# LJacksonPan/RaTrack

Hardware: AMD Instinct MI355X
Metric: radar frame-pairs/sec (backbone forward, eval) at B=64,N=256 per GPU (higher is better)
Workload: dtype f32 (2xfp16 split MFMA: three fp16 products per fp32 product, fp32 accumulate, power-of-two scales per matrix and position); 1 GPU; Track4D.backbone forward, B=64 frame-pairs x N=256 points per GPU, S=512 centroids, eval-mode BN, random-init weights, hipGraph=True, batches in flight=4; global_batch=64, parallelism=replicas x1 (no collective on the forward path)

## Files before the change

include/rtk_fused.h:

```cpp
#ifndef RTK_FUSED_H
#define RTK_FUSED_H

#include "rtk_pointnet2.h"

#ifdef __cplusplus
extern "C" {
#endif

#define RTK_MAX_SRC 4
#define RTK_MAX_LAYERS 4

typedef struct {
    const float *ptr;
    int pitch;
    int channels;
    int per_sample;
} rtk_src_t;

#define RTK_LAYER_SPLIT 0x100
typedef struct {
    const float *w_packed;
    const float *bias;
    int cin16, cout16;
    int act;
    float inv_scale;
} rtk_layer_t;

typedef struct {
    const float *known_feats;
    int pitch, channels, m;
    const int *idx;
    const float *dist2;
    const int *nuniq;
} rtk_interp_t;

RTK_EXPORT int rtk_pointwise_mlp(int rows, int rows_per_sample, const rtk_interp_t *interp, int nsrc,
                                 const rtk_src_t *srcs, const float *sample_bias, int nlayers,
                                 const rtk_layer_t *layers, float *out, int out_pitch, int out_channels,
                                 int out_channel_major, const int *row_nuniq, float *colmax, rtk_stream_t stream);

RTK_EXPORT int rtk_sa_scale(int samples, int n, int npoint, int nsample, const float *xyz,
                            const float *new_xyz, const int *idx, const float *q, int q_pitch, int c1_16,
                            const float *w1xyz_packed, int nlayers, const rtk_layer_t *layers, float *out,
                            int out_pitch, int out_offset, const int *src_nuniq, const int *dst_nuniq,
                            rtk_stream_t stream);

RTK_EXPORT int rtk_cost_volume(int samples, int n1, int n2, const float *xyz1, const float *xyz2,
                               const int64_t *knn_idx, const float *p1, const float *p2,
                               const float *wd_packed, const rtk_layer_t *layers,
                               const rtk_layer_t *wn, float *out, int out_pitch, rtk_stream_t stream);

RTK_EXPORT int rtk_patch_cost(int samples, int n, const float *xyz, const int64_t *knn_idx,
                              const float *feat, int feat_pitch, const rtk_layer_t *wn, float *out,
                              int out_pitch, int out_channel_major, rtk_stream_t stream);

RTK_EXPORT int rtk_pack_split_layer(int cout, int cin, const float *w, int transposed, void *image, float *inv_scale,
                                    rtk_stream_t stream);
RTK_EXPORT int rtk_cost_volume_split(int samples, int n1, int n2, const float *xyz1, const float *xyz2,
                                     const int64_t *knn_idx, const float *p1, const float *p2, const float *wd_packed,
                                     const void *split_images, const float *image_scales, const float *bias2,
                                     const float *bias3, const rtk_layer_t *wn, float *out, int out_pitch, rtk_stream_t stream);
RTK_EXPORT int rtk_cost_volume_split_shared(int samples, int n1, int n2, const float *xyz1, const float *xyz2,
                                            const int64_t *knn_idx, const float *p1, const float *p2, const float *wd_packed,
                                            const void *split_images, const float *image_scales, const float *bias2,
                                            const float *bias3, const rtk_layer_t *wn, float *out, int out_pitch, int workgroups,
                                            rtk_stream_t stream);
RTK_EXPORT int rtk_sa_scale_split(int samples, int n, int npoint, int nsample, const float *xyz, const float *new_xyz,
                                  const int *idx, const float *q, int q_pitch, int c1, const float *w1xyz_packed,
                                  const void *split_image, const float *image_scale, const float *bias2, float *out, int out_pitch,
                                  int out_offset, const int *src_nuniq, const int *dst_nuniq, rtk_stream_t stream);
RTK_EXPORT int rtk_split_mlp2(int positions, const float *x, const void *images, const float *image_scales, const float *bias1,
                              const float *bias2, float *y, rtk_stream_t stream);

RTK_EXPORT int rtk_prepare_inputs(int b, int n, const float *pc1, const float *pc2, const float *feature1,
                                  const float *feature2, float *xyz, float *raw, rtk_stream_t stream);

RTK_EXPORT int rtk_fps_centroids(int b, int n, int npoint, const float *xyz, int *idx, float *new_xyz, int *nuniq,
                                 int *tie, const int *n_valid, float *snap, int *first_tie, rtk_stream_t stream);

RTK_EXPORT int rtk_knn_point_masked(int b, int s, int n, int k, const float *query, const float *points, int64_t *idx,
                                    const int *n_valid, rtk_stream_t stream);

RTK_EXPORT int rtk_fps_relevel(int b, int npoint, int levels, const float *xyz1, const int *nuniq1, const int *tie,
                               int *idx, float *new_xyz, int *nuniq, int *tie_work, const int *idx1, const float *snap1,
                               int snap_pitch, const int *first_tie1, rtk_stream_t stream);

RTK_EXPORT int rtk_gru_step(int b, int layers, int hidden, const float *x, const float *h_in, const float *w_ih,
                            const float *w_hh, const float *b_ih, const float *b_hh, float *h_out, float *y,
                            rtk_stream_t stream);

RTK_EXPORT int rtk_gru_step_head(int b, int layers, int hidden, const float *x, const float *h_in, const float *w_ih,
                                 const float *w_hh, const float *b_ih, const float *b_hh, float *h_out, float *y, const float *head_wt,
                                 const float *head_bias, float *head_out, int head_cout, rtk_stream_t stream);

#define RTK_GT_MAX_JOBS 4
typedef struct {
    const float *wt, *bias;
    float *out;
    int cout, s0, count, out_pitch;
} rtk_gterm_job_t;
RTK_EXPORT int rtk_global_terms(int samples, int cin, const float *g, int njobs, const rtk_gterm_job_t *jobs, float *bcast, int bcast_pitch,
                                int n, rtk_stream_t stream);

#define RTK_COPY_MAX_JOBS 8
typedef struct {
    const void *src;
    void *dst;
    long bytes;
} rtk_copy_job_t;
RTK_EXPORT int rtk_copy_multi(int njobs, const rtk_copy_job_t *jobs, rtk_stream_t stream);

RTK_EXPORT int rtk_to_channel_major(int samples, int n, int channels, const float *src, int src_pitch, int per_sample,
                                    float *dst, int dst_channels, int dst_channel_offset, rtk_stream_t stream);

RTK_EXPORT int rtk_ball_query_pair(int b, int n, int npoint, float radius1, int nsample1, float radius2, int nsample2,
                                   const float *new_xyz, const float *xyz, int *idx1, int *idx2, const int *nuniq,
                                   rtk_stream_t stream);

RTK_EXPORT int rtk_three_nn_masked(int b, int n, int m, const float *unknown, const float *known, float *dist2, int *idx,
                                   const int *unknown_nuniq, const int *known_nuniq, rtk_stream_t stream);

RTK_EXPORT int rtk_geometry_front(int b, int clouds, int n, int npoint, const float *frame1, const float *frame2, int channel_major,
                                  const float *feature1, const float *feature2, float *xyz, float *raw, int *fps_idx, float *new_xyz,
                                  int *nuniq, int *tie, int *first_tie, float *snap, const int *n_valid, int64_t *knn12, int64_t *knn11,
                                  const float *q1_w, float *q1_out, int q1_cout, rtk_stream_t stream);
RTK_EXPORT int rtk_geometry_tables(int samples, int n, int npoint, const float *xyz0, const float *new_xyz, const int *nuniq,
                                   const float *radii, const int *nsamples, int *const *ball, int *const *nn_idx, float *const *nn_dist2,
                                   rtk_stream_t stream);

typedef struct {
    const float *src; float *dst;
    int channels, src_pitch, per_sample, dst_channels, dst_channel_offset;
} rtk_layout_job_t;
RTK_EXPORT int rtk_to_channel_major_multi(int samples, int n, int njobs, const rtk_layout_job_t *jobs, rtk_stream_t stream);

RTK_EXPORT int rtk_log_sinkhorn(int m, int n, const float *scores, float alpha, int iters, float *out, rtk_stream_t stream);

RTK_EXPORT int rtk_dbscan(int n, const float *feat, int pitch, const int *channels, const float *score, float threshold, double eps,
                          int min_samples, int *labels, rtk_stream_t stream);

#define RTK_DESC 141

typedef struct {
    const float *ptr;
    long long sb, sc, sp;
} rtk_bcn_view_t;

typedef struct {
    int B, N;
    rtk_bcn_view_t pc1, flow, feature1, prop, cls;
    const int *n_valid;
    const unsigned char *active;
} rtk_track_frame_t;

#define RTK_DBSCAN_POINT_BYTES 48
RTK_EXPORT int rtk_dbscan_batched(const rtk_track_frame_t *frame, float threshold, double eps, int min_samples, int K, int *labels,
                                  int *obj, int *num_objects, int *flags, void *work, long long work_bytes, rtk_stream_t stream);

RTK_EXPORT int rtk_object_descriptors(const rtk_track_frame_t *frame, int K, const int *obj, const int *num_objects,
                                      const int *prev_count, const float *desc_prev, float *desc, rtk_stream_t stream);

#define RTK_AFFINITY_WEIGHTS (141 * 564 + 564 + 564 * 282 + 282 + 282 * 70 + 70 + 70 * 35 + 35 + 35 + 1)
RTK_EXPORT int rtk_affinity_pairs(int B, int K, const float *weights, const float *desc_prev, const int *prev_count,
                                  const unsigned char *reset, const float *desc, const int *num_objects, float *aff,
                                  rtk_stream_t stream);

RTK_EXPORT int rtk_associate_batched(int B, int N, int K, const unsigned char *active, const unsigned char *reset, const float *aff,
                                     const int *num_objects, const int *obj, const int *prev_ids, const int *prev_count, float alpha,
                                     int iters, int *counter, int *ids, int *count, int *object_ids, float *object_conf, int *indices1,
                                     int *num_prev, int *point_track_id, float *scores, rtk_stream_t stream);

RTK_EXPORT int rtk_track_max_objects(void);

#ifdef __cplusplus
}
#endif
#endif
```

ratrack_amd/csrc/fused_common.h:

```cpp
#pragma once
#include <hip/hip_runtime.h>

#include <utility>

typedef float f4 __attribute__((ext_vector_type(4)));

#define RTK_ACT_NONE 0
#define RTK_ACT_RELU 1
#define RTK_ACT_LEAKY 2
#define RTK_ACT_SIGMOID 3

__device__ __forceinline__ f4 f4_zero() { return (f4){0.f, 0.f, 0.f, 0.f}; }

__device__ __forceinline__ f4 mfma4(float a, float b, f4 c) { return __builtin_amdgcn_mfma_f32_16x16x4f32(a, b, c, 0, 0, 0); }

__device__ __forceinline__ float act1(float x, int act) {
    switch (act) {
        case RTK_ACT_RELU: return fmaxf(x, 0.f);
        case RTK_ACT_LEAKY: return x > 0.f ? x : 0.1f * x;
        case RTK_ACT_SIGMOID: return 1.f / (1.f + __expf(-x));
        default: return x;
    }
}

// ... 111 lines not shown
struct LayerStep {
    static constexpr int G = V >= 4 ? 4 : V;
    static constexpr int GV = (V + G - 1) / G;
    static constexpr int NG = U * GV;
    template <int GJ>
    static __device__ __forceinline__ void load(WS &ws, f4 (&dst)[G]) {
        constexpr int u = GJ / GV, v0 = (GJ % GV) * G;
#pragma unroll
        for (int q = 0; q < G; ++q) {
            if (v0 + q < V) {
                const int fi = FBASE + u * V + v0 + q;
                if (fi % F == 0 && fi != 0) ws.next();
                dst[q] = ws.frag(fi % F);
            }
        }
    }
    static __device__ __forceinline__ void run(WS &ws, const f4 (&h)[U], f4 (&acc)[V], f4 (&a)[2][G]) {
        constexpr int u = GI / GV, v0 = (GI % GV) * G;
        if constexpr (GI + 1 < NG) load<GI + 1>(ws, a[(GI + 1) & 1]);
        f4(&c)[G] = a[GI & 1];
#pragma unroll
        for (int q = 0; q < G; ++q) if (v0 + q < V) acc[v0 + q] = mfma4(c[q].x, h[u].x, acc[v0 + q]);
#pragma unroll
        for (int q = 0; q < G; ++q) if (v0 + q < V) acc[v0 + q] = mfma4(c[q].y, h[u].y, acc[v0 + q]);
#pragma unroll
        for (int q = 0; q < G; ++q) if (v0 + q < V) acc[v0 + q] = mfma4(c[q].z, h[u].z, acc[v0 + q]);
#pragma unroll
        for (int q = 0; q < G; ++q) if (v0 + q < V) acc[v0 + q] = mfma4(c[q].w, h[u].w, acc[v0 + q]);
        __builtin_amdgcn_sched_barrier(0);
    }
};

template <int U, int V, int FBASE, class WS, int F, int... GI>
__device__ __forceinline__ void mlp_layer_ws_impl(WS &ws, const f4 (&h)[U], f4 (&acc)[V], std::integer_sequence<int, GI...>) {
    constexpr int G = V >= 4 ? 4 : V;
    f4 a[2][G];
    LayerStep<U, V, FBASE, 0, WS, F>::template load<0>(ws, a[0]);
    (LayerStep<U, V, FBASE, GI, WS, F>::run(ws, h, acc, a), ...);
}

template <int U, int V, int FBASE, int NW, int F, int NF>
__device__ __forceinline__ void mlp_layer_ws(WStream<NW, F, NF> &ws, const f4 (&h)[U], f4 (&acc)[V]) {
    constexpr int G = V >= 4 ? 4 : V;
    constexpr int NG = U * ((V + G - 1) / G);
    mlp_layer_ws_impl<U, V, FBASE, WStream<NW, F, NF>, F>(ws, h, acc, std::make_integer_sequence<int, NG>{});
}


typedef __bf16 bf8v __attribute__((ext_vector_type(8)));
typedef unsigned u4v __attribute__((ext_vector_type(4)));

__device__ __forceinline__ unsigned pack_hi16(float lo, float hi) {
    return __builtin_amdgcn_perm(__float_as_uint(hi), __float_as_uint(lo), 0x07060302u);
}
__device__ __forceinline__ float trunc_bf16(float x) { return __uint_as_float(__float_as_uint(x) & 0xffff0000u); }

__device__ __forceinline__ void split3(const f4 x0, const f4 x1, u4v (&b)[3]) {
    float x[8] = {x0.x, x0.y, x0.z, x0.w, x1.x, x1.y, x1.z, x1.w}, r1[8], r2[8];
#pragma unroll
    for (int t = 0; t < 8; ++t) {
        r1[t] = __fsub_rn(x[t], trunc_bf16(x[t]));
        r2[t] = __fsub_rn(r1[t], trunc_bf16(r1[t]));
    }
#pragma unroll
    for (int w = 0; w < 4; ++w) {
        b[0][w] = pack_hi16(x[2 * w], x[2 * w + 1]);
        b[1][w] = pack_hi16(r1[2 * w], r1[2 * w + 1]);
        b[2][w] = pack_hi16(r2[2 * w], r2[2 * w + 1]);
    }
}


typedef _Float16 h8v __attribute__((ext_vector_type(8)));
typedef _Float16 h2v __attribute__((ext_vector_type(2)));
typedef float f2v __attribute__((ext_vector_type(2)));

struct LaneScale {
    float s;
    float inv;
    unsigned mb;
};
__device__ __forceinline__ LaneScale lane_scale_of(unsigned mbits) {
    const unsigned e = mbits >> 23;
    unsigned sf = 268u - e;
    sf = sf > 253u ? 253u : sf;
    return LaneScale{__uint_as_float(sf << 23), __uint_as_float((254u - sf) << 23), mbits};
}
__device__ __forceinline__ void tensor_amax_update(float *amax, unsigned mb) {
#pragma unroll
    for (int d = 32; d >= 1; d >>= 1) { const unsigned o = (unsigned)__shfl_xor((int)mb, d, 64); mb = o > mb ? o : mb; }
    if ((threadIdx.x & 63) == 0 && mb > __atomic_load_n(reinterpret_cast<unsigned *>(amax), __ATOMIC_RELAXED))
        atomicMax(reinterpret_cast<unsigned *>(amax), mb);
}

template <int N>
__device__ __forceinline__ float abs_max_f4(const f4 (&h)[N]) {
    float m = 0.f;
#pragma unroll
    for (int e = 0; e < N; ++e) {
        m = __builtin_fmaxf(__builtin_fmaxf(m, __builtin_fabsf(h[e].x)), __builtin_fabsf(h[e].y));
        m = __builtin_fmaxf(__builtin_fmaxf(m, __builtin_fabsf(h[e].z)), __builtin_fabsf(h[e].w));
    }
    return m;
}
struct SplitWord { unsigned h, l; };
__device__ __forceinline__ SplitWord split2_word(float xa, float xb, float s) {
    const f2v xs = (f2v){xa, xb} * s;
    const h2v h = __builtin_convertvector(xs, h2v);
    const _Float16 la = (_Float16)__builtin_fmaf(xa, s, -(float)h[0]);
    const _Float16 lb = (_Float16)__builtin_fmaf(xb, s, -(float)h[1]);
    return SplitWord{__builtin_bit_cast(unsigned, h), __builtin_bit_cast(unsigned, (h2v){la, lb})};
}
__device__ __forceinline__ void split2(const f4 x0, const f4 x1, float s, u4v (&b)[2]) {
    const SplitWord w0 = split2_word(x0.x, x0.y, s), w1 = split2_word(x0.z, x0.w, s), w2 = split2_word(x1.x, x1.y, s), w3 = split2_word(x1.z, x1.w, s);
    b[0] = (u4v){w0.h, w1.h, w2.h, w3.h};
    b[1] = (u4v){w0.l, w1.l, w2.l, w3.l};
}
__device__ __forceinline__ f4 mfma16_h(u4v a, u4v b, f4 c) {
    return __builtin_amdgcn_mfma_f32_16x16x32_f16(__builtin_bit_cast(h8v, a), __builtin_bit_cast(h8v, b), c, 0, 0, 0);
}

__device__ __forceinline__ f4 mfma16_bf(u4v a, u4v b, f4 c) {
    return __builtin_amdgcn_mfma_f32_16x16x32_bf16(__builtin_bit_cast(bf8v, a), __builtin_bit_cast(bf8v, b), c, 0, 0, 0);
}

constexpr int split16_nf(int U, int V) { return ((U + 1) / 2) * V * 2; }

template <int N>
__device__ __forceinline__ LaneScale lane_scale16(const f4 (&h)[N]) {
    unsigned mb = __float_as_uint(abs_max_f4(h));
    auto r = __builtin_amdgcn_permlane16_swap(mb, mb, false, false);
    mb = r[0] > r[1] ? r[0] : r[1];
    r = __builtin_amdgcn_permlane32_swap(mb, mb, false, false);
    return lane_scale_of(r[0] > r[1] ? r[0] : r[1]);
}

template <int U, int V, int FBASE, int GI, class WS, int F>
struct LayerStepS {
    static constexpr int GV = (V + 1) / 2;
    static constexpr int NG = ((U + 1) / 2) * GV;
    template <int GJ>
    static __device__ __forceinline__ void load(WS &ws, f4 (&dst)[4]) {
        constexpr int up = GJ / GV, v0 = (GJ % GV) * 2;
#pragma unroll
        for (int q = 0; q < 4; ++q) {
            if (v0 + q / 2 < V) {
                const int fi = FBASE + (up * V + v0 + q / 2) * 2 + q % 2;
                if (fi % F == 0 && fi != 0) ws.next();
                dst[q] = ws.frag(fi % F);
            }
        }
    }
    static __device__ __forceinline__ void run(WS &ws, const f4 (&h)[U], float scale, f4 (&acc)[V], f4 (&a)[2][4], u4v (&b)[2]) {
        constexpr int up = GI / GV, v0 = (GI % GV) * 2;
        if constexpr (GI + 1 < NG) load<GI + 1>(ws, a[(GI + 1) & 1]);
        if constexpr (GI % GV == 0) split2(h[2 * up], 2 * up + 1 < U ? h[2 * up + 1] : f4_zero(), scale, b);
        const f4(&c)[4] = a[GI & 1];
#define RTK_S16_MM(pa, pb)                                                                            \
        acc[v0] = mfma16_h(__builtin_bit_cast(u4v, c[pa]), b[pb], acc[v0]);                            \
        if constexpr (v0 + 1 < V) acc[v0 + 1] = mfma16_h(__builtin_bit_cast(u4v, c[2 + pa]), b[pb], acc[v0 + 1]);
        RTK_S16_MM(1, 0) RTK_S16_MM(0, 1) RTK_S16_MM(0, 0)
#undef RTK_S16_MM
        __builtin_amdgcn_sched_barrier(0);
    }
};

template <int U, int V, int FBASE, class WS, int F, int... GI>
__device__ __forceinline__ void mlp_layer_split_impl(WS &ws, const f4 (&h)[U], float scale, f4 (&acc)[V], std::integer_sequence<int, GI...>) {
    f4 a[2][4];
    u4v b[2];
    LayerStepS<U, V, FBASE, 0, WS, F>::template load<0>(ws, a[0]);
    (LayerStepS<U, V, FBASE, GI, WS, F>::run(ws, h, scale, acc, a, b), ...);
}

template <int U, int V, int FBASE, int NW, int F, int NF>
__device__ __forceinline__ void mlp_layer_ws_split(WStream<NW, F, NF> &ws, const f4 (&h)[U], float scale, f4 (&acc)[V]) {
    constexpr int NG = ((U + 1) / 2) * ((V + 1) / 2);
    mlp_layer_split_impl<U, V, FBASE, WStream<NW, F, NF>, F>(ws, h, scale, acc, std::make_integer_sequence<int, NG>{});
}

struct WResident {
    const f4 *w;
    int lane;
    __device__ __forceinline__ void next() {}
    __device__ __forceinline__ f4 frag(int f) const { return w[f * 64 + lane]; }
};

template <int U, int V>
__device__ __forceinline__ void mlp_layer_res(const f4 *w, int lane, const f4 (&h)[U], f4 (&acc)[V]) {
    constexpr int G = V >= 4 ? 4 : V;
    constexpr int NG = U * ((V + G - 1) / G);
    WResident wr{w, lane};
    mlp_layer_ws_impl<U, V, 0, WResident, (1 << 30)>(wr, h, acc, std::make_integer_sequence<int, NG>{});
}

__device__ __forceinline__ f4 bias_frag(const float *__restrict__ bias, int v, int g) {
    return *reinterpret_cast<const f4 *>(bias + 16 * v + 4 * g);
}

__device__ __forceinline__ void rtk_dpp_fence(f4 &v) {
    int zero;
    asm volatile("s_mov_b32 %0, 0" : "=s"(zero));
    v.x = __int_as_float(__float_as_int(v.x) | zero);
    v.y = __int_as_float(__float_as_int(v.y) | zero);
    v.z = __int_as_float(__float_as_int(v.z) | zero);
    v.w = __int_as_float(__float_as_int(v.w) | zero);
}
#define RTK_DPP4(op, ctrl)                                                 \
    op " %0, %0, %0 " ctrl " row_mask:0xf bank_mask:0xf\n"                 \
    op " %1, %1, %1 " ctrl " row_mask:0xf bank_mask:0xf\n"                 \
    op " %2, %2, %2 " ctrl " row_mask:0xf bank_mask:0xf\n"                 \
    op " %3, %3, %3 " ctrl " row_mask:0xf bank_mask:0xf\n"

__device__ __forceinline__ void row_max16_f4(f4 &v) {
    rtk_dpp_fence(v);
    asm volatile("s_nop 1\n" RTK_DPP4("v_max_f32_dpp", "row_ror:8") RTK_DPP4("v_max_f32_dpp", "row_ror:4")
                 RTK_DPP4("v_max_f32_dpp", "row_ror:2") RTK_DPP4("v_max_f32_dpp", "row_ror:1")
                 : "+v"(v.x), "+v"(v.y), "+v"(v.z), "+v"(v.w));
}

__device__ __forceinline__ void row_sum16_f4(f4 &v) {
    rtk_dpp_fence(v);
    asm volatile("s_nop 1\n" RTK_DPP4("v_add_f32_dpp", "row_ror:8") RTK_DPP4("v_add_f32_dpp", "row_ror:4")
                 RTK_DPP4("v_add_f32_dpp", "row_ror:2") RTK_DPP4("v_add_f32_dpp", "row_ror:1")
                 : "+v"(v.x), "+v"(v.y), "+v"(v.z), "+v"(v.w));
}

__device__ __forceinline__ void row_sum16_valu_f4(f4 &v) {
    asm volatile("s_nop 1\n" RTK_DPP4("v_add_f32_dpp", "row_ror:8") RTK_DPP4("v_add_f32_dpp", "row_ror:4")
                 RTK_DPP4("v_add_f32_dpp", "row_ror:2") RTK_DPP4("v_add_f32_dpp", "row_ror:1")
                 : "+v"(v.x), "+v"(v.y), "+v"(v.z), "+v"(v.w));
}

#define RTK_DPP16(op, ctrl)                                                                                                          \
    op " %0, %0, %0 " ctrl " row_mask:0xf bank_mask:0xf\n" op " %1, %1, %1 " ctrl " row_mask:0xf bank_mask:0xf\n"                   \
    op " %2, %2, %2 " ctrl " row_mask:0xf bank_mask:0xf\n" op " %3, %3, %3 " ctrl " row_mask:0xf bank_mask:0xf\n"                   \
    op " %4, %4, %4 " ctrl " row_mask:0xf bank_mask:0xf\n" op " %5, %5, %5 " ctrl " row_mask:0xf bank_mask:0xf\n"                   \
    op " %6, %6, %6 " ctrl " row_mask:0xf bank_mask:0xf\n" op " %7, %7, %7 " ctrl " row_mask:0xf bank_mask:0xf\n"                   \
    op " %8, %8, %8 " ctrl " row_mask:0xf bank_mask:0xf\n" op " %9, %9, %9 " ctrl " row_mask:0xf bank_mask:0xf\n"                   \
    op " %10, %10, %10 " ctrl " row_mask:0xf bank_mask:0xf\n" op " %11, %11, %11 " ctrl " row_mask:0xf bank_mask:0xf\n"             \
    op " %12, %12, %12 " ctrl " row_mask:0xf bank_mask:0xf\n" op " %13, %13, %13 " ctrl " row_mask:0xf bank_mask:0xf\n"             \
    op " %14, %14, %14 " ctrl " row_mask:0xf bank_mask:0xf\n" op " %15, %15, %15 " ctrl " row_mask:0xf bank_mask:0xf\n"
__device__ __forceinline__ void row_sum16_valu_f4x4(f4 (&v)[4]) {
    asm volatile("s_nop 1\n" RTK_DPP16("v_add_f32_dpp", "row_ror:8") RTK_DPP16("v_add_f32_dpp", "row_ror:4")
                 RTK_DPP16("v_add_f32_dpp", "row_ror:2") RTK_DPP16("v_add_f32_dpp", "row_ror:1")
                 : "+v"(v[0].x), "+v"(v[0].y), "+v"(v[0].z), "+v"(v[0].w), "+v"(v[1].x), "+v"(v[1].y), "+v"(v[1].z), "+v"(v[1].w),
                   "+v"(v[2].x), "+v"(v[2].y), "+v"(v[2].z), "+v"(v[2].w), "+v"(v[3].x), "+v"(v[3].y), "+v"(v[3].z), "+v"(v[3].w));
}

#define RTK_DPP_PAIR(op, c0, m0, c1, m1)                                                                                     \
    asm volatile("s_nop 1\n"                                                                                                 \
                 op " %0, %0, %0 " c0 " row_mask:0xf bank_mask:" m0 "\n" op " %1, %1, %1 " c0 " row_mask:0xf bank_mask:" m0 "\n"  \
                 op " %2, %2, %2 " c0 " row_mask:0xf bank_mask:" m0 "\n" op " %3, %3, %3 " c0 " row_mask:0xf bank_mask:" m0 "\n"  \
                 op " %0, %4, %4 " c1 " row_mask:0xf bank_mask:" m1 "\n" op " %1, %5, %5 " c1 " row_mask:0xf bank_mask:" m1 "\n"  \
                 op " %2, %6, %6 " c1 " row_mask:0xf bank_mask:" m1 "\n" op " %3, %7, %7 " c1 " row_mask:0xf bank_mask:" m1 "\n"  \
                 : "+v"(a.x), "+v"(a.y), "+v"(a.z), "+v"(a.w) : "v"(b.x), "v"(b.y), "v"(b.z), "v"(b.w))
__device__ __forceinline__ void row_max_pair8(f4 &a, const f4 b) { RTK_DPP_PAIR("v_max_f32_dpp", "row_ror:8", "0x3", "row_ror:8", "0xc"); }
__device__ __forceinline__ void row_max_pair4(f4 &a, const f4 b) { RTK_DPP_PAIR("v_max_f32_dpp", "row_shl:4", "0x5", "row_shr:4", "0xa"); }
__device__ __forceinline__ void row_sum_pair8(f4 &a, const f4 b) { RTK_DPP_PAIR("v_add_f32_dpp", "row_ror:8", "0x3", "row_ror:8", "0xc"); }
__device__ __forceinline__ void row_sum_pair4(f4 &a, const f4 b) { RTK_DPP_PAIR("v_add_f32_dpp", "row_shl:4", "0x5", "row_shr:4", "0xa"); }
#undef RTK_DPP_PAIR
__device__ __forceinline__ void quad_max_valu_f4(f4 &v) {
    asm volatile("s_nop 1\n" RTK_DPP4("v_max_f32_dpp", "quad_perm:[1,0,3,2]") RTK_DPP4("v_max_f32_dpp", "quad_perm:[2,3,0,1]")
                 : "+v"(v.x), "+v"(v.y), "+v"(v.z), "+v"(v.w));
}
__device__ __forceinline__ void quad_sum_valu_f4(f4 &v) {
    asm volatile("s_nop 1\n" RTK_DPP4("v_add_f32_dpp", "quad_perm:[1,0,3,2]") RTK_DPP4("v_add_f32_dpp", "quad_perm:[2,3,0,1]")
                 : "+v"(v.x), "+v"(v.y), "+v"(v.z), "+v"(v.w));
}
__device__ __forceinline__ f4 wave_max_pair16(const f4 a, const f4 b, float inf) {
    f4 o;
#pragma unroll
    for (int r = 0; r < 4; ++r) {
        const auto t = __builtin_amdgcn_permlane16_swap(__float_as_uint(a[r]), __float_as_uint(b[r]), false, false);
        o[r] = __builtin_amdgcn_fmed3f(__uint_as_float(t[0]), __uint_as_float(t[1]), inf);
    }
    return o;
}
__device__ __forceinline__ f4 row_max16_transpose4(f4 q0, f4 q1, const f4 q2, const f4 q3) {
    row_max_pair8(q0, q2);
    row_max_pair8(q1, q3);
    row_max_pair4(q0, q1);
    quad_max_valu_f4(q0);
    return q0;
}
__device__ __forceinline__ f4 row_sum16_transpose4(f4 q0, f4 q1, const f4 q2, const f4 q3) {
    row_sum_pair8(q0, q2);
    row_sum_pair8(q1, q3);
    row_sum_pair4(q0, q1);
    quad_sum_valu_f4(q0);
    return q0;
}

template <int GROUP>
__device__ __forceinline__ void row_max_group_f4(f4 &v) {
    if constexpr (GROUP >= 16) {
        row_max16_f4(v);
    } else if constexpr (GROUP == 8) {
        rtk_dpp_fence(v);
        asm volatile("s_nop 1\n" RTK_DPP4("v_max_f32_dpp", "quad_perm:[1,0,3,2]") RTK_DPP4("v_max_f32_dpp", "quad_perm:[2,3,0,1]")
                     RTK_DPP4("v_max_f32_dpp", "row_half_mirror")
                     : "+v"(v.x), "+v"(v.y), "+v"(v.z), "+v"(v.w));
    } else {
        rtk_dpp_fence(v);
        asm volatile("s_nop 1\n" RTK_DPP4("v_max_f32_dpp", "quad_perm:[1,0,3,2]") RTK_DPP4("v_max_f32_dpp", "quad_perm:[2,3,0,1]")
                     : "+v"(v.x), "+v"(v.y), "+v"(v.z), "+v"(v.w));
    }
}
```

ratrack_amd/csrc/fused_misc.hip:

```cpp
#include <math.h>

#include "assoc_common.h"
#include "rtk_common.h"
#include "rtk_fused.h"
#include "rtk_train.h"

__global__ void prepare_inputs_kernel(int b, int n, const float *__restrict__ pc1, const float *__restrict__ pc2,
                                      const float *__restrict__ f1, const float *__restrict__ f2, float *__restrict__ xyz,
                                      float *__restrict__ raw) {
    const long t = (long)blockIdx.x * blockDim.x + threadIdx.x;
    if (t >= 2L * b * n) return;
    const int s = (int)(t / n), p = (int)(t % n);
    const bool second = s >= b;
    const int sb = second ? s - b : s;
    const float *pc = second ? pc2 : pc1;
    const float *f = second ? f2 : f1;
    xyz[t * 3 + 0] = pc[((long)sb * 3 + 0) * n + p];
    xyz[t * 3 + 1] = pc[((long)sb * 3 + 1) * n + p];
    xyz[t * 3 + 2] = pc[((long)sb * 3 + 2) * n + p];
    *reinterpret_cast<float4 *>(raw + t * 4) = make_float4(f[((long)sb * 2 + 0) * n + p], f[((long)sb * 2 + 1) * n + p], 0.f, 0.f);
}

extern "C" int rtk_prepare_inputs(int b, int n, const float *pc1, const float *pc2, const float *feature1,
                                  const float *feature2, float *xyz, float *raw, rtk_stream_t stream) {
    RTK_REQUIRE(b > 0 && n > 0 && pc1 && pc2 && feature1 && feature2 && xyz && raw, "prepare_inputs: bad arguments");
    const long total = 2L * b * n;
    prepare_inputs_kernel<<<rtk_divup(total, 256), 256, 0, (hipStream_t)stream>>>(b, n, pc1, pc2, feature1, feature2, xyz, raw);
    RTK_CHECK_LAUNCH("prepare_inputs");
    return RTK_OK;
}

#define GRU_MAXL 8
constexpr int GRU_INFLIGHT = 32;
__global__ __launch_bounds__(384) void gru_step_kernel(int b, int layers, int hidden, const float *__restrict__ x,
                                                       const float *__restrict__ h_in, const float *__restrict__ w_ih,
                                                       const float *__restrict__ w_hh, const float *__restrict__ b_ih,
                                                       const float *__restrict__ b_hh, float *__restrict__ h_out,
                                                       float *__restrict__ y, const float *__restrict__ head_wt,
                                                       const float *__restrict__ head_bias, float *__restrict__ head_out, int head_cout) {
    __shared__ float s_x[128], s_h[128], s_gi[384], s_gh[384];
    const int s = blockIdx.x, t = threadIdx.x, H = hidden;
    if (t < H) s_x[t] = x[(long)s * H + t];
    for (int l = 0; l < layers; ++l) {
        if (t < H) s_h[t] = h_in[((long)l * b + s) * H + t];
        __syncthreads();
        if (t < 3 * H) {
            const float *wi = w_ih + (long)l * H * 3 * H + t;
            const float *wh = w_hh + (long)l * H * 3 * H + t;
            float ai = b_ih[l * 3 * H + t], ah = b_hh[l * 3 * H + t];
            for (int k0 = 0; k0 < H; k0 += GRU_INFLIGHT) {
                float wv[GRU_INFLIGHT], uv[GRU_INFLIGHT];
#pragma unroll
                for (int q = 0; q < GRU_INFLIGHT; ++q) {
                    wv[q] = wi[(long)(k0 + q) * 3 * H];
                    uv[q] = wh[(long)(k0 + q) * 3 * H];
                }
#pragma unroll
                for (int q = 0; q < GRU_INFLIGHT; ++q) {
                    ai = fmaf(wv[q], s_x[k0 + q], ai);
                    ah = fmaf(uv[q], s_h[k0 + q], ah);
                }
            }
            s_gi[t] = ai;
            s_gh[t] = ah;
        }
        __syncthreads();
        if (t < H) {
            const float r = 1.f / (1.f + expf(-(s_gi[t] + s_gh[t])));
            const float z = 1.f / (1.f + expf(-(s_gi[H + t] + s_gh[H + t])));
            const float nn = tanhf(s_gi[2 * H + t] + r * s_gh[2 * H + t]);
            const float hn = (1.f - z) * nn + z * s_h[t];
            h_out[((long)l * b + s) * H + t] = hn;
            s_x[t] = hn;
            if (l == layers - 1) y[(long)s * H + t] = hn;
        }
        __syncthreads();
    }
    if (head_wt) {
        for (int c = t; c < head_cout; c += blockDim.x) {
            float acc = head_bias ? head_bias[c] : 0.f;
            for (int k0 = 0; k0 < H; k0 += 16) {
                float wv[16];
#pragma unroll
                for (int q = 0; q < 16; ++q) wv[q] = head_wt[(long)(k0 + q) * head_cout + c];
#pragma unroll
                for (int q = 0; q < 16; ++q) acc = fmaf(wv[q], s_x[k0 + q], acc);
            }
            head_out[(long)s * head_cout + c] = acc;
        }
    }
}

extern "C" int rtk_gru_step(int b, int layers, int hidden, const float *x, const float *h_in, const float *w_ih,
                            const float *w_hh, const float *b_ih, const float *b_hh, float *h_out, float *y,
                            rtk_stream_t stream) {
    RTK_REQUIRE(b > 0 && layers > 0 && layers <= GRU_MAXL && hidden > 0 && hidden <= 128 && hidden % GRU_INFLIGHT == 0 && x && h_in && w_ih &&
                w_hh && b_ih && b_hh && h_out && y, "gru_step: bad arguments (hidden=%d, layers=%d)", hidden, layers);
    gru_step_kernel<<<b, 384, 0, (hipStream_t)stream>>>(b, layers, hidden, x, h_in, w_ih, w_hh, b_ih, b_hh, h_out, y, nullptr, nullptr, nullptr, 0);
    RTK_CHECK_LAUNCH("gru_step");
    return RTK_OK;
}

extern "C" int rtk_gru_step_head(int b, int layers, int hidden, const float *x, const float *h_in, const float *w_ih,
                                 const float *w_hh, const float *b_ih, const float *b_hh, float *h_out, float *y, const float *head_wt,
                                 const float *head_bias, float *head_out, int head_cout, rtk_stream_t stream) {
    RTK_REQUIRE(b > 0 && layers > 0 && layers <= GRU_MAXL && hidden > 0 && hidden <= 128 && hidden % GRU_INFLIGHT == 0 && x && h_in && w_ih &&
                w_hh && b_ih && b_hh && h_out && y && head_wt && head_out && head_cout > 0,
                "gru_step_head: bad arguments (hidden=%d, layers=%d, head_cout=%d)", hidden, layers, head_cout);
    gru_step_kernel<<<b, 384, 0, (hipStream_t)stream>>>(b, layers, hidden, x, h_in, w_ih, w_hh, b_ih, b_hh, h_out, y, head_wt, head_bias,
                                                        head_out, head_cout);
    RTK_CHECK_LAUNCH("gru_step_head");
    return RTK_OK;
}

struct GtParams {
    int samples, cin, njobs, n, bcast_pitch;
    const float *g;
    float *bcast;
    rtk_gterm_job_t job[RTK_GT_MAX_JOBS];
};

__global__ __launch_bounds__(256) void global_terms_kernel(const GtParams P) {
    __shared__ __attribute__((aligned(16))) float s_g[512];
    const int s = blockIdx.x, t = threadIdx.x;
    for (int k = t; k < P.cin; k += 256) s_g[k] = P.g[(long)s * P.cin + k];
    __syncthreads();
    int total = 0;
    for (int j = 0; j < P.njobs; ++j)
        if (s >= P.job[j].s0 && s < P.job[j].s0 + P.job[j].count) total += P.job[j].cout;
    for (int o = blockIdx.y * 256 + t; o < total; o += 256 * gridDim.y) {
        int c = o, j = 0;
        for (; j < P.njobs; ++j) {
            if (s < P.job[j].s0 || s >= P.job[j].s0 + P.job[j].count) continue;
            if (c < P.job[j].cout) break;
            c -= P.job[j].cout;
        }
        const rtk_gterm_job_t &J = P.job[j];
        float acc = J.bias ? J.bias[c] : 0.f;
        for (int k0 = 0; k0 < P.cin; k0 += 64) {
            float wv[64];
#pragma unroll
            for (int q = 0; q < 64; ++q) wv[q] = J.wt[(long)min(k0 + q, P.cin - 1) * J.cout + c];
#pragma unroll
            for (int q = 0; q < 64; ++q)
                if (k0 + q < P.cin) acc = fmaf(wv[q], s_g[k0 + q], acc);
        }
        J.out[(long)(s - J.s0) * J.out_pitch + c] = acc;
    }
    if (P.bcast) {
        const int per_row = P.cin >> 2, rows_per_iter = 256 / per_row, q = t % per_row;
        if (t < rows_per_iter * per_row) {
            const float4 v = *reinterpret_cast<const float4 *>(s_g + 4 * q);
            for (int r = blockIdx.y * rows_per_iter + t / per_row; r < P.n; r += rows_per_iter * gridDim.y)
                *reinterpret_cast<float4 *>(P.bcast + ((long)s * P.n + r) * P.bcast_pitch + 4 * q) = v;
        }
    }
}

extern "C" int rtk_global_terms(int samples, int cin, const float *g, int njobs, const rtk_gterm_job_t *jobs, float *bcast, int bcast_pitch,
                                int n, rtk_stream_t stream) {
    RTK_REQUIRE(samples > 0 && cin > 0 && cin <= 512 && cin % 32 == 0 && g && njobs >= 0 && njobs <= RTK_GT_MAX_JOBS && (njobs == 0 || jobs),
                "global_terms: bad arguments (samples=%d cin=%d njobs=%d)", samples, cin, njobs);
    RTK_REQUIRE(!bcast || (n > 0 && bcast_pitch >= cin && bcast_pitch % 4 == 0 && cin <= 1024), "global_terms: bad broadcast target");
    GtParams P;
    P.samples = samples; P.cin = cin; P.njobs = njobs; P.n = n; P.bcast_pitch = bcast_pitch; P.g = g; P.bcast = bcast;
    for (int j = 0; j < njobs; ++j) {
        RTK_REQUIRE(jobs[j].wt && jobs[j].out && jobs[j].cout > 0 && jobs[j].s0 >= 0 && jobs[j].count >= 0 && jobs[j].s0 + jobs[j].count <= samples &&
                    jobs[j].out_pitch >= jobs[j].cout, "global_terms: bad job %d", j);
        P.job[j] = jobs[j];
    }
    global_terms_kernel<<<dim3(samples, bcast ? 8 : 2), 256, 0, (hipStream_t)stream>>>(P);
    RTK_CHECK_LAUNCH("global_terms");
    return RTK_OK;
}

struct CopyParams {
    int njobs;
    rtk_copy_job_t job[RTK_COPY_MAX_JOBS];
    long first_block[RTK_COPY_MAX_JOBS + 1];
};
constexpr int COPY_BLOCK_BYTES = 256 * 16 * 4;

__global__ __launch_bounds__(256) void copy_multi_kernel(const CopyParams P) {
    const long blk = blockIdx.x;
    int j = 0;
#pragma unroll
    for (int q = 1; q < RTK_COPY_MAX_JOBS; ++q) j += (q < P.njobs && blk >= P.first_block[q]) ? 1 : 0;
    const rtk_copy_job_t &J = P.job[j];
    const long off = (blk - P.first_block[j]) * COPY_BLOCK_BYTES;
    const char *src = reinterpret_cast<const char *>(J.src) + off;
    char *dst = reinterpret_cast<char *>(J.dst) + off;
    const long left = J.bytes - off;
    if ((((uintptr_t)src | (uintptr_t)dst) & 15) == 0) {
#pragma unroll
        for (int u = 0; u < 4; ++u) {
            const long o = ((long)u * 256 + threadIdx.x) * 16;
            if (o + 16 <= left) *reinterpret_cast<float4 *>(dst + o) = *reinterpret_cast<const float4 *>(src + o);
            else for (long b = o; b < left && b < o + 16; b += 4) *reinterpret_cast<float *>(dst + b) = *reinterpret_cast<const float *>(src + b);
        }
    } else {
        for (long o = (long)threadIdx.x * 4; o < left && o < COPY_BLOCK_BYTES; o += 256 * 4)
            *reinterpret_cast<float *>(dst + o) = *reinterpret_cast<const float *>(src + o);
    }
}

extern "C" int rtk_copy_multi(int njobs, const rtk_copy_job_t *jobs, rtk_stream_t stream) {
    RTK_REQUIRE(njobs > 0 && njobs <= RTK_COPY_MAX_JOBS && jobs, "copy_multi: %d jobs (1..%d)", njobs, RTK_COPY_MAX_JOBS);
    CopyParams P;
    P.njobs = njobs;
    long blocks = 0;
    for (int j = 0; j < njobs; ++j) {
        RTK_REQUIRE(jobs[j].src && jobs[j].dst && jobs[j].bytes > 0 && jobs[j].bytes % 4 == 0 &&
                    (((uintptr_t)jobs[j].src | (uintptr_t)jobs[j].dst) & 3) == 0, "copy_multi: bad job %d", j);
        P.job[j] = jobs[j];
        P.first_block[j] = blocks;
        blocks += (jobs[j].bytes + COPY_BLOCK_BYTES - 1) / COPY_BLOCK_BYTES;
    }
    P.first_block[njobs] = blocks;
    RTK_REQUIRE(blocks < 0x7fffffffL, "copy_multi: too large");
    copy_multi_kernel<<<(unsigned)blocks, 256, 0, (hipStream_t)stream>>>(P);
    RTK_CHECK_LAUNCH("copy_multi");
    return RTK_OK;
}

__global__ __launch_bounds__(384) void gru_step_bwd_kernel(int b, int layers, int hidden, const float *__restrict__ x,
                                                           const float *__restrict__ h_in, const float *__restrict__ h_out,
                                                           const float *__restrict__ w_ih_t, const float *__restrict__ w_hh_t,
                                                           const float *__restrict__ w_ih, const float *__restrict__ w_hh,
                                                           const float *__restrict__ b_ih, const float *__restrict__ b_hh,
                                                           const float *__restrict__ dy, const float *__restrict__ dh_out,
                                                           float *__restrict__ dx, float *__restrict__ dh_in, float *__restrict__ dgi,
                                                           float *__restrict__ dgh) {
    __shared__ float s_x[128], s_h[128], s_gi[384], s_gh[384], s_dx[3][128], s_dh[3][128], s_carry[128], s_direct[128];
    const int s = blockIdx.x, t = threadIdx.x, H = hidden;
    if (t < H) s_carry[t] = dy[(long)s * H + t];
    for (int l = layers - 1; l >= 0; --l) {
        if (t < H) {
            s_x[t] = l == 0 ? x[(long)s * H + t] : h_out[((long)(l - 1) * b + s) * H + t];
            s_h[t] = h_in[((long)l * b + s) * H + t];
        }
        __syncthreads();
        if (t < 3 * H) {
            const float *wi = w_ih_t + (long)l * H * 3 * H + t;
            const float *wh = w_hh_t + (long)l * H * 3 * H + t;
            float ai = b_ih[l * 3 * H + t], ah = b_hh[l * 3 * H + t];
            for (int k0 = 0; k0 < H; k0 += GRU_INFLIGHT) {
                float wv[GRU_INFLIGHT], uv[GRU_INFLIGHT];
#pragma unroll
                for (int q = 0; q < GRU_INFLIGHT; ++q) {
                    wv[q] = wi[(long)(k0 + q) * 3 * H];
                    uv[q] = wh[(long)(k0 + q) * 3 * H];
                }
#pragma unroll
                for (int q = 0; q < GRU_INFLIGHT; ++q) {
                    ai = fmaf(wv[q], s_x[k0 + q], ai);
                    ah = fmaf(uv[q], s_h[k0 + q], ah);
                }
            }
            s_gi[t] = ai;
            s_gh[t] = ah;
        }
        __syncthreads();
        float g_r = 0.f, g_z = 0.f, g_n = 0.f, g_nr = 0.f;
        if (t < H) {
            const float r = 1.f / (1.f + expf(-(s_gi[t] + s_gh[t])));
            const float z = 1.f / (1.f + expf(-(s_gi[H + t] + s_gh[H + t])));
            const float hn = s_gh[2 * H + t];
            const float nn = tanhf(s_gi[2 * H + t] + r * hn);
            const float dhp = s_carry[t] + (dh_out ? dh_out[((long)l * b + s) * H + t] : 0.f);
            const float dn = dhp * (1.f - z) * (1.f - nn * nn);
            g_n = dn;
            g_nr = dn * r;
            g_r = dn * hn * r * (1.f - r);
            g_z = dhp * (s_h[t] - nn) * z * (1.f - z);
            s_direct[t] = dhp * z;
        }
        __syncthreads();
        if (t < H) {
            s_gi[t] = g_r; s_gi[H + t] = g_z; s_gi[2 * H + t] = g_n;
            s_gh[t] = g_r; s_gh[H + t] = g_z; s_gh[2 * H + t] = g_nr;
        }
        __syncthreads();
        if (t < 3 * H) {
            dgi[((long)l * b + s) * 3 * H + t] = s_gi[t];
            dgh[((long)l * b + s) * 3 * H + t] = s_gh[t];
        }
        {
            const int part = t / H, j = t % H;
            if (part < 3) {
                const float *wi = w_ih + ((long)l * 3 * H + (long)part * H) * H + j;
                const float *wh = w_hh + ((long)l * 3 * H + (long)part * H) * H + j;
                float ax = 0.f, ah = 0.f;
                for (int i0 = 0; i0 < H; i0 += 16) {
                    float wv[16], uv[16];
#pragma unroll
                    for (int q = 0; q < 16; ++q) {
                        wv[q] = wi[(long)(i0 + q) * H];
                        uv[q] = wh[(long)(i0 + q) * H];
                    }
#pragma unroll
                    for (int q = 0; q < 16; ++q) {
                        ax = fmaf(wv[q], s_gi[part * H + i0 + q], ax);
                        ah = fmaf(uv[q], s_gh[part * H + i0 + q], ah);
                    }
                }
                s_dx[part][j] = ax;
                s_dh[part][j] = ah;
            }
        }
        __syncthreads();
        if (t < H) {
            const float gx = s_dx[0][t] + s_dx[1][t] + s_dx[2][t];
            dh_in[((long)l * b + s) * H + t] = s_direct[t] + (s_dh[0][t] + s_dh[1][t] + s_dh[2][t]);
            s_carry[t] = gx;
            if (l == 0) dx[(long)s * H + t] = gx;
        }
        __syncthreads();
    }
}

extern "C" int rtk_gru_step_bwd(int b, int layers, int hidden, const float *x, const float *h_in, const float *h_out,
// ... 143 lines not shown
```

ratrack_amd/csrc/fused_pointwise.hip:

```cpp
#include <string.h>

#include "rtk_common.h"
#include "fused_common.h"
#include "rtk_fused.h"

struct PwParams {
    int rows, rows_per_sample;
    rtk_interp_t interp;
    int nsrc;
    rtk_src_t src[RTK_MAX_SRC];
    const float *sample_bias;
    rtk_layer_t layer[RTK_MAX_LAYERS];
    float *out;
    int out_pitch, out_channels, out_cm;
    const int *row_nuniq;
    float *colmax;
    int gx;
};

template <int V>
__device__ __forceinline__ void init_bias(f4 (&acc)[V], const float *__restrict__ bias, int g) {
#pragma unroll
    for (int v = 0; v < V; ++v) acc[v] = bias_frag(bias, v, g);
}
template <int V>
__device__ __forceinline__ void init_zero(f4 (&acc)[V]) {
#pragma unroll
    for (int v = 0; v < V; ++v) acc[v] = f4_zero();
}
template <int V>
__device__ __forceinline__ void scale_bias(f4 (&acc)[V], float c, const float *__restrict__ bias, int g) {
#pragma unroll
    for (int v = 0; v < V; ++v) acc[v] = __builtin_elementwise_fma(acc[v], (f4){c, c, c, c}, bias_frag(bias, v, g));
}

template <bool SPLIT, int U, int V, int FBASE, class WS>
__device__ __forceinline__ void pw_layer(WS &ws, const f4 (&h)[U], f4 (&acc)[V], const rtk_layer_t &L, int g, const float *sample_bias, bool first) {
    if constexpr (SPLIT) {
        const LaneScale sc = lane_scale16(h);
        init_zero<V>(acc);
        if (first) ws.next_if_deferred();
        mlp_layer_ws_split<U, V, FBASE>(ws, h, sc.s, acc);
        scale_bias<V>(acc, sc.inv * L.inv_scale, L.bias, g);
    } else {
        init_bias<V>(acc, L.bias, g);
        if (first) ws.next_if_deferred();
        mlp_layer_ws<U, V, FBASE>(ws, h, acc);
    }
    if (sample_bias) {
#pragma unroll
        for (int v = 0; v < V; ++v) acc[v] += bias_frag(sample_bias, v, g);
    }
    apply_act<V>(acc, L.act);
}

template <int V>
__device__ __forceinline__ void store_tile(const PwParams &P, const f4 (&acc)[V], int p, int b, int g, bool valid) {
    if (P.colmax) {
        unsigned *cm = reinterpret_cast<unsigned *>(P.colmax) + (size_t)b * 16 * V + 4 * g;
        const bool lead = (threadIdx.x & 15) == 0;
#pragma unroll
        for (int v = 0; v < V; ++v) {
            f4 m = valid ? acc[v] : f4_zero();
            row_max16_f4(m);
            if (lead) {
                atomicMax(cm + 16 * v + 0, __float_as_uint(m.x));
                atomicMax(cm + 16 * v + 1, __float_as_uint(m.y));
                atomicMax(cm + 16 * v + 2, __float_as_uint(m.z));
                atomicMax(cm + 16 * v + 3, __float_as_uint(m.w));
            }
        }
    }
    if (!valid) return;
    if (!P.out_cm) {
        float *o = P.out + (size_t)p * P.out_pitch;
#pragma unroll
        for (int v = 0; v < V; ++v) {
            const int c = 16 * v + 4 * g;
            if (c + 3 < P.out_channels) {
                *reinterpret_cast<f4 *>(o + c) = acc[v];
            } else {
                if (c + 0 < P.out_channels) o[c + 0] = acc[v].x;
                if (c + 1 < P.out_channels) o[c + 1] = acc[v].y;
                if (c + 2 < P.out_channels) o[c + 2] = acc[v].z;
            }
        }
    } else {
        const int n = P.rows_per_sample;
        float *o = P.out + (size_t)b * P.out_channels * n + (p - b * n);
#pragma unroll
        for (int v = 0; v < V; ++v) {
            const int c = 16 * v + 4 * g;
            if (c + 0 < P.out_channels) o[(size_t)(c + 0) * n] = acc[v].x;
            if (c + 1 < P.out_channels) o[(size_t)(c + 1) * n] = acc[v].y;
            if (c + 2 < P.out_channels) o[(size_t)(c + 2) * n] = acc[v].z;
            if (c + 3 < P.out_channels) o[(size_t)(c + 3) * n] = acc[v].w;
        }
    }
}

#define PW_NW 4
#ifndef PW_WGS_TARGET
#define PW_WGS_TARGET 256
#endif
#ifndef PW_F
#define PW_F 16
#endif

template <int U, int V1, int V2, int V3, int V4, bool INTERP, bool SPLIT>
__global__ __launch_bounds__(64 * PW_NW, 2) void pointwise_mlp_kernel(const PwParams P) {
    __shared__ __attribute__((aligned(16))) f4 s_w[2 * PW_F * 64];
    const int lane = threadIdx.x & 63, g = lane >> 4, j = lane & 15;
    const int wave_in_wg = threadIdx.x >> 6;
    int b, bx, nbx;
    rtk_decode_block(P.gx, b, bx, nbx);
    const int rps = P.rows_per_sample;
    const int live_rows = P.row_nuniq ? min(rps, __builtin_amdgcn_readfirstlane(P.row_nuniq[b])) : rps;
    const int live_groups = (live_rows + PW_NW * 16 - 1) / (PW_NW * 16);
    if (bx >= live_groups) return;
    constexpr int F1 = SPLIT ? split16_nf(U, V1) : U * V1, F2 = SPLIT ? split16_nf(V1, V2) : V1 * V2,
                  F3 = SPLIT ? split16_nf(V2, V3) : V2 * V3, F4 = SPLIT ? split16_nf(V3, V4) : V3 * V4;
    constexpr int NF = F1 + F2 + F3 + F4;
    WStream<PW_NW, PW_F, NF> ws;
    if constexpr (NF > PW_F) ws.start_deferred(reinterpret_cast<const f4 *>(P.layer[0].w_packed), s_w, wave_in_wg, lane);
    else ws.start(reinterpret_cast<const f4 *>(P.layer[0].w_packed), s_w, wave_in_wg, lane);

    int ustart[RTK_MAX_SRC + 1];
    ustart[0] = INTERP ? (P.interp.channels + 15) >> 4 : 0;
#pragma unroll
    for (int s = 0; s < RTK_MAX_SRC; ++s) ustart[s + 1] = ustart[s] + (s < P.nsrc ? (P.src[s].channels + 15) >> 4 : 0);
    const int uend = ustart[RTK_MAX_SRC];

    for (int G = bx; G < live_groups; G += nbx) {
        asm volatile("" ::: "memory");
        const int r = G * (PW_NW * 16) + wave_in_wg * 16 + j;
        const bool valid = r < live_rows;
        const int p = b * rps + (r < rps ? r : rps - 1);

        f4 h[U];
        if (INTERP) {
            const int *idp = P.interp.idx + (size_t)p * 3;
            int id[3] = {idp[0], idp[1], idp[2]};
            if (P.interp.nuniq) {
                const int e = P.interp.nuniq[b];
                id[0] = id[0] < e ? id[0] : 0; id[1] = id[1] < e ? id[1] : 0; id[2] = id[2] < e ? id[2] : 0;
            }
            const float *d2 = P.interp.dist2 + (size_t)p * 3;
            const float r0 = __fdiv_rn(1.0f, __fadd_rn(__fsqrt_rn(d2[0]), 1e-8f));
            const float r1 = __fdiv_rn(1.0f, __fadd_rn(__fsqrt_rn(d2[1]), 1e-8f));
            const float r2 = __fdiv_rn(1.0f, __fadd_rn(__fsqrt_rn(d2[2]), 1e-8f));
            const float norm = __fadd_rn(__fadd_rn(r0, r1), r2);
            const float w0 = __fdiv_rn(r0, norm), w1 = __fdiv_rn(r1, norm), w2 = __fdiv_rn(r2, norm);
            const float *k0 = P.interp.known_feats + ((size_t)b * P.interp.m + id[0]) * P.interp.pitch;
            const float *k1 = P.interp.known_feats + ((size_t)b * P.interp.m + id[1]) * P.interp.pitch;
            const float *k2 = P.interp.known_feats + ((size_t)b * P.interp.m + id[2]) * P.interp.pitch;
#pragma unroll
            for (int u = 0; u < U; ++u) {
                if (u < ustart[0]) {
                    const int c = 16 * u + 4 * g;
                    const bool ok = c < P.interp.channels;
                    const int cc = ok ? c : 0;
                    const f4 a0 = *reinterpret_cast<const f4 *>(k0 + cc);
                    const f4 a1 = *reinterpret_cast<const f4 *>(k1 + cc);
                    const f4 a2 = *reinterpret_cast<const f4 *>(k2 + cc);
                    f4 v;
                    v.x = __fmaf_rn(w2, a2.x, __fmaf_rn(w1, a1.x, __fmul_rn(w0, a0.x)));
                    v.y = __fmaf_rn(w2, a2.y, __fmaf_rn(w1, a1.y, __fmul_rn(w0, a0.y)));
                    v.z = __fmaf_rn(w2, a2.z, __fmaf_rn(w1, a1.z, __fmul_rn(w0, a0.z)));
                    v.w = __fmaf_rn(w2, a2.w, __fmaf_rn(w1, a1.w, __fmul_rn(w0, a0.w)));
                    h[u] = ok ? v : f4_zero();
                }
            }
        }
        const float *rowp[RTK_MAX_SRC];
        const float *dummy = reinterpret_cast<const float *>(P.layer[0].w_packed);
#pragma unroll
        for (int q = 0; q < RTK_MAX_SRC; ++q)
            rowp[q] = q < P.nsrc ? P.src[q].ptr + (P.src[q].per_sample ? (size_t)b : (size_t)p) * P.src[q].pitch + 4 * g : nullptr;
#pragma unroll
        for (int u = 0; u < U; ++u) {
            if (!INTERP || u >= ustart[0]) {
                const float *rp = rowp[0];
                int us = ustart[0], ch = P.src[0].channels;
#pragma unroll
                for (int q = 1; q < RTK_MAX_SRC; ++q)
                    if (q < P.nsrc && u >= ustart[q]) { rp = rowp[q]; us = ustart[q]; ch = P.src[q].channels; }
                const int c = 16 * (u - us);
                const bool ok = u < uend && c + 4 * g < ch;
                const f4 v = *reinterpret_cast<const f4 *>(ok ? rp + c : dummy);
                h[u] = ok ? v : f4_zero();
            }
        }

        f4 a1[V1];
        pw_layer<SPLIT, U, V1, 0>(ws, h, a1, P.layer[0], g, P.sample_bias ? P.sample_bias + (size_t)b * 16 * V1 : nullptr, true);
        if constexpr (V2 == 0) {
            store_tile<V1>(P, a1, p, b, g, valid);
        } else {
            f4 a2[V2];
            pw_layer<SPLIT, V1, V2, F1>(ws, a1, a2, P.layer[1], g, nullptr, false);
            if constexpr (V3 == 0) {
                store_tile<V2>(P, a2, p, b, g, valid);
            } else {
                f4 a3[V3];
                pw_layer<SPLIT, V2, V3, F1 + F2>(ws, a2, a3, P.layer[2], g, nullptr, false);
                if constexpr (V4 == 0) {
                    store_tile<V3>(P, a3, p, b, g, valid);
                } else {
                    f4 a4[V4];
                    pw_layer<SPLIT, V3, V4, F1 + F2 + F3>(ws, a3, a4, P.layer[3], g, nullptr, false);
                    store_tile<V4>(P, a4, p, b, g, valid);
                }
            }
        }
    }
    ws.finish();
}

template <int U, int V1, int V2, int V3, int V4>
static int launch_pw(const PwParams &P0, bool interp, bool split, hipStream_t s) {
    PwParams P = P0;
    const int samples = P.rows / P.rows_per_sample;
    const int groups = (P.rows_per_sample + PW_NW * 16 - 1) / (PW_NW * 16);
    int gx = PW_WGS_TARGET / samples;
    if (gx < 1) gx = 1;
    if (gx > groups) gx = groups;
    P.gx = samples % 8 == 0 ? gx : 0;
    const dim3 blocks = P.gx ? dim3(gx * samples) : dim3(gx, samples);
    if (interp && split) pointwise_mlp_kernel<U, V1, V2, V3, V4, true, true><<<blocks, 256, 0, s>>>(P);
    else if (interp) pointwise_mlp_kernel<U, V1, V2, V3, V4, true, false><<<blocks, 256, 0, s>>>(P);
    else if (split) pointwise_mlp_kernel<U, V1, V2, V3, V4, false, true><<<blocks, 256, 0, s>>>(P);
    else pointwise_mlp_kernel<U, V1, V2, V3, V4, false, false><<<blocks, 256, 0, s>>>(P);
    return 0;
}

extern "C" int rtk_pointwise_mlp(int rows, int rows_per_sample, const rtk_interp_t *interp, int nsrc,
                                 const rtk_src_t *srcs, const float *sample_bias, int nlayers,
                                 const rtk_layer_t *layers, float *out, int out_pitch, int out_channels,
                                 int out_channel_major, const int *row_nuniq, float *colmax, rtk_stream_t stream) {
    RTK_REQUIRE(rows > 0 && rows_per_sample > 0 && rows % rows_per_sample == 0 && rows / rows_per_sample <= 65535,
                "pointwise_mlp: bad row counts (%d, %d)", rows, rows_per_sample);
    RTK_REQUIRE(nsrc >= 0 && nsrc <= RTK_MAX_SRC && (nsrc == 0 || srcs), "pointwise_mlp: nsrc=%d", nsrc);
    RTK_REQUIRE(nlayers >= 1 && nlayers <= RTK_MAX_LAYERS && layers && out, "pointwise_mlp: nlayers=%d", nlayers);
    PwParams P;
    memset(&P, 0, sizeof(P));
    P.rows = rows;
    P.rows_per_sample = rows_per_sample;
    int U = 0;
    if (interp) {
        RTK_REQUIRE(interp->known_feats && interp->idx && interp->dist2 && interp->pitch % 4 == 0 && interp->channels % 4 == 0,
                    "pointwise_mlp: bad interp segment");
        P.interp = *interp;
        U += (interp->channels + 15) / 16;
    }
    P.nsrc = nsrc;
    for (int s = 0; s < nsrc; ++s) {
        RTK_REQUIRE(srcs[s].ptr && srcs[s].pitch % 4 == 0 && srcs[s].channels > 0 && srcs[s].pitch >= ((srcs[s].channels + 3) / 4) * 4,
                    "pointwise_mlp: bad source %d (pitch %d, channels %d)", s, srcs[s].pitch, srcs[s].channels);
        P.src[s] = srcs[s];
        U += (srcs[s].channels + 15) / 16;
    }
    P.sample_bias = sample_bias;
    int V[RTK_MAX_LAYERS] = {0, 0, 0, 0};
    int cin = U;
    const bool split = (layers[0].act & RTK_LAYER_SPLIT) != 0;
    for (int l = 0; l < nlayers; ++l) {
        RTK_REQUIRE(layers[l].w_packed && layers[l].bias && layers[l].cin16 == cin && layers[l].cout16 > 0,
                    "pointwise_mlp: layer %d expects cin16=%d, got %d (cout16=%d)", l, cin, layers[l].cin16, layers[l].cout16);
        RTK_REQUIRE(((layers[l].act & RTK_LAYER_SPLIT) != 0) == split, "pointwise_mlp: split and fp32 images in one chain (layer %d)", l);
        const size_t prev_floats = l == 0 ? 0 : (split ? (size_t)split16_nf(layers[l - 1].cin16, layers[l - 1].cout16) * 256
                                                        : (size_t)layers[l - 1].cin16 * layers[l - 1].cout16 * 256);
        RTK_REQUIRE(l == 0 || layers[l].w_packed == layers[l - 1].w_packed + prev_floats,
                    "pointwise_mlp: the packed weights of a chain must be contiguous (layer %d)", l);
        P.layer[l] = layers[l];
        P.layer[l].act = layers[l].act & 0xff;
        V[l] = layers[l].cout16;
        cin = V[l];
    }
    P.out = out;
    P.out_pitch = out_pitch;
    P.out_channels = out_channels;
    P.out_cm = out_channel_major;
    P.row_nuniq = row_nuniq;
    P.colmax = colmax;
    RTK_REQUIRE(out_channels > 0 && out_channels <= 16 * cin, "pointwise_mlp: out_channels=%d", out_channels);
    RTK_REQUIRE(out_channel_major || (out_pitch % 4 == 0 && out_pitch >= out_channels), "pointwise_mlp: bad out_pitch %d", out_pitch);
    hipStream_t s = (hipStream_t)stream;
    const bool it = interp != nullptr;
    const long key = ((((long)U * 32 + V[0]) * 32 + V[1]) * 32 + V[2]) * 32 + V[3];
#define PW_CASE(u, v1, v2, v3, v4)                                               \
    case ((((long)(u) * 32 + (v1)) * 32 + (v2)) * 32 + (v3)) * 32 + (v4):        \
        launch_pw<u, v1, v2, v3, v4>(P, it, split, s);                           \
        break;
    switch (key) {
        PW_CASE(1, 2, 0, 0, 0)
        PW_CASE(4, 6, 0, 0, 0)
        PW_CASE(6, 12, 0, 0, 0)
        PW_CASE(8, 4, 0, 0, 0)
        PW_CASE(8, 8, 0, 0, 0)
        PW_CASE(10, 8, 0, 0, 0)
        PW_CASE(8, 16, 0, 0, 0)
        PW_CASE(16, 8, 4, 2, 1)
        PW_CASE(8, 8, 4, 2, 1)
        PW_CASE(25, 2, 0, 0, 0)
        PW_CASE(8, 2, 0, 0, 0)
        default:
            rtk_set_error("pointwise_mlp: no kernel instance for shape U=%d V=(%d,%d,%d,%d)", U, V[0], V[1], V[2], V[3]);
            return RTK_ERR_UNSUPPORTED;
    }
#undef PW_CASE
    RTK_CHECK_LAUNCH("pointwise_mlp");
    return RTK_OK;
}
```

ratrack_amd/csrc/fused_split.hip:

```cpp
#include "rtk_common.h"
#include "rtk_fused.h"
#include "split_mfma.h"

namespace {

#ifndef SP_NW
#define SP_NW 4
#endif
#ifndef SP_F
#define SP_F 32
#endif
constexpr int CV_F = 32;

__global__ __launch_bounds__(256) void pack_split_kernel(int cout, int cin, const float *__restrict__ w, int transposed, u4v *__restrict__ out,
                                                         float *__restrict__ inv_scale) {
    __shared__ unsigned s_m[4];
    float m = 0.f;
    const f4 *w4 = reinterpret_cast<const f4 *>(w);
    for (int i = threadIdx.x; i < cout * cin / 4; i += 256) {
        const f4 t = w4[i];
        m = __builtin_fmaxf(__builtin_fmaxf(m, __builtin_fabsf(t.x)), __builtin_fabsf(t.y));
        m = __builtin_fmaxf(__builtin_fmaxf(m, __builtin_fabsf(t.z)), __builtin_fabsf(t.w));
    }
    unsigned mb = __float_as_uint(m);
#pragma unroll
    for (int d = 32; d >= 1; d >>= 1) { const unsigned o = __shfl_xor(mb, d, 64); mb = o > mb ? o : mb; }
    if ((threadIdx.x & 63) == 0) s_m[threadIdx.x >> 6] = mb;
    __syncthreads();
    mb = max(max(s_m[0], s_m[1]), max(s_m[2], s_m[3]));
    const LaneScale sc = lane_scale_of(mb);
    if (blockIdx.x == 0 && threadIdx.x == 0) *inv_scale = sc.inv;
    const int VB = cout / 32, slot = blockIdx.x * 256 + threadIdx.x;
    if (slot >= (cin / 16) * VB * 64) return;
    const int lane = slot & 63, v = (slot >> 6) % VB, s = (slot >> 6) / VB, hh = lane >> 5, i = lane & 31;
    const int o = 32 * v + i, c0 = 32 * (s >> 1) + 16 * (s & 1) + 4 * hh;
    f4 x0, x1;
    if (transposed) {
#pragma unroll
        for (int r = 0; r < 4; ++r) { x0[r] = w[(size_t)(c0 + r) * cout + o]; x1[r] = w[(size_t)(c0 + 8 + r) * cout + o]; }
    } else {
        const float *row = w + (size_t)o * cin + c0;
        x0 = *reinterpret_cast<const f4 *>(row); x1 = *reinterpret_cast<const f4 *>(row + 8);
    }
    u4v b[2];
    split2(x0, x1, sc.s, b);
#pragma unroll
    for (int p = 0; p < 2; ++p) out[((size_t)(s * VB + v) * 2 + p) * 64 + lane] = b[p];
}

__device__ __forceinline__ f4 leaky_med4(f4 t, float inf) {
    const f4 u = t * 0.1f;
    return (f4){__builtin_amdgcn_fmed3f(t.x, u.x, inf), __builtin_amdgcn_fmed3f(t.y, u.y, inf), __builtin_amdgcn_fmed3f(t.z, u.z, inf),
                __builtin_amdgcn_fmed3f(t.w, u.w, inf)};
}
__device__ __forceinline__ f4 scale_bias4(f4 a, float c, f4 b) { return __builtin_elementwise_fma(a, (f4){c, c, c, c}, b); }
__device__ __forceinline__ float rtk_hidden_inf();

__global__ __launch_bounds__(64 * SP_NW) __attribute__((amdgpu_waves_per_eu(1, 1)))
void split_mlp2_kernel(int positions, const float *__restrict__ x, const f4 *__restrict__ blob, const float *__restrict__ wsc,
                       const float *__restrict__ bias1, const float *__restrict__ bias2, float *__restrict__ y) {
    const float kinf = rtk_hidden_inf();
    __shared__ __attribute__((aligned(16))) f4 s_w[2 * SP_F * 64];
    const int lane = threadIdx.x & 63, wave = __builtin_amdgcn_readfirstlane(threadIdx.x >> 6), hh = lane >> 5, col = lane & 31;
    constexpr int NF = 2 * SPLIT_NF;
    WStreamA<SP_NW, SP_F, NF> ws;
    ws.start_parts(blob, s_w, wave, lane);
    const float wi1 = ldc(wsc), wi2 = ldc(wsc + 1);
    const int tiles = (positions + 32 * SP_NW - 1) / (32 * SP_NW);
    for (int T = blockIdx.x; T < tiles; T += gridDim.x) {
        asm volatile("" ::: "memory");
        const long pos = (long)T * 32 * SP_NW + 32 * wave + col;
        const bool valid = pos < positions;
        const float *xr = x + (valid ? pos : (long)positions - 1) * 256 + 4 * hh;
        f4 h[32], bq[2][8];
#pragma unroll
        for (int i = 0; i < 32; ++i) h[i] = *reinterpret_cast<const f4 *>(xr + 8 * i);
        f16v acc[SPLIT_VB];
        LaneScale sc = lane_scale32(h);
        split_layer<0>(ws, h, sc.s, acc, BiasSide{bias1 + 4 * hh, bq});
        float c = sc.inv * wi1;
        split_epilogue(acc, bias1 + 4 * hh, bq, [&](int e, f4 a, f4 b) { h[e] = leaky_med4(scale_bias4(a, c, b), kinf); });
        sc = lane_scale32(h);
        split_layer<SPLIT_NF>(ws, h, sc.s, acc, BiasSide{bias2 + 4 * hh, bq});
        ws.sync();
        c = sc.inv * wi2;
        float *yr = y + pos * 256 + 4 * hh;
        split_epilogue(acc, bias2 + 4 * hh, bq, [&](int e, f4 a, f4 b) {
            if (valid) *reinterpret_cast<f4 *>(yr + 8 * e) = leaky_med4(scale_bias4(a, c, b), kinf);
        });
    }
    ws.finish();
}

__device__ __forceinline__ f16v mfma_f32x2(float a, float b, f16v c) { return __builtin_amdgcn_mfma_f32_32x32x2f32(a, b, c, 0, 0, 0); }

struct WnSplit {
    const float *wa;
    const float *wb, *wc;
    const float *bb, *bc;
};

struct CvSplitParams {
    int samples, n1, n2, gx;
    const float *xyz1, *xyz2;
    const int64_t *knn;
    const float *p1, *p2;
    const float *wd;
    const f4 *blob;
    const float *wsc;
    const float *bias2, *bias3;
    WnSplit wn;
    float *out;
    int out_pitch;
    float *amax;
    float *sv1, *sv2, *sv3;
    uint2 *mk1, *mk2;
};

__device__ __forceinline__ void split_sign_masks(const f4 (&a)[32], uint2 (&m)[2]) {
    m[0] = m[1] = make_uint2(0u, 0u);
#pragma unroll
    for (int v = 0; v < SPLIT_VB; ++v)
#pragma unroll
        for (int q = 0; q < 4; ++q)
#pragma unroll
            for (int r = 0; r < 4; ++r) {
                const unsigned bit = (a[4 * v + q][r] > 0.f ? 1u : 0u) << (4 * ((2 * v + (q >> 1)) & 7) + r);
                if (v < 4) m[q & 1].x |= bit; else m[q & 1].y |= bit;
            }
}
__device__ __forceinline__ unsigned split_mask_bits(const uint2 (&m)[2], int v, int q) {
    return ((v < 4 ? m[q & 1].x : m[q & 1].y) >> (4 * ((2 * v + (q >> 1)) & 7))) & 15u;
}

__device__ __forceinline__ f4 *cv_at(float *base, unsigned byte_off) { return reinterpret_cast<f4 *>(reinterpret_cast<char *>(base) + byte_off); }
__device__ __forceinline__ const f4 *cv_at(const float *base, unsigned byte_off) {
    return reinterpret_cast<const f4 *>(reinterpret_cast<const char *>(base) + byte_off);
}

__device__ __forceinline__ void wn_hidden(const WnSplit &W, float dx, float dy, float dz, float (&t2)[8]) {
    float t1[8];
#pragma unroll
    for (int o = 0; o < 8; ++o) {
        float a = __fmaf_rn(ldc(W.wa + o), dx, 0.f);
        a = __fmaf_rn(ldc(W.wa + 16 + o), dy, a);
        a = __fmaf_rn(ldc(W.wa + 32 + o), dz, a);
        t1[o] = fmaxf(__fadd_rn(a, ldc(W.wa + 48 + o)), 0.f);
    }
#pragma unroll
    for (int o = 0; o < 8; ++o) {
        float a = ldc(W.bb + o);
#pragma unroll
        for (int c = 0; c < 8; ++c) a = __fmaf_rn(ldc(W.wb + (16 * (c >> 2) + o) * 4 + (c & 3)), t1[c], a);
        t2[o] = fmaxf(a, 0.f);
    }
}
struct WnBlock {
    f16v bias;
    float w[4];
};
__device__ __forceinline__ WnBlock wn_block(const WnSplit &W, int v, int hh, int col) {
    WnBlock k;
    k.bias = split_bias(W.bc, v, hh);
    const int ch = 32 * v + col;
    const float *wr = W.wc + ((ch >> 4) * 64 + (ch & 15)) * 4;
#pragma unroll
    for (int st = 0; st < 4; ++st) {
        const int kk = 2 * st + hh;
        k.w[st] = ldc(wr + 64 * (kk >> 2) + (kk & 3));
    }
    return k;
}
__device__ __forceinline__ f16v wn_pre(const WnBlock &k, int hh, const float (&t2)[8]) {
    f16v w = k.bias;
#pragma unroll
    for (int st = 0; st < 4; ++st) w = mfma_f32x2(k.w[st], hh ? t2[2 * st + 1] : t2[2 * st], w);
    return w;
}
__device__ __forceinline__ float rtk_hidden_inf() {
    float v;
    asm volatile("s_mov_b32 %0, 0x7f800000" : "=s"(v));
    return v;
}
__device__ __forceinline__ float relu1(float x, float inf) { return __builtin_amdgcn_fmed3f(x, 0.f, inf); }
__device__ __forceinline__ f4 relu_med4(f4 t, float inf) { return (f4){relu1(t.x, inf), relu1(t.y, inf), relu1(t.z, inf), relu1(t.w, inf)}; }

constexpr int CV_ROWS_F4 = 32 * 32;
struct CvRowsRequest {
    const char *p2;
    f4 *rows;
    int nbrow;
    unsigned lanepart;
    int sub;
    __device__ __forceinline__ CvRowsRequest(const float *p2_, f4 *rows_, int nbrow_, int half, int lane)
        : p2(reinterpret_cast<const char *>(p2_)), rows(rows_), nbrow(nbrow_), lanepart(512u * half + (unsigned)(((lane & 31) ^ (lane >> 5)) << 4)), sub(lane >> 5) {}
    template <int T>
    __device__ __forceinline__ void one() const {
        const int r0 = __builtin_amdgcn_readlane(nbrow, 2 * T), r1 = __builtin_amdgcn_readlane(nbrow, 2 * T + 1);
        const unsigned off = ((unsigned)(sub ? r1 : r0) << 10) + (lanepart ^ (unsigned)(((2 * T) & 15) << 4));
        __builtin_amdgcn_global_load_lds((const __attribute__((address_space(1))) void *)(p2 + off),
                                         (__attribute__((address_space(3))) void *)(rows + T * 64), 16, 0, 0);
    }
    template <int... T>
    __device__ __forceinline__ void all(std::integer_sequence<int, T...>) const { (one<T>(), ...); }
};
template <int HALF>
__device__ __forceinline__ void cv_rows_request(const float *p2, int nbrow, f4 *rows, int lane) {
    asm volatile("s_waitcnt lgkmcnt(0)" ::: "memory");
    CvRowsRequest(p2, rows, nbrow, HALF, lane).all(std::make_integer_sequence<int, 16>{});
}
template <bool SAVE>
struct CvLayer2Side {
    StoreRowsSide st;
    CvRowsRequest rq;
    template <int GI>
    __device__ __forceinline__ void at(const f4 (&h)[32]) const {
        if constexpr (SAVE) st.template at<GI>(h);
        constexpr int per_chunk = CV_F / SPLIT_GF, ig = split_issue_groups(CV_F), g = GI % per_chunk, n = (GI / per_chunk) * ig + g;
        if constexpr (g < ig && 3 * n < 16) {
            rq.template one<3 * n>();
            if constexpr (3 * n + 1 < 16) rq.template one<3 * n + 1>();
            if constexpr (3 * n + 2 < 16) rq.template one<3 * n + 2>();
        }
    }
};
template <int HALF>
__device__ __forceinline__ void cv_rows_read(const f4 *rows, int col, int hh, f4 (&h)[32]) {
#pragma unroll
    for (int e = 0; e < 16; ++e) h[16 * HALF + e] = rows[col * 32 + ((2 * e + hh) ^ (col & 15))];
}
template <int K>
__device__ __forceinline__ f4 add_row_bcast(const f4 q, const f4 r) {
    f4 o;
    asm("s_nop 1\n"
        "v_add_f32_dpp %0, %4, %8 row_newbcast:%12 row_mask:0xf bank_mask:0xf\n"
        "v_add_f32_dpp %1, %5, %9 row_newbcast:%12 row_mask:0xf bank_mask:0xf\n"
        "v_add_f32_dpp %2, %6, %10 row_newbcast:%12 row_mask:0xf bank_mask:0xf\n"
        "v_add_f32_dpp %3, %7, %11 row_newbcast:%12 row_mask:0xf bank_mask:0xf"
        : "=&v"(o.x), "=&v"(o.y), "=&v"(o.z), "=&v"(o.w)
        : "v"(q.x), "v"(q.y), "v"(q.z), "v"(q.w), "v"(r.x), "v"(r.y), "v"(r.z), "v"(r.w), "n"(K));
    return o;
}
template <int K>
__device__ __forceinline__ f4 mul_row_bcast(const f4 q, const f4 r) {
    f4 o;
    asm("s_nop 1\n"
        "v_mul_f32_dpp %0, %4, %8 row_newbcast:%12 row_mask:0xf bank_mask:0xf\n"
        "v_mul_f32_dpp %1, %5, %9 row_newbcast:%12 row_mask:0xf bank_mask:0xf\n"
        "v_mul_f32_dpp %2, %6, %10 row_newbcast:%12 row_mask:0xf bank_mask:0xf\n"
        "v_mul_f32_dpp %3, %7, %11 row_newbcast:%12 row_mask:0xf bank_mask:0xf"
        : "=&v"(o.x), "=&v"(o.y), "=&v"(o.z), "=&v"(o.w)
        : "v"(q.x), "v"(q.y), "v"(q.z), "v"(q.w), "v"(r.x), "v"(r.y), "v"(r.z), "v"(r.w), "n"(K));
    return o;
}
template <int V0, int V1>
__device__ __forceinline__ void cv_layer1_blocks(const CvSplitParams &P, const f4 q0, const f4 q1, float b0, float b1, int hh, int col, float kinf, f4 (&h)[32]) {
    static_assert(V1 <= 8, "eight 32-channel blocks");
    auto block = [&](auto vc) {
        constexpr int v = decltype(vc)::value;
        f16v c;
        auto slot = [&](auto qc) {
            constexpr int q = decltype(qc)::value, e = 4 * v + q;
            const f4 t = add_row_bcast<e & 15>(e < 16 ? q0 : q1, h[e]);
            c[4 * q] = t.x; c[4 * q + 1] = t.y; c[4 * q + 2] = t.z; c[4 * q + 3] = t.w;
        };
        slot(std::integral_constant<int, 0>{}); slot(std::integral_constant<int, 1>{});
        slot(std::integral_constant<int, 2>{}); slot(std::integral_constant<int, 3>{});
        const int ch = 32 * v + col;
        const float *wr = P.wd + (ch >> 4) * 64 + (ch & 15);
        c = mfma_f32x2(ldc(wr + 16 * hh), b0, c);
        c = mfma_f32x2(ldc(wr + 16 * (2 + hh)), b1, c);
#pragma unroll
        for (int q = 0; q < 4; ++q) h[4 * v + q] = leaky_med4((f4){c[4 * q], c[4 * q + 1], c[4 * q + 2], c[4 * q + 3]}, kinf);
    };
    block(std::integral_constant<int, V0>{}); block(std::integral_constant<int, V0 + 1>{});
    block(std::integral_constant<int, V0 + 2>{}); block(std::integral_constant<int, V0 + 3>{});
}

#ifndef CV_FWD_VGPRS
#define CV_FWD_VGPRS 448
#endif
template <bool SAVE>
__global__ __launch_bounds__(64 * SP_NW) __attribute__((amdgpu_waves_per_eu(1, 1), amdgpu_num_vgpr(CV_FWD_VGPRS)))
void cost_volume_split_kernel(const CvSplitParams P) {
    const float kinf = rtk_hidden_inf();
    __shared__ __attribute__((aligned(16))) f4 s_w[2 * CV_F * 64];
    __shared__ __attribute__((aligned(16))) f4 s_rows[SP_NW * CV_ROWS_F4];
    const int lane = threadIdx.x & 63, wave = __builtin_amdgcn_readfirstlane(threadIdx.x >> 6), hh = lane >> 5, col = lane & 31, pp = col >> 4,
              j = col & 15;
    f4 *rows = s_rows + wave * CV_ROWS_F4;
    constexpr int PPW = 2 * SP_NW;
    const int groups = (P.n1 + PPW - 1) / PPW;
    const bool flat = P.gx > 0;
    const int xcd = blockIdx.x & 7, t0 = flat ? (int)(blockIdx.x >> 3) : (int)blockIdx.x, tstep = flat ? P.gx >> 3 : (int)gridDim.x;
    const int ntiles = flat ? (P.samples >> 3) * groups : groups;
    auto locate = [&](int t, int &b_, int &G_) {
        if (flat) { const int sk = t / groups; b_ = sk * 8 + xcd; G_ = t - sk * groups; }
        else { b_ = blockIdx.y; G_ = t; }
    };
    int b, bx;
    locate(t0 < ntiles ? t0 : 0, b, bx);
    WStreamA<SP_NW, CV_F, 2 * SPLIT_NF> ws;
    ws.start_parts(P.blob, s_w, wave, lane);
    const float wi2 = ldc(P.wsc), wi3 = ldc(P.wsc + 1);
    int pt = bx * PPW + 2 * wave + pp;
    bool valid = pt < P.n1;
    long i = (long)b * P.n1 + (valid ? pt : P.n1 - 1);
    long nb = 0;
    float dx = 0.f, dy = 0.f, dz = 0.f;
    f4 q0 = {0.f, 0.f, 0.f, 0.f}, q1 = q0;
    if (t0 < ntiles) {
        nb = (long)b * P.n2 + (long)P.knn[i * 16 + j];
        cv_rows_request<0>(P.p2, (int)nb, rows, lane);
        q0 = ldc4(P.p1 + i * 256 + 4 * hh + 8 * j); q1 = ldc4(P.p1 + i * 256 + 4 * hh + 8 * (16 + j));
        dx = __fsub_rn(P.xyz2[nb * 3], P.xyz1[i * 3]); dy = __fsub_rn(P.xyz2[nb * 3 + 1], P.xyz1[i * 3 + 1]);
        dz = __fsub_rn(P.xyz2[nb * 3 + 2], P.xyz1[i * 3 + 2]);
    }
    for (int t = t0; t < ntiles; t += tstep) {
        asm volatile("" ::: "memory");
        const bool more = t + tstep < ntiles;
        int bn, Gn;
        locate(more ? t + tstep : t, bn, Gn);
        const int ptn = Gn * PPW + 2 * wave + pp;
        const bool validn = ptn < P.n1;
        const long in_ = (long)bn * P.n1 + (validn ? ptn : P.n1 - 1);
        long knn_next = 0;
        if (more) knn_next = (long)P.knn[in_ * 16 + j];
        f4 h[32];
        float t2[8];
        {
            const float b0 = hh ? dy : dx, b1 = hh ? 0.f : dz;
            cv_rows_read<0>(rows, col, hh, h);
            cv_rows_request<1>(P.p2, (int)nb, rows, lane);
            cv_layer1_blocks<0, 4>(P, q0, q1, b0, b1, hh, col, kinf, h);
            wn_hidden(P.wn, dx, dy, dz, t2);
            __builtin_amdgcn_sched_barrier(0);
            cv_rows_read<1>(rows, col, hh, h);
            cv_layer1_blocks<4, 8>(P, q0, q1, b0, b1, hh, col, kinf, h);
        }
        const long nbn = (long)bn * P.n2 + knn_next;
        const long pos = i * 16 + j;
        const unsigned ro = (unsigned)pos * 1024u + 16u * hh;
        if (SAVE && valid) {
            uint2 m[2];
            split_sign_masks(h, m);
            P.mk1[pos * 4 + hh] = m[0];
            P.mk1[pos * 4 + 2 + hh] = m[1];
        }
        f16v acc[SPLIT_VB];
        f4 bq[2][8];
        LaneScale sc = lane_scale32(h);
        if (SAVE && P.amax) tensor_amax_update(P.amax, sc.mb);
        split_layer<0>(ws, h, sc.s, acc, SidePair<CvLayer2Side<SAVE>, BiasSide>{{StoreRowsSide{P.sv1, ro, valid}, CvRowsRequest(P.p2, rows, (int)nbn, 0, lane)},
                                                                              BiasSide{P.bias2 + 4 * hh, bq}});
        float c = sc.inv * wi2;
        split_epilogue(acc, P.bias2 + 4 * hh, bq, [&](int e, f4 a, f4 b) { h[e] = leaky_med4(scale_bias4(a, c, b), kinf); });
        if (SAVE && valid) {
            uint2 m[2];
            split_sign_masks(h, m);
            P.mk2[pos * 4 + hh] = m[0];
            P.mk2[pos * 4 + 2 + hh] = m[1];
        }
        sc = lane_scale32(h);
        if (SAVE && P.amax) tensor_amax_update(P.amax + 1, sc.mb);
        if (SAVE) split_layer<SPLIT_NF>(ws, h, sc.s, acc, SidePair<StoreRowsSide, BiasSide>{StoreRowsSide{P.sv2, ro, valid}, BiasSide{P.bias3 + 4 * hh, bq}});
        else split_layer<SPLIT_NF>(ws, h, sc.s, acc, BiasSide{P.bias3 + 4 * hh, bq});
        ws.sync();
        c = sc.inv * wi3;
        split_epilogue(acc, P.bias3 + 4 * hh, bq, [&](int e, f4 a, f4 b) { h[e] = leaky_med4(scale_bias4(a, c, b), kinf); });
        if (SAVE && valid) {
#pragma unroll
            for (int e = 0; e < 32; ++e) *cv_at(P.sv3, ro + 32u * e) = h[e];
        }
        WnBlock wk = wn_block(P.wn, 0, hh, col);
        float *o = P.out + i * P.out_pitch + 4 * hh;
        f16v wpre = wn_pre(wk, hh, t2);
        wk = wn_block(P.wn, 1, hh, col);
        auto out_block = [&](int v) {
            const f16v w = wpre;
            if (v + 1 < SPLIT_VB) wpre = wn_pre(wk, hh, t2);
            if (v + 2 < SPLIT_VB) wk = wn_block(P.wn, v + 2, hh, col);
            f4 r[4];
#pragma unroll
            for (int q = 0; q < 4; ++q)
#pragma unroll
                for (int e = 0; e < 4; ++e) r[q][e] = relu1(w[4 * q + e], kinf) * h[4 * v + q][e];
            const f4 t = row_sum16_transpose4(r[0], r[1], r[2], r[3]);
            if (valid && (j & 3) == 0) *reinterpret_cast<f4 *>(o + 32 * v + 8 * (2 * ((j >> 3) & 1) + ((j >> 2) & 1))) = t;
        };
        out_block(0);
        out_block(1);
        float cn[6] = {0.f, 0.f, 0.f, 0.f, 0.f, 0.f};
        f4 q0n = q0, q1n = q1;
        if (more) {
#pragma unroll
            for (int c = 0; c < 3; ++c) { cn[c] = ldc(P.xyz2 + nbn * 3 + c); cn[3 + c] = ldc(P.xyz1 + in_ * 3 + c); }
            q0n = ldc4(P.p1 + in_ * 256 + 4 * hh + 8 * j); q1n = ldc4(P.p1 + in_ * 256 + 4 * hh + 8 * (16 + j));
        }
#pragma unroll
        for (int v = 2; v < SPLIT_VB; ++v) out_block(v);
        pt = ptn; valid = validn; i = in_; nb = nbn; q0 = q0n; q1 = q1n;
        dx = __fsub_rn(cn[0], cn[3]); dy = __fsub_rn(cn[1], cn[4]); dz = __fsub_rn(cn[2], cn[5]);
    }
    ws.finish();
}

struct CvSplitBwdParams {
    CvSplitParams f;
    const float *dout;
    int dout_pitch;
    const float *a3;
    const uint2 *mk1, *mk2;
    float *dz1, *dz2, *dz3, *dq3, *d4, *dp1, *dpd, *dt2, *dbrows;
};

__device__ __forceinline__ f4 leaky_grad_bits4(f4 d, unsigned bits) {
    return (f4){(bits & 1u) ? d.x : 0.1f * d.x, (bits & 2u) ? d.y : 0.1f * d.y, (bits & 4u) ? d.z : 0.1f * d.z, (bits & 8u) ? d.w : 0.1f * d.w};
}

__global__ __launch_bounds__(64 * SP_NW) __attribute__((amdgpu_waves_per_eu(1, 1))) void cost_volume_bwd_split_kernel(const CvSplitBwdParams Q) {
    const float kinf = rtk_hidden_inf();
    __shared__ __attribute__((aligned(16))) f4 s_w[2 * SP_F * 64];
    __shared__ float s_wct[128 * 64];
    const CvSplitParams &P = Q.f;
    const int lane = threadIdx.x & 63, wave = __builtin_amdgcn_readfirstlane(threadIdx.x >> 6), hh = lane >> 5, col = lane & 31, pp = col >> 4,
              j = col & 15;
    const int jq = 2 * ((j >> 3) & 1) + ((j >> 2) & 1);
    for (int e = threadIdx.x; e < 128 * 64; e += 64 * SP_NW) {
        const int l = e & 63, st = e >> 6, o = l & 31, ch = 32 * (st >> 4) + 8 * ((st >> 2) & 3) + 4 * (l >> 5) + (st & 3);
        s_wct[e] = o < 8 ? P.wn.wc[((ch >> 4) * 64 + (o >> 2) * 16 + (ch & 15)) * 4 + (o & 3)] : 0.f;
    }
    int b, bx, nbx;
    rtk_decode_block(P.gx, b, bx, nbx);
    constexpr int PPW = 2 * SP_NW;
    const int groups = (P.n1 + PPW - 1) / PPW;
    WStreamA<SP_NW, SP_F, 2 * SPLIT_NF> ws;
    ws.start_parts(P.blob, s_w, wave, lane);
    const float wi3 = ldc(P.wsc), wi2 = ldc(P.wsc + 1);
    int pt = bx * PPW + 2 * wave + pp;
    bool valid = pt < P.n1;
    long i = (long)b * P.n1 + (valid ? pt : P.n1 - 1);
    float dx = 0.f, dy = 0.f, dz = 0.f;
    if (bx < groups) {
        const long nb = (long)b * P.n2 + (long)P.knn[i * 16 + j];
        dx = __fsub_rn(P.xyz2[nb * 3], P.xyz1[i * 3]); dy = __fsub_rn(P.xyz2[nb * 3 + 1], P.xyz1[i * 3 + 1]);
        dz = __fsub_rn(P.xyz2[nb * 3 + 2], P.xyz1[i * 3 + 2]);
    }
    for (int G = bx; G < groups; G += nbx) {
        asm volatile("" ::: "memory");
        const long pos = i * 16 + j;
        const unsigned ro = (unsigned)pos * 1024u + 16u * hh;
        if (valid && hh == 0) *reinterpret_cast<f4 *>(Q.d4 + pos * 4) = (f4){dx, dy, dz, 1.0f};
        uint2 m2[2] = {Q.mk2[pos * 4 + hh], Q.mk2[pos * 4 + 2 + hh]}, m1[2] = {Q.mk1[pos * 4 + hh], Q.mk1[pos * 4 + 2 + hh]};
        f4 h[32];
#pragma unroll
        for (int e = 0; e < 32; ++e) h[e] = *cv_at(Q.a3, ro + 32u * e);
        float t2[8];
        WnBlock wk = wn_block(P.wn, 0, hh, col);
        const float *dor = Q.dout + i * Q.dout_pitch + 4 * hh;
        const f4 dq0 = ldc4(dor + 8 * j), dq1 = ldc4(dor + 8 * (16 + j));
        wn_hidden(P.wn, dx, dy, dz, t2);
        f16v dt2;
#pragma unroll
        for (int e = 0; e < 16; ++e) dt2[e] = 0.f;
        f16v wpre = wn_pre(wk, hh, t2);
        wk = wn_block(P.wn, 1, hh, col);
        auto block_a = [&](auto vc) {
            constexpr int v = decltype(vc)::value;
            const f16v w = wpre;
            if constexpr (v + 1 < SPLIT_VB) wpre = wn_pre(wk, hh, t2);
            if constexpr (v + 2 < SPLIT_VB) wk = wn_block(P.wn, v + 2, hh, col);
            f4 zs[4];
            auto slot = [&](auto qc) {
                constexpr int q = decltype(qc)::value, e = 4 * v + q;
                const f4 a = h[e];
                f4 wv;
#pragma unroll
                for (int r = 0; r < 4; ++r) wv[r] = relu1(w[4 * q + r], kinf);
                const f4 da = mul_row_bcast<e & 15>(e < 16 ? dq0 : dq1, a);
                const f4 t = mul_row_bcast<e & 15>(e < 16 ? dq0 : dq1, wv);
                f4 qq, z;
#pragma unroll
                for (int r = 0; r < 4; ++r) {
                    qq[r] = wv[r] > 0.f ? da[r] : 0.f;
                    z[r] = a[r] > 0.f ? t[r] : 0.1f * t[r];
                    dt2 = mfma_f32x2(s_wct[(16 * v + 4 * q + r) * 64 + lane], qq[r], dt2);
                }
                h[e] = z;
                zs[q] = z;
                if (valid) *cv_at(Q.dq3, ro + 32u * e) = qq;
            };
            slot(std::integral_constant<int, 0>{}); slot(std::integral_constant<int, 1>{});
            slot(std::integral_constant<int, 2>{}); slot(std::integral_constant<int, 3>{});
            if (Q.dbrows) {
                const f4 r = row_sum16_transpose4(zs[0], zs[1], zs[2], zs[3]);
                if (valid && (j & 3) == 0) *reinterpret_cast<f4 *>(Q.dbrows + i * 512 + 32 * v + 8 * jq + 4 * hh) = r;
            }
        };
        block_a(std::integral_constant<int, 0>{}); block_a(std::integral_constant<int, 1>{}); block_a(std::integral_constant<int, 2>{});
        block_a(std::integral_constant<int, 3>{}); block_a(std::integral_constant<int, 4>{}); block_a(std::integral_constant<int, 5>{});
        block_a(std::integral_constant<int, 6>{}); block_a(std::integral_constant<int, 7>{});
        if (valid) *reinterpret_cast<f4 *>(Q.dt2 + pos * 8 + 4 * hh) = (f4){dt2[0], dt2[1], dt2[2], dt2[3]};
        f16v acc[SPLIT_VB];
        LaneScale sc = lane_scale32(h);
        if (P.amax) tensor_amax_update(P.amax, sc.mb);
        split_layer<0>(ws, h, sc.s, acc, StoreRowsSide{Q.dz3, ro, valid});
        float c = sc.inv * wi3;
#pragma unroll
        for (int v = 0; v < SPLIT_VB; ++v) {
#pragma unroll
            for (int q = 0; q < 4; ++q) h[4 * v + q] = leaky_grad_bits4(acc_slot(acc, 4 * v + q) * c, split_mask_bits(m2, v, q));
            if (Q.dbrows) {
                const f4 r = row_sum16_transpose4(h[4 * v], h[4 * v + 1], h[4 * v + 2], h[4 * v + 3]);
                if (valid && (j & 3) == 0) *reinterpret_cast<f4 *>(Q.dbrows + i * 512 + 256 + 32 * v + 8 * jq + 4 * hh) = r;
            }
        }
        sc = lane_scale32(h);
        if (P.amax) tensor_amax_update(P.amax + 1, sc.mb);
        split_layer<SPLIT_NF>(ws, h, sc.s, acc, StoreRowsSide{Q.dz2, ro, valid});
        ws.sync();
        c = sc.inv * wi2;
        const int Gn = G + nbx;
        const bool more = Gn < groups;
        const int ptn = Gn * PPW + 2 * wave + pp;
        const bool validn = ptn < P.n1;
        const long in_ = (long)b * P.n1 + (validn ? ptn : P.n1 - 1);
        long knn_next = 0;
        if (more) knn_next = (long)P.knn[in_ * 16 + j];
        float dxn = 0.f, dyn = 0.f, dzn = 0.f;
        float *dpr = Q.dp1 + i * 256 + 4 * hh;
        float *dpd = Q.dpd + i * 768 + 4 * hh;
#pragma unroll
        for (int v = 0; v < SPLIT_VB; ++v) {
            if (v == 2 && more) {
                const long nbn = (long)b * P.n2 + knn_next;
                dxn = __fsub_rn(P.xyz2[nbn * 3], P.xyz1[in_ * 3]); dyn = __fsub_rn(P.xyz2[nbn * 3 + 1], P.xyz1[in_ * 3 + 1]);
                dzn = __fsub_rn(P.xyz2[nbn * 3 + 2], P.xyz1[in_ * 3 + 2]);
            }
            f4 r[4];
#pragma unroll
            for (int q = 0; q < 4; ++q) {
                r[q] = leaky_grad_bits4(acc_slot(acc, 4 * v + q) * c, split_mask_bits(m1, v, q));
                if (valid) *cv_at(Q.dz1, ro + 32u * (4 * v + q)) = r[q];
            }
            const f4 s0 = row_sum16_transpose4(r[0], r[1], r[2], r[3]);
            const f4 sx = row_sum16_transpose4(r[0] * dx, r[1] * dx, r[2] * dx, r[3] * dx);
            const f4 sy = row_sum16_transpose4(r[0] * dy, r[1] * dy, r[2] * dy, r[3] * dy);
            const f4 sz = row_sum16_transpose4(r[0] * dz, r[1] * dz, r[2] * dz, r[3] * dz);
            if (valid && (j & 3) == 0) {
                *reinterpret_cast<f4 *>(dpr + 32 * v + 8 * jq) = s0;
                *reinterpret_cast<f4 *>(dpd + 32 * v + 8 * jq) = sx;
                *reinterpret_cast<f4 *>(dpd + 256 + 32 * v + 8 * jq) = sy;
                *reinterpret_cast<f4 *>(dpd + 512 + 32 * v + 8 * jq) = sz;
            }
        }
        pt = ptn; valid = validn; i = in_; dx = dxn; dy = dyn; dz = dzn;
    }
    ws.finish();
}

struct SaSplitParams {
    int samples, n, npoint, gx;
    const float *xyz, *new_xyz;
    const int *idx;
    const float *q;
    int q_pitch;
    const float *w1;
    const f4 *image;
    const float *wsc;
    const float *bias2;
    float *out;
    int out_pitch, out_offset;
    const int *src_nuniq, *dst_nuniq;
};

#ifndef SA_SPLIT_WAVES
#define SA_SPLIT_WAVES 5
#endif
#ifndef SA_WGS_TARGET
#define SA_WGS_TARGET 1024
#endif
template <int NS, int C1>
__global__ __launch_bounds__(256, SA_SPLIT_WAVES) void sa_scale_split_kernel(const SaSplitParams P) {
    constexpr int KS = C1 / 16, VB1 = C1 / 32, NFR = KS * 2 * 2, CPT = 32 / NS;
    const float kinf = rtk_hidden_inf();
    __shared__ __attribute__((aligned(16))) f4 s_img[NFR * 64];
    const int lane = threadIdx.x & 63, hh = lane >> 5, col = lane & 31, pp = col / NS, slot = col % NS;
    int b, bx, nbx;
    rtk_decode_block(P.gx, b, bx, nbx);
    const int dst_e = P.dst_nuniq ? __builtin_amdgcn_readfirstlane(P.dst_nuniq[b]) : P.npoint;
    const int live_c = min(dst_e, P.npoint);
    const int live_units = (live_c + CPT - 1) / CPT;
    if (bx * 4 >= live_units) return;
    for (int i = threadIdx.x; i < NFR * 64; i += blockDim.x) s_img[i] = P.image[i];
    __syncthreads();
    const int src_e = P.src_nuniq ? P.src_nuniq[b] : 0x7fffffff;
    const float winv = ldc(P.wsc);
    for (int unit = bx * 4 + (threadIdx.x >> 6); unit < live_units; unit += nbx * 4) {
        int cl = unit * CPT + pp;
        const bool valid = cl < live_c;
        if (!valid) cl = live_c - 1;
        const int c = b * P.npoint + cl;
        const int id = P.idx[(long)c * NS + slot];
        const long src = (long)b * P.n + id;
        const float dx = __fsub_rn(P.xyz[src * 3], P.new_xyz[(long)c * 3]), dy = __fsub_rn(P.xyz[src * 3 + 1], P.new_xyz[(long)c * 3 + 1]),
                    dz = __fsub_rn(P.xyz[src * 3 + 2], P.new_xyz[(long)c * 3 + 2]);
        const float *qrow = P.q + ((long)b * P.n + (id < src_e ? id : 0)) * P.q_pitch + 4 * hh;
        const float b0 = hh ? dy : dx, b1 = hh ? 1.0f : dz;
        f4 h[4 * VB1];
#pragma unroll
        for (int v = 0; v < VB1; ++v) {
            f16v a;
#pragma unroll
            for (int q = 0; q < 4; ++q) {
                const f4 t = *reinterpret_cast<const f4 *>(qrow + 32 * v + 8 * q);
                a[4 * q] = t.x; a[4 * q + 1] = t.y; a[4 * q + 2] = t.z; a[4 * q + 3] = t.w;
            }
            const int ch = 32 * v + col;
            const float *wr = P.w1 + (ch >> 4) * 64 + (ch & 15);
            a = mfma_f32x2(wr[16 * hh], b0, a);
            a = mfma_f32x2(wr[16 * (2 + hh)], b1, a);
#pragma unroll
            for (int q = 0; q < 4; ++q) h[4 * v + q] = relu_med4((f4){a[4 * q], a[4 * q + 1], a[4 * q + 2], a[4 * q + 3]}, kinf);
        }
        const LaneScale sc = lane_scale32(h);
        const float cs = sc.inv * winv;
        f16v acc[2];
#pragma unroll
        for (int v = 0; v < 2; ++v)
#pragma unroll
            for (int e = 0; e < 16; ++e) acc[v][e] = 0.f;
#pragma unroll
        for (int s = 0; s < KS; ++s) {
            u4v bp[2];
            split2(h[2 * s], h[2 * s + 1], sc.s, bp);
            u4v fr[2][2];
#pragma unroll
            for (int v = 0; v < 2; ++v)
#pragma unroll
                for (int p = 0; p < 2; ++p) fr[v][p] = __builtin_bit_cast(u4v, s_img[((s * 2 + v) * 2 + p) * 64 + lane]);
#define RTK_SA_MM(pa, pb) acc[0] = mfma_h(fr[0][pa], bp[pb], acc[0]); acc[1] = mfma_h(fr[1][pa], bp[pb], acc[1]);
            RTK_SA_MM(1, 0) RTK_SA_MM(0, 1) RTK_SA_MM(0, 0)
#undef RTK_SA_MM
        }
        f4 m[2][4];
#pragma unroll
        for (int v = 0; v < 2; ++v)
#pragma unroll
            for (int q = 0; q < 4; ++q)
                m[v][q] = scale_bias4((f4){acc[v][4 * q], acc[v][4 * q + 1], acc[v][4 * q + 2], acc[v][4 * q + 3]}, cs,
                                      *reinterpret_cast<const f4 *>(P.bias2 + 32 * v + 8 * q + 4 * hh));
        const int qo = 2 * ((col >> 3) & 1) + ((col >> 2) & 1);
        float *o = P.out + (long)c * P.out_pitch + P.out_offset + 4 * hh + 8 * qo;
        if constexpr (NS == 32) {
            f4 t[4];
#pragma unroll
            for (int q = 0; q < 4; ++q) t[q] = wave_max_pair16(m[0][q], m[1][q], kinf);
            const f4 r = relu_med4(row_max16_transpose4(t[0], t[1], t[2], t[3]), kinf);
            if (valid && (col & 3) == 0) *reinterpret_cast<f4 *>(o + 32 * ((col >> 4) & 1)) = r;
        } else {
#pragma unroll
            for (int v = 0; v < 2; ++v) {
                const f4 r = relu_med4(row_max16_transpose4(m[v][0], m[v][1], m[v][2], m[v][3]), kinf);
                if (valid && (col & 3) == 0) *reinterpret_cast<f4 *>(o + 32 * v) = r;
            }
        }
    }
}

}

extern "C" int rtk_pack_split_layer(int cout, int cin, const float *w, int transposed, void *image, float *inv_scale, rtk_stream_t stream) {
    RTK_REQUIRE(cout > 0 && cin > 0 && cout % 32 == 0 && cin % 32 == 0 && w && image && inv_scale, "pack_split_layer: bad arguments");
    RTK_REQUIRE((long)cout * cin <= (1L << 22), "pack_split_layer: more than 2^22 weights (every workgroup scans the matrix for its scale)");
    const int slots = (cin / 16) * (cout / 32) * 64;
    pack_split_kernel<<<(slots + 255) / 256, 256, 0, (hipStream_t)stream>>>(cout, cin, w, transposed, (u4v *)image, inv_scale);
    RTK_CHECK_LAUNCH("pack_split_layer");
    return RTK_OK;
}

extern "C" int rtk_split_mlp2(int positions, const float *x, const void *images, const float *image_scales, const float *bias1,
                              const float *bias2, float *y, rtk_stream_t stream) {
    RTK_REQUIRE(positions > 0 && x && images && image_scales && bias1 && bias2 && y, "split_mlp2: bad arguments");
    const int tiles = (positions + 32 * SP_NW - 1) / (32 * SP_NW);
    split_mlp2_kernel<<<tiles < 256 ? tiles : 256, 64 * SP_NW, 0, (hipStream_t)stream>>>(positions, x, (const f4 *)images, image_scales, bias1, bias2, y);
    RTK_CHECK_LAUNCH("split_mlp2");
    return RTK_OK;
}

static int cv_split_fill(const char *who, CvSplitParams &P, int samples, int n1, int n2, const float *xyz1, const float *xyz2,
                         const int64_t *knn_idx, const void *split_images, const float *image_scales, const rtk_layer_t *wn, dim3 &grid) {
    RTK_REQUIRE(samples > 0 && samples <= 65535 && n1 > 0 && n2 >= 16 && xyz1 && xyz2 && knn_idx && split_images && image_scales,
                "%s: bad arguments", who);
    RTK_REQUIRE(wn && wn[0].w_packed && wn[1].w_packed && wn[2].w_packed && wn[1].bias && wn[2].bias && wn[1].cin16 == 1 &&
                wn[1].cout16 == 1 && wn[2].cin16 == 1 && wn[2].cout16 == 16, "%s: bad WeightNet layers", who);
    P.samples = samples; P.n1 = n1; P.n2 = n2;
    P.xyz1 = xyz1; P.xyz2 = xyz2; P.knn = knn_idx;
    P.blob = reinterpret_cast<const f4 *>(split_images);
    P.wsc = image_scales;
    P.wn.wa = wn[0].w_packed; P.wn.wb = wn[1].w_packed; P.wn.wc = wn[2].w_packed; P.wn.bb = wn[1].bias; P.wn.bc = wn[2].bias;
    P.p1 = P.p2 = P.wd = P.bias2 = P.bias3 = nullptr;
    P.out = nullptr; P.out_pitch = 0; P.sv1 = P.sv2 = P.sv3 = nullptr; P.mk1 = P.mk2 = nullptr; P.amax = nullptr;
    const int groups = (n1 + 2 * SP_NW - 1) / (2 * SP_NW);
    int gx = 256 / samples;
    if (gx < 1) gx = 1;
    if (gx > groups) gx = groups;
    P.gx = samples % 8 == 0 ? gx : 0;
    grid = P.gx ? dim3(gx * samples) : dim3(gx, samples);
    return RTK_OK;
}

static int cu_count() {
    int dev = 0, n = 0;
    if (hipGetDevice(&dev) != hipSuccess || hipDeviceGetAttribute(&n, hipDeviceAttributeMultiprocessorCount, dev) != hipSuccess || n < 8) return 256;
    return n;
}

static int cv_split_forward(const char *who, int samples, int n1, int n2, const float *xyz1, const float *xyz2, const int64_t *knn_idx,
                            const float *p1, const float *p2, const float *wd_packed, const void *split_images, const float *image_scales,
                            const float *bias2, const float *bias3, const rtk_layer_t *wn, float *out, int out_pitch, float *a1, float *a2,
                            float *a3, void *mask1, void *mask2, float *amax, int workgroups, rtk_stream_t stream) {
    CvSplitParams P;
    dim3 grid;
    if (cv_split_fill(who, P, samples, n1, n2, xyz1, xyz2, knn_idx, split_images, image_scales, wn, grid) != RTK_OK) return RTK_ERR_INVALID;
    RTK_REQUIRE(p1 && p2 && wd_packed && bias2 && bias3 && out, "%s: bad arguments", who);
    RTK_REQUIRE((double)samples * n2 <= 4194304.0, "%s: more than 2^22 rows in p2 (32-bit byte offsets of the row requests): split the batch", who);
    RTK_REQUIRE(out_pitch % 4 == 0 && out_pitch >= 256, "%s: bad out_pitch", who);
    const bool save = a1 != nullptr;
    RTK_REQUIRE(!save || ((double)samples * n1 * 16.0 * 1024.0 < 4294967296.0), "%s: more than 4 GiB per saved activation (32-bit row "
                "offsets): split the batch", who);
    P.p1 = p1; P.p2 = p2; P.wd = wd_packed; P.bias2 = bias2; P.bias3 = bias3; P.out = out; P.out_pitch = out_pitch;
    P.sv1 = a1; P.sv2 = a2; P.sv3 = a3; P.mk1 = (uint2 *)mask1; P.mk2 = (uint2 *)mask2; P.amax = amax;
    if (samples % 8 == 0) {
        const int tiles_x = (samples / 8) * ((n1 + 2 * SP_NW - 1) / (2 * SP_NW));
        int per_xcd = (workgroups > 0 ? workgroups : cu_count()) / 8;
        if (per_xcd < 1) per_xcd = 1;
        if (per_xcd > tiles_x) per_xcd = tiles_x;
        P.gx = 8 * per_xcd;
        grid = dim3(P.gx);
    }
    if (save) cost_volume_split_kernel<true><<<grid, 64 * SP_NW, 0, (hipStream_t)stream>>>(P);
    else cost_volume_split_kernel<false><<<grid, 64 * SP_NW, 0, (hipStream_t)stream>>>(P);
    RTK_CHECK_LAUNCH(who);
    return RTK_OK;
}

extern "C" int rtk_cost_volume_split(int samples, int n1, int n2, const float *xyz1, const float *xyz2, const int64_t *knn_idx,
                                     const float *p1, const float *p2, const float *wd_packed, const void *split_images,
                                     const float *image_scales, const float *bias2, const float *bias3, const rtk_layer_t *wn, float *out,
                                     int out_pitch, rtk_stream_t stream) {
    return cv_split_forward("cost_volume_split", samples, n1, n2, xyz1, xyz2, knn_idx, p1, p2, wd_packed, split_images, image_scales, bias2, bias3,
                            wn, out, out_pitch, nullptr, nullptr, nullptr, nullptr, nullptr, nullptr, 0, stream);
}

extern "C" int rtk_cost_volume_split_shared(int samples, int n1, int n2, const float *xyz1, const float *xyz2, const int64_t *knn_idx,
                                            const float *p1, const float *p2, const float *wd_packed, const void *split_images,
                                            const float *image_scales, const float *bias2, const float *bias3, const rtk_layer_t *wn,
                                            float *out, int out_pitch, int workgroups, rtk_stream_t stream) {
    RTK_REQUIRE(workgroups >= 0, "cost_volume_split_shared: workgroups = %d", workgroups);
    return cv_split_forward("cost_volume_split_shared", samples, n1, n2, xyz1, xyz2, knn_idx, p1, p2, wd_packed, split_images, image_scales,
                            bias2, bias3, wn, out, out_pitch, nullptr, nullptr, nullptr, nullptr, nullptr, nullptr, workgroups, stream);
}

extern "C" int rtk_cost_volume_split_train(int samples, int n1, int n2, const float *xyz1, const float *xyz2, const int64_t *knn_idx,
                                           const float *p1, const float *p2, const float *wd_packed, const void *split_images,
                                           const float *image_scales, const float *bias2, const float *bias3, const rtk_layer_t *wn,
                                           float *out, int out_pitch, float *a1, float *a2, float *a3, void *mask1, void *mask2,
                                           float *act_amax, rtk_stream_t stream) {
    RTK_REQUIRE(a1 && a2 && a3 && mask1 && mask2, "cost_volume_split_train: null activation buffer");
    return cv_split_forward("cost_volume_split_train", samples, n1, n2, xyz1, xyz2, knn_idx, p1, p2, wd_packed, split_images, image_scales,
                            bias2, bias3, wn, out, out_pitch, a1, a2, a3, mask1, mask2, act_amax, 0, stream);
}

extern "C" int rtk_cost_volume_bwd_split(int samples, int n1, int n2, const float *xyz1, const float *xyz2, const int64_t *knn_idx,
                                         const void *split_images_t, const float *image_scales_t, const rtk_layer_t *wn, const float *dout,
                                         int dout_pitch,
                                         const float *a3, const void *mask1, const void *mask2, float *dz1, float *dz2, float *dz3,
                                         float *dq3, float *d4, float *dp1, float *dpd, float *dt2, float *dbias_rows,
                                         float *dz_amax, rtk_stream_t stream) {
    CvSplitBwdParams Q;
    dim3 grid;
    if (cv_split_fill("cost_volume_bwd_split", Q.f, samples, n1, n2, xyz1, xyz2, knn_idx, split_images_t, image_scales_t, wn, grid) != RTK_OK)
        return RTK_ERR_INVALID;
    RTK_REQUIRE(dout && mask1 && mask2 && a3 && dz1 && dz2 && dz3 && dq3 && d4 && dp1 && dpd && dt2, "cost_volume_bwd_split: bad arguments");
    RTK_REQUIRE((double)samples * n1 * 16.0 * 1024.0 < 4294967296.0, "cost_volume_bwd_split: more than 4 GiB per (position, 256) tensor "
                "(32-bit row offsets): split the batch");
    RTK_REQUIRE(dout_pitch % 4 == 0 && dout_pitch >= 256, "cost_volume_bwd_split: bad dout_pitch");
    Q.dout = dout; Q.dout_pitch = dout_pitch; Q.a3 = a3; Q.mk1 = (const uint2 *)mask1; Q.mk2 = (const uint2 *)mask2;
    Q.dz1 = dz1; Q.dz2 = dz2; Q.dz3 = dz3; Q.dq3 = dq3; Q.d4 = d4; Q.dp1 = dp1; Q.dpd = dpd; Q.dt2 = dt2; Q.dbrows = dbias_rows;
    Q.f.amax = dz_amax;
    cost_volume_bwd_split_kernel<<<grid, 64 * SP_NW, 0, (hipStream_t)stream>>>(Q);
    RTK_CHECK_LAUNCH("cost_volume_bwd_split");
    return RTK_OK;
}

extern "C" int rtk_sa_scale_split(int samples, int n, int npoint, int nsample, const float *xyz, const float *new_xyz, const int *idx,
                                  const float *q, int q_pitch, int c1, const float *w1xyz_packed, const void *split_image,
                                  const float *image_scale, const float *bias2, float *out, int out_pitch, int out_offset,
                                  const int *src_nuniq, const int *dst_nuniq, rtk_stream_t stream) {
    RTK_REQUIRE(samples > 0 && n > 0 && npoint > 0 && xyz && new_xyz && idx && q && w1xyz_packed && split_image && image_scale && bias2 && out,
                "sa_scale_split: bad arguments");
    RTK_REQUIRE(q_pitch % 4 == 0 && out_pitch % 4 == 0 && out_offset % 4 == 0, "sa_scale_split: pitches/offset must be multiples of 4");
    RTK_REQUIRE((long)samples * npoint * nsample < 0x7fffffffL && (long)samples * n < 0x7fffffffL && samples <= 65535,
                "sa_scale_split: problem too large for 32-bit indexing");
    SaSplitParams P;
    P.samples = samples; P.n = n; P.npoint = npoint;
    P.xyz = xyz; P.new_xyz = new_xyz; P.idx = idx; P.q = q; P.q_pitch = q_pitch; P.w1 = w1xyz_packed;
    P.image = reinterpret_cast<const f4 *>(split_image); P.wsc = image_scale; P.bias2 = bias2;
    P.out = out; P.out_pitch = out_pitch; P.out_offset = out_offset; P.src_nuniq = src_nuniq; P.dst_nuniq = dst_nuniq;
    const int units = (npoint + 32 / nsample - 1) / (32 / nsample);
    int bx = (units + 3) / 4;
    while ((long)bx * samples > SA_WGS_TARGET && bx > 1) bx = (bx + 1) / 2;
    P.gx = samples % 8 == 0 ? bx : 0;
    const dim3 blocks = P.gx ? dim3(bx * samples) : dim3(bx, samples);
    hipStream_t s = (hipStream_t)stream;
    if (nsample == 32 && c1 == 64) sa_scale_split_kernel<32, 64><<<blocks, 256, 0, s>>>(P);
    else if (nsample == 16 && c1 == 64) sa_scale_split_kernel<16, 64><<<blocks, 256, 0, s>>>(P);
    else if (nsample == 16 && c1 == 32) sa_scale_split_kernel<16, 32><<<blocks, 256, 0, s>>>(P);
    else {
        rtk_set_error("sa_scale_split: no kernel instance for nsample=%d, %d -> 64 channels", nsample, c1);
        return RTK_ERR_UNSUPPORTED;
    }
    RTK_CHECK_LAUNCH("sa_scale_split");
    return RTK_OK;
}
```

ratrack_amd/fused.py:

```python
import ctypes
import os

import torch

from . import _lib
from . import pointnet2_hip as _native

ACT_NONE, ACT_RELU, ACT_LEAKY, ACT_SIGMOID = 0, 1, 2, 3


class _Src(ctypes.Structure):
    _fields_ = [("ptr", ctypes.c_void_p), ("pitch", ctypes.c_int), ("channels", ctypes.c_int), ("per_sample", ctypes.c_int)]


class _Layer(ctypes.Structure):
    _fields_ = [("w_packed", ctypes.c_void_p), ("bias", ctypes.c_void_p), ("cin16", ctypes.c_int), ("cout16", ctypes.c_int),
                ("act", ctypes.c_int), ("inv_scale", ctypes.c_float)]


class _Interp(ctypes.Structure):
    _fields_ = [("known_feats", ctypes.c_void_p), ("pitch", ctypes.c_int), ("channels", ctypes.c_int), ("m", ctypes.c_int),
                ("idx", ctypes.c_void_p), ("dist2", ctypes.c_void_p), ("nuniq", ctypes.c_void_p)]


_vp, _ci = ctypes.c_void_p, ctypes.c_int
_lib.SIGNATURES.update({
    "rtk_pointwise_mlp": [_ci, _ci, ctypes.POINTER(_Interp), _ci, ctypes.POINTER(_Src), _vp, _ci, ctypes.POINTER(_Layer), _vp,
                          _ci, _ci, _ci, _vp, _vp, _vp],
    "rtk_sa_scale": [_ci] * 4 + [_vp] * 4 + [_ci, _ci, _vp, _ci, ctypes.POINTER(_Layer), _vp, _ci, _ci, _vp, _vp, _vp],
    "rtk_cost_volume": [_ci] * 3 + [_vp] * 6 + [ctypes.POINTER(_Layer), ctypes.POINTER(_Layer), _vp, _ci, _vp],
    "rtk_patch_cost": [_ci] * 2 + [_vp] * 3 + [_ci, ctypes.POINTER(_Layer), _vp, _ci, _ci, _vp],
    "rtk_pack_split_layer": [_ci, _ci, _vp, _ci, _vp, _vp, _vp],
    "rtk_cost_volume_split": [_ci] * 3 + [_vp] * 10 + [ctypes.POINTER(_Layer), _vp, _ci, _vp],
    "rtk_cost_volume_split_shared": [_ci] * 3 + [_vp] * 10 + [ctypes.POINTER(_Layer), _vp, _ci, _ci, _vp],
    "rtk_split_mlp2": [_ci, _vp, _vp, _vp, _vp, _vp, _vp, _vp],
    "rtk_sa_scale_split": [_ci] * 4 + [_vp] * 4 + [_ci, _ci, _vp, _vp, _vp, _vp, _vp, _ci, _ci, _vp, _vp, _vp],
    "rtk_prepare_inputs": [_ci] * 2 + [_vp] * 6 + [_vp],
    "rtk_fps_centroids": [_ci] * 3 + [_vp] * 8 + [_vp],
    "rtk_knn_point_masked": [_ci] * 4 + [_vp] * 4 + [_vp],
    "rtk_fps_relevel": [_ci] * 3 + [_vp] * 9 + [_ci, _vp, _vp],
    "rtk_gru_step": [_ci] * 3 + [_vp] * 8 + [_vp],
    "rtk_to_channel_major": [_ci] * 3 + [_vp, _ci, _ci, _vp, _ci, _ci, _vp],
    "rtk_ball_query_pair": [_ci] * 3 + [ctypes.c_float, _ci, ctypes.c_float, _ci] + [_vp] * 5 + [_vp],
    "rtk_geometry_front": [_ci] * 4 + [_vp, _vp, _ci] + [_vp] * 13 + [_vp, _vp, _ci, _vp],
    "rtk_geometry_tables": [_ci] * 3 + [_vp] * 3 + [ctypes.POINTER(ctypes.c_float), ctypes.POINTER(_ci), ctypes.POINTER(_vp), ctypes.POINTER(_vp),
                            ctypes.POINTER(_vp), _vp],
    "rtk_three_nn_masked": [_ci] * 3 + [_vp] * 6 + [_vp],
    "rtk_to_channel_major_multi": [_ci] * 3 + [_vp, _vp],
    "rtk_log_sinkhorn": [_ci, _ci, _vp, ctypes.c_float, _ci, _vp, _vp],
    "rtk_dbscan": [_ci, _vp, _ci, _vp, _vp, ctypes.c_float, ctypes.c_double, _ci, _vp, _vp],
    "rtk_dbscan_batched": [_vp, ctypes.c_float, ctypes.c_double, _ci, _ci, _vp, _vp, _vp, _vp, _vp, ctypes.c_longlong, _vp],
    "rtk_object_descriptors": [_vp, _ci, _vp, _vp, _vp, _vp, _vp, _vp],
    "rtk_affinity_pairs": [_ci, _ci] + [_vp] * 7 + [_vp],
    "rtk_associate_batched": [_ci] * 3 + [_vp] * 7 + [ctypes.c_float, _ci] + [_vp] * 9 + [_vp],
    "rtk_track_max_objects": [],
})


class _GtJob(ctypes.Structure):
    _fields_ = [("wt", ctypes.c_void_p), ("bias", ctypes.c_void_p), ("out", ctypes.c_void_p), ("cout", ctypes.c_int), ("s0", ctypes.c_int),
                ("count", ctypes.c_int), ("out_pitch", ctypes.c_int)]


class _CopyJob(ctypes.Structure):
    _fields_ = [("src", ctypes.c_void_p), ("dst", ctypes.c_void_p), ("bytes", ctypes.c_long)]


_lib.SIGNATURES.update({
    "rtk_gru_step_head": [_ci] * 3 + [_vp] * 11 + [_ci, _vp],
    "rtk_global_terms": [_ci, _ci, _vp, _ci, ctypes.POINTER(_GtJob), _vp, _ci, _ci, _vp],
    "rtk_copy_multi": [_ci, ctypes.POINTER(_CopyJob), _vp],
})


def copy_multi(pairs):
    for i in range(0, len(pairs), 8):
        part = pairs[i:i + 8]
        jobs = (_CopyJob * len(part))()
        for j, (d, s_) in enumerate(part):
            assert d.is_contiguous() and s_.is_contiguous() and d.shape == s_.shape and d.dtype == s_.dtype and d.device == s_.device
            jobs[j].src, jobs[j].dst, jobs[j].bytes = s_.data_ptr(), d.data_ptr(), d.numel() * d.element_size()
        _lib.call("rtk_copy_multi", len(part), jobs, _stream())


class _LayoutJob(ctypes.Structure):
    _fields_ = [("src", ctypes.c_void_p), ("dst", ctypes.c_void_p), ("channels", ctypes.c_int), ("src_pitch", ctypes.c_int),
                ("per_sample", ctypes.c_int), ("dst_channels", ctypes.c_int), ("dst_channel_offset", ctypes.c_int)]


def _stream():
    return torch.cuda.current_stream().cuda_stream


def ceil16(c):
    return (c + 15) // 16 * 16


_TRACE = None


class trace_work:
    def __enter__(self):
        global _TRACE
        _TRACE = self.records = []
        return self

    def __exit__(self, *a):
        global _TRACE
        _TRACE = None
        return False

    def executed_macs(self):
        per = {}
        for kind, rows, macs_per_row in self.records:
            r = float(rows.sum().item()) if torch.is_tensor(rows) else float(rows)
            per[kind] = per.get(kind, 0.0) + r * macs_per_row
        return sum(per.values()), per


def _live_rows(nuniq, rows_per_sample, samples):
    if nuniq is None:
        return samples * rows_per_sample
    return torch.clamp(nuniq[:samples].to(torch.int64), max=rows_per_sample)



def fold_bn(w, bn_prefix, sd, eps=1e-5):
    g, b = sd[bn_prefix + ".weight"].double(), sd[bn_prefix + ".bias"].double()
    m, v = sd[bn_prefix + ".running_mean"].double(), sd[bn_prefix + ".running_var"].double()
    s = g / torch.sqrt(v + eps)
    w = w.double().reshape(w.shape[0], -1)
    return (w * s[:, None]), (b - s * m)


def pack_layer(w):
    cout, cin = w.shape
    V, U = ceil16(cout) // 16, ceil16(cin) // 16
    if cout % 16 == 0 and cin % 16 == 0:
        wp = w.float()
    else:
        wp = torch.zeros(V * 16, U * 16, dtype=torch.float32, device=w.device)
        wp[:cout, :cin] = w.float()
    return wp.reshape(V, 16, U, 4, 4).permute(2, 0, 3, 1, 4).contiguous().reshape(-1)


SPLIT_IMAGE_256 = 2 * 256 * 256


def split3_bf16(w):
    x = w.float().contiguous()
    out = []
    for _ in range(3):
        top = (x.view(torch.int32) & -65536)
        out.append((top >> 16).to(torch.int16))
        x = x - top.view(torch.float32)
    return torch.stack(out)


def pow2_scale(amax):
    e = (torch.as_tensor(amax, dtype=torch.float32).reshape(1).view(torch.int32).item() >> 23) & 0xff
    sf = min(268 - e, 253)
    return 2.0 ** (sf - 127), 2.0 ** (127 - sf)


def split2_f16(w, scale):
    x = w.float().contiguous() * scale
    h = x.half()
    l = (x - h.float()).half()
    return torch.stack([h.view(torch.int16), l.view(torch.int16)])


def pack_layer_split(w):
    cout, cin = w.shape
    assert cout % 32 == 0 and cin % 32 == 0
    scale, inv = pow2_scale(w.float().abs().max())
    p = split2_f16(w, scale)
    p = p.reshape(2, cout // 32, 32, cin // 32, 2, 2, 2, 4)
    return p.permute(3, 4, 1, 0, 6, 2, 5, 7).contiguous().reshape(-1), inv


def pack_split_device(w, transposed=False):
    cout, cin = (w.shape[1], w.shape[0]) if transposed else w.shape
    image = torch.empty(2 * cout * cin, dtype=torch.int16, device=w.device)
    inv = torch.empty(1, dtype=torch.float32, device=w.device)
    _lib.call("rtk_pack_split_layer", cout, cin, w.data_ptr(), 1 if transposed else 0, image.data_ptr(), inv.data_ptr(), _stream())
    return image, inv


def pack_layer_split16(w):
    cout, cin = w.shape
    V, U2 = ceil16(cout) // 16, (ceil16(cin) // 16 + 1) // 2
    wp = torch.zeros(V * 16, U2 * 32, dtype=torch.float32, device=w.device)
    wp[:cout, :cin] = w.float()
    scale, inv = pow2_scale(wp.abs().max())
    p = split2_f16(wp, scale).reshape(2, V, 16, U2, 2, 4, 4)
    return p.permute(3, 1, 0, 5, 2, 4, 6).contiguous().reshape(-1), inv


PW_SPLIT = True
LAYER_SPLIT = 0x100


def pad_bias(b, cout):
    out = torch.zeros(ceil16(cout), dtype=torch.float32, device=b.device)
    out[:b.numel()] = b.float()
    return out


class Chain:

    def split_arr(self):
        if self._split is None:
            packed = [pack_layer_split16(w.to(self._device)) for w, _ in self._layers]
            blob = torch.cat([im for im, _ in packed]).contiguous()
            arr = (_Layer * len(self._layers))()
            off = boff = 0
            for i, (w, act) in enumerate(self._layers):
                cout, cin = w.shape
                u, v = ceil16(cin) // 16, ceil16(cout) // 16
                arr[i].w_packed = blob.data_ptr() + 2 * off
                arr[i].bias = self.bias.data_ptr() + 4 * boff
                arr[i].cin16, arr[i].cout16, arr[i].act, arr[i].inv_scale = u, v, act | LAYER_SPLIT, packed[i][1]
                off += ((u + 1) // 2) * v * 2 * 512
                boff += v * 16
            self._split = (arr, blob)
        return self._split[0]

    def __init__(self, layers, device):
        packs, biases, meta = [], [], []
        self.dims = [tuple(w.shape) for w, _, _ in layers]
        for w, b, act in layers:
            cout, cin = w.shape
            packs.append(pack_layer(w.to(device)))
            biases.append(pad_bias(b.to(device), cout))
            meta.append((ceil16(cin) // 16, ceil16(cout) // 16, act))
        self.blob = torch.cat(packs).contiguous()
        self.bias = torch.cat(biases).contiguous()
        self._layers, self._device, self._split = [(w, act) for w, _, act in layers], device, None
        arr = (_Layer * len(layers))()
        woff = boff = 0
        for i, (u, v, act) in enumerate(meta):
            arr[i].w_packed = self.blob.data_ptr() + 4 * woff
            arr[i].bias = self.bias.data_ptr() + 4 * boff
            arr[i].cin16, arr[i].cout16, arr[i].act = u, v, act
            woff += u * v * 256
            boff += v * 16
        self.arr = arr
        self.n = len(layers)
        self.cout = layers[-1][0].shape[0]
        self.cout16 = meta[-1][1]


def _colptr(t, col=0):
    assert t.dim() == 2 and t.stride(1) == 1 and t.dtype == torch.float32
    return t.data_ptr() + 4 * col, t.stride(0)


def pointwise(rows, rows_per_sample, srcs, chain, out, out_channels=None, sample_bias=None, interp=None, channel_major=False,
              row_nuniq=None, colmax=None):
    arr = (_Src * max(len(srcs), 1))()
    for i, (t, ch, per) in enumerate(srcs):
        ptr, pitch = _colptr(t)
        arr[i].ptr, arr[i].pitch, arr[i].channels, arr[i].per_sample = ptr, pitch, ch, int(per)
    ip = None
    if interp is not None:
        kf, ch, m, idx, d2 = interp[:5]
        nu = interp[5] if len(interp) > 5 else None
        ptr, pitch = _colptr(kf)
        ip = ctypes.pointer(_Interp(ptr, pitch, ch, m, idx.data_ptr(), d2.data_ptr(), nu.data_ptr() if nu is not None else None))
    oc = out_channels if out_channels is not None else chain.cout
    if _TRACE is not None:
        macs = sum(co * ci for co, ci in chain.dims) + (3 * interp[1] if interp is not None else 0)
        _TRACE.append(("pointwise", _live_rows(row_nuniq, rows_per_sample, rows // rows_per_sample), macs))
    if channel_major:
        optr, opitch = out.data_ptr(), 0
    else:
        optr, opitch = _colptr(out)
    _lib.call("rtk_pointwise_mlp", rows, rows_per_sample, ip, len(srcs), arr,
              sample_bias.data_ptr() if sample_bias is not None else None, chain.n, chain.split_arr() if PW_SPLIT else chain.arr, optr, opitch, oc,
              int(channel_major), row_nuniq.data_ptr() if row_nuniq is not None else None,
              colmax.data_ptr() if colmax is not None else None, _stream())
    return out


pointwise_mlp = pointwise


def offset_image(w4, device):
    cout = w4.shape[0]
    V = ceil16(cout) // 16
    wp = torch.zeros(V * 16, 4, dtype=torch.float32, device=device)
    wp[:cout] = w4.float().to(device)
    return wp.reshape(V, 16, 4).permute(0, 2, 1).contiguous().reshape(-1)


class _WeightNet:

    def __init__(self, sd, prefix, device):
        g = lambda k: sd[prefix + k].double()
        wa, ba = g(".mlp_convs.0.weight").reshape(8, 3), g(".mlp_convs.0.bias")
        wb, bb = g(".mlp_convs.1.weight").reshape(8, 8), g(".mlp_convs.1.bias")
        wc, bc = g(".mlp_convs.2.weight").reshape(-1, 8), g(".mlp_convs.2.bias")
        self.wa = offset_image(torch.cat([wa, ba[:, None]], 1), device)
        self.wb, self.bb = pack_layer(wb.to(device)), pad_bias(bb.to(device), 8)
        self.wc, self.bc = pack_layer(wc.to(device)), pad_bias(bc.to(device), wc.shape[0])
        arr = (_Layer * 3)()
        arr[0].w_packed, arr[0].cin16, arr[0].cout16 = self.wa.data_ptr(), 1, 1
        arr[1].w_packed, arr[1].bias, arr[1].cin16, arr[1].cout16 = self.wb.data_ptr(), self.bb.data_ptr(), 1, 1
        arr[2].w_packed, arr[2].bias, arr[2].cin16, arr[2].cout16 = self.wc.data_ptr(), self.bc.data_ptr(), 1, ceil16(wc.shape[0]) // 16
        self.arr = arr


SA_SPLIT = True


class _SAScale:

    def __init__(self, sd, prefix, nsample, radius, device):
        self.nsample, self.radius = nsample, float(radius)
        ws = []
        i = 0
        while (prefix + ".layer%d.conv.weight" % i) in sd:
            ws.append(fold_bn(sd[prefix + ".layer%d.conv.weight" % i], prefix + ".layer%d.bn.bn" % i, sd))
            i += 1
        w1, b1 = ws[0]
        self.c1 = w1.shape[0]
        self.wf = w1[:, 3:]
        self.w1img = offset_image(torch.cat([w1[:, :3], b1[:, None]], 1), device)
        self.chain = Chain([(w, b, ACT_RELU) for w, b in ws[1:]], device)
        self.cout = ws[-1][0].shape[0]
        self.split_image = None
        if SA_SPLIT and len(ws) == 2 and self.cout == 64 and self.c1 in (32, 64) and nsample in (16, 32) and torch.device(device).type == "cuda":
            w2 = ws[1][0].float().to(device).contiguous()
            self.split_bias = ws[1][1].float().to(device).contiguous()
            self.split_image, self.split_scale = pack_split_device(w2)
            torch.cuda.current_stream().synchronize()


class _PNHeadWeights:

    RADII = [[2, 4], [4, 8], [8, 16]]
    NSAMPLES = [[4, 8], [8, 16], [16, 32]]

    def __init__(self, sd, prefix, device):
        d = lambda k: sd[prefix + k].double()
        self.scales = [[_SAScale(sd, "%ssa%d.mlps.%d" % (prefix, l + 1, s), self.NSAMPLES[l][s], self.RADII[l][s], device)
                        for s in range(2)] for l in range(3)]
        self.wq1 = torch.cat([self.scales[0][0].wf, self.scales[0][1].wf], 0)
        self.trans = []
        for l in (1, 2):
            wl, bl = d("linear%d.weight" % l), d("linear%d.bias" % l)
            rows, bias = [wl], [bl]
            for s in range(2):
                wf = self.scales[l][s].wf
                rows.append(wf @ wl)
                bias.append(wf @ bl)
            self.trans.append(Chain([(torch.cat(rows, 0), torch.cat(bias, 0), ACT_NONE)], device))
        self.lin3 = Chain([(d("linear3.weight"), d("linear3.bias"), ACT_NONE)], device)
        self.fp = {}
        for name in ("fp3", "fp2", "fp1"):
            w, b = fold_bn(sd[prefix + name + ".mlp.layer0.conv.weight"], prefix + name + ".mlp.layer0.bn.bn", sd)
            self.fp[name] = Chain([(w, b, ACT_RELU)], device)


FUSED_GEOMETRY = True
GEOMETRY_POISON = None
CHECK_FPS_RELEVEL = False


def check_fps_relevel(xyz1, idx, new_xyz, nuniq):
    S_, npoint, _ = xyz1.shape
    src = xyz1
    for l in range(idx.shape[0]):
        i = torch.empty(S_, npoint, dtype=torch.int32, device=src.device)
        out = torch.empty(S_, npoint, 3, dtype=torch.float32, device=src.device)
        cnt = torch.empty(S_, dtype=torch.int32, device=src.device)
        _lib.call("rtk_fps_centroids", S_, npoint, npoint, src.data_ptr(), i.data_ptr(), out.data_ptr(), cnt.data_ptr(), None, None, None, None,
                  _stream())
        assert torch.equal(i, idx[l].view(S_, npoint)), "fps_relevel: level %d indices differ from the full selection" % (l + 2)
        assert torch.equal(out, new_xyz[l].view(S_, npoint, 3)), "fps_relevel: level %d centroids differ" % (l + 2)
        assert torch.equal(cnt, nuniq[l].view(-1)), "fps_relevel: level %d exhausted-cloud counters differ" % (l + 2)
        src = out


class _NullCtx:
    def __enter__(self):
        return self

    def __exit__(self, *a):
        return False


class Geometry:

    def __init__(self, xyz, npoint, side=None, knn_frames=0, finite=False, n_valid=None, level_hook=None, tail_hook=None, zeros=None,
                 prepare=None, q1=None):
        zeros_given = zeros
        zeros = zeros or (lambda n_, dtype, device: torch.zeros(n_, dtype=dtype, device=device))
        S_, n, _ = xyz.shape
        if n_valid is not None:
            assert n_valid.shape == (S_,) and n_valid.dtype == torch.int32 and n_valid.is_contiguous() and n <= 2048
        nv = n_valid.data_ptr() if n_valid is not None else None
        dev = xyz.device
        self.n, self.samples, self.npoint = n, S_, npoint
        self.xyz = [xyz]
        self.nuniq = []
        self.events = {}
        ns_all = [ns for row in _PNHeadWeights.NSAMPLES for ns in row]
        nn_rows = [npoint, npoint, n]
        sizes = [S_ * npoint] * 3 + [S_] * 7 + [S_ * npoint * ns for ns in ns_all] + [S_ * r * 3 for r in nn_rows]
        fused_geo = (FUSED_GEOMETRY and n <= 2048 and npoint <= 512 and max(n, npoint) * 12 <= 64 * 1024 and
                     (not knn_frames or (n >= 16 and S_ == 2 * knn_frames)) and (prepare is None or S_ % 2 == 0))
        if fused_geo and zeros_given is None and not finite:
            ws = torch.empty(sum(sizes), dtype=torch.int32, device=dev)
            if GEOMETRY_POISON is not None:
                ws.fill_(GEOMETRY_POISON)
        else:
            ws = zeros(sum(sizes), torch.int32, dev)
        parts = list(torch.split(ws, sizes))
        fps_idx, cnt, tie, tie23, first_tie, ball, nn_idx = parts[0:3], parts[3:6], parts[6], parts[7:9], parts[9], parts[10:16], parts[16:19]
        snap = torch.empty(S_ * n, dtype=torch.float32, device=dev) if n <= 2048 else None
        self.fps_idx = [t.view(S_, npoint) for t in fps_idx]
        self.tie = tie
        xyz_all = torch.empty(3, S_, npoint, 3, dtype=torch.float32, device=dev)
        new_xyz = [xyz_all[l] for l in range(3)]
        d2_all = zeros(sum(nn_rows) * S_ * 3, torch.float32, dev) if finite else torch.empty(sum(nn_rows) * S_ * 3, dtype=torch.float32, device=dev)
        d2_parts = torch.split(d2_all, [S_ * r * 3 for r in nn_rows])
        B = knn_frames
        self.knn = [torch.empty(B, n, 16, dtype=torch.int64, device=dev) for _ in range(2)] if B else None
        big = n > 2048
        temp = torch.full((S_, n), 1e10, dtype=torch.float32, device=dev) if big else None
        self._scratch = (snap, temp, n_valid, xyz)

        self.fused_geometry = fused_geo
        self.q1_done = False
        q1w = q1 is not None and prepare is not None
        if prepare is not None and not fused_geo:
            pc1, pc2, f1, f2, raw = prepare
# ... 20 lines not shown
                _lib.call("rtk_geometry_front", b1, S_, n, npoint, *fr, fps_idx[0].data_ptr(), xyz_all.data_ptr(), cnt[0].data_ptr(),
                          tie.data_ptr(), first_tie.data_ptr(), snap.data_ptr(), nv, self.knn[0].data_ptr() if B else None,
                          self.knn[1].data_ptr() if B else None, q1[0].data_ptr() if q1w else None, q1[1].data_ptr() if q1w else None,
                          q1[1].shape[1] if q1w else 0, _stream())
                self.q1_done = q1w
                self._record("front", side)
                if CHECK_FPS_RELEVEL and not torch.cuda.is_current_stream_capturing():
                    check_fps_relevel(new_xyz[0], torch.stack(self.fps_idx[1:]), xyz_all[1:], torch.stack(list(cnt[1:3])))
                radii = (ctypes.c_float * 6)(*[float(r) for row in _PNHeadWeights.RADII for r in row])
                nsam = (_ci * 6)(*ns_all)
                balls = (_vp * 6)(*[t.data_ptr() for t in ball])
                self.nn = {}
                for i, (name, (u, k)) in enumerate({"fp3": (2, 3), "fp2": (1, 2), "fp1": (0, 1)}.items()):
                    self.nn[name] = (d2_parts[i].view(S_, nn_rows[i], 3), nn_idx[i].view(S_, nn_rows[i], 3), self.xyz[k].shape[1])
                nni = (_vp * 3)(*[self.nn[k][1].data_ptr() for k in ("fp3", "fp2", "fp1")])
                nnd = (_vp * 3)(*[self.nn[k][0].data_ptr() for k in ("fp3", "fp2", "fp1")])
                _lib.call("rtk_geometry_tables", S_, n, npoint, xyz.data_ptr(), xyz_all.data_ptr(), cnt[0].data_ptr(), radii, nsam, balls, nni, nnd,
                          _stream())
                for lvl in range(3):
                    if level_hook is not None:
                        level_hook(self, lvl)
                    self._record(lvl, side)
                self._record("nn", side)
                if B:
                    self.events["knn"] = self.events.get("front")
                if tail_hook is not None:
                    tail_hook(self)
            return
        with ctx:
            if not big:
                _lib.call("rtk_fps_centroids", S_, n, npoint, xyz.data_ptr(), fps_idx[0].data_ptr(), new_xyz[0].data_ptr(),
                          cnt[0].data_ptr(), tie.data_ptr(), nv, snap.data_ptr(), first_tie.data_ptr(), _stream())
            else:
                _native.furthest_point_sampling_wrapper(S_, n, npoint, xyz, temp, self.fps_idx[0])
                new_xyz[0].copy_(torch.gather(xyz, 1, self.fps_idx[0].long().unsqueeze(-1).expand(-1, -1, 3)))
                cnt[0].fill_(npoint)
                tie.fill_(npoint)

            def relevel():
                resume = (fps_idx[0].data_ptr(), snap.data_ptr(), n, first_tie.data_ptr()) if not big else (None, None, 0, None)
                _lib.call("rtk_fps_relevel", S_, npoint, 2, new_xyz[0].data_ptr(), cnt[0].data_ptr(), tie.data_ptr(),
                          fps_idx[1].data_ptr(), new_xyz[1].data_ptr(), cnt[1].data_ptr(), tie23[0].data_ptr(), *resume, _stream())
                if CHECK_FPS_RELEVEL and not torch.cuda.is_current_stream_capturing():
                    check_fps_relevel(new_xyz[0], torch.stack(self.fps_idx[1:]), xyz_all[1:], torch.stack(list(cnt[1:3])))
            for lvl in range(3):
                self.xyz.append(new_xyz[lvl])
                self.nuniq.append(cnt[lvl])
            self.ball = []
            for lvl in range(3):
                row = []
                for s in range(2):
                    ns, r = _PNHeadWeights.NSAMPLES[lvl][s], _PNHeadWeights.RADII[lvl][s]
                    bidx = ball[lvl * 2 + s].view(S_, npoint, ns)
                    row.append(bidx)
                self.ball.append(row)
            for lvl in range(3):
                (r1, r2), (n1, n2) = _PNHeadWeights.RADII[lvl], _PNHeadWeights.NSAMPLES[lvl]
                nsrc = self.xyz[lvl].shape[1]
                if nsrc * 12 <= 64 * 1024:
                    _lib.call("rtk_ball_query_pair", S_, nsrc, npoint, float(r1), n1, float(r2), n2, self.xyz[lvl + 1].data_ptr(),
                              self.xyz[lvl].data_ptr(), self.ball[lvl][0].data_ptr(), self.ball[lvl][1].data_ptr(),
                              self.nuniq[lvl].data_ptr(), _stream())
                else:
                    for s in range(2):
                        _native.ball_query_wrapper(S_, nsrc, npoint, float(_PNHeadWeights.RADII[lvl][s]), _PNHeadWeights.NSAMPLES[lvl][s],
                                                   self.xyz[lvl + 1], self.xyz[lvl], self.ball[lvl][s])
                if level_hook is not None:
                    level_hook(self, lvl)
                self._record(lvl, side)
                if lvl == 0:
                    relevel()
            self.nn = {}
            for i, (name, (u, k)) in enumerate({"fp3": (2, 3), "fp2": (1, 2), "fp1": (0, 1)}.items()):
                nu, m = self.xyz[u].shape[1], self.xyz[k].shape[1]
                d2 = d2_parts[i].view(S_, nu, 3)
                idx = nn_idx[i].view(S_, nu, 3)
                mask = self.nuniq[u - 1].data_ptr() if u > 0 else None
                _lib.call("rtk_three_nn_masked", S_, nu, m, self.xyz[u].data_ptr(), self.xyz[k].data_ptr(), d2.data_ptr(), idx.data_ptr(),
                          mask, self.nuniq[k - 1].data_ptr(), _stream())
                self.nn[name] = (d2, idx, m)
            self._record("nn", side)
            if B:
                x1, x2 = xyz[:B], xyz[B:]
                if n_valid is None:
                    _native.knn_point_wrapper(B, n, n, 16, x1, x2, self.knn[0])
                    _native.knn_point_wrapper(B, n, n, 16, x1, x1, self.knn[1])
                else:
                    _lib.call("rtk_knn_point_masked", B, n, n, 16, x1.data_ptr(), x2.data_ptr(), self.knn[0].data_ptr(),
                              n_valid[B:].data_ptr(), _stream())
                    _lib.call("rtk_knn_point_masked", B, n, n, 16, x1.data_ptr(), x1.data_ptr(), self.knn[1].data_ptr(),
                              n_valid[:B].data_ptr(), _stream())
                self._record("knn", side)
            if tail_hook is not None:
                tail_hook(self)

    def _record(self, key, side):
        if side is not None:
            ev = torch.cuda.Event()
            ev.record(side)
            self.events[key] = ev

    def wait(self, key):
        ev = self.events.get(key)
        if ev is not None:
            torch.cuda.current_stream().wait_event(ev)

    def head(self, count):
        g = object.__new__(Geometry)
        g.n, g.samples, g.npoint = self.n, count, self.npoint
        g.xyz = [x[:count] for x in self.xyz]
        g.ball = [[b[:count] for b in row] for row in self.ball]
        g.nuniq = [c[:count] for c in self.nuniq]
        g.fps_idx, g.tie = [i[:count] for i in self.fps_idx], self.tie[:count]
        g.events, g.knn = self.events, self.knn
        g.nn = {k: (d2[:count], idx[:count], m) for k, (d2, idx, m) in self.nn.items()}
        return g


CV_SPLIT_MAX_ROWS = 1 << 22


def cv_shared_workgroups(samples, n1, dev):
    cus = torch.cuda.get_device_properties(dev).multi_processor_count
    if samples % 8 or cus % 8:
        return 0
    tiles = (samples // 8) * ((n1 + 7) // 8)
    lo, hi = max(1, cus // 16), max(1, cus // 8 * 3 // 4)
    balance = lambda w: tiles / (w * -(-tiles // w))
    ok = [w for w in range(hi, lo - 1, -1) if balance(w) >= 0.95]
    w = ok[0] if ok else max(range(lo, hi + 1), key=balance)
    return 8 * min(w, tiles)


def sa_scale(geo, W, lvl, s, q, qcol, out, out_offset):
    sc = W.scales[lvl][s]
    qptr, qpitch = _colptr(q, qcol)
    optr, opitch = _colptr(out)
    src, dst = geo.xyz[lvl], geo.xyz[lvl + 1]
    src_nu = geo.nuniq[lvl - 1].data_ptr() if lvl > 0 else None
    if _TRACE is not None:
        macs = sc.nsample * (4 * sc.c1 + sum(co * ci for co, ci in sc.chain.dims))
        _TRACE.append(("sa_scale", _live_rows(geo.nuniq[lvl], geo.npoint, geo.samples), macs))
    if sc.split_image is not None:
        _lib.call("rtk_sa_scale_split", geo.samples, src.shape[1], geo.npoint, sc.nsample, src.data_ptr(), dst.data_ptr(),
                  geo.ball[lvl][s].data_ptr(), qptr, qpitch, sc.c1, sc.w1img.data_ptr(), sc.split_image.data_ptr(), sc.split_scale.data_ptr(),
                  sc.split_bias.data_ptr(),
                  optr, opitch, out_offset, src_nu, geo.nuniq[lvl].data_ptr(), _stream())
        return
    _lib.call("rtk_sa_scale", geo.samples, src.shape[1], geo.npoint, sc.nsample, src.data_ptr(), dst.data_ptr(),
              geo.ball[lvl][s].data_ptr(), qptr, qpitch, ceil16(sc.c1) // 16, sc.w1img.data_ptr(),
              sc.chain.n, sc.chain.arr, optr, opitch, out_offset, src_nu, geo.nuniq[lvl].data_ptr(), _stream())


def run_pnhead(W, geo, q1, out=None, gmax=None):
    S_, n, S = geo.samples, geo.n, geo.npoint
    dev = q1.device
    new = lambda rows, c: torch.empty(rows, c, dtype=torch.float32, device=dev)
    nu = geo.nuniq
    sa1 = new(S_ * S, 64)
    geo.wait(0)
    sa_scale(geo, W, 0, 0, q1, 0, sa1, 0)
    sa_scale(geo, W, 0, 1, q1, 16, sa1, 32)
    t1 = pointwise(S_ * S, S, [(sa1, 64, False)], W.trans[0], new(S_ * S, 96), row_nuniq=nu[0])
    sa2 = new(S_ * S, 96)
    geo.wait(1)
    sa_scale(geo, W, 1, 0, t1, 32, sa2, 0)
    sa_scale(geo, W, 1, 1, t1, 64, sa2, 32)
    t2 = pointwise(S_ * S, S, [(sa2, 96, False)], W.trans[1], new(S_ * S, 192), row_nuniq=nu[1])
    sa3 = new(S_ * S, 128)
    geo.wait(2)
    sa_scale(geo, W, 2, 0, t2, 64, sa3, 0)
    sa_scale(geo, W, 2, 1, t2, 128, sa3, 64)
    l3 = pointwise(S_ * S, S, [(sa3, 128, False)], W.lin3, new(S_ * S, 64), row_nuniq=nu[2])
    geo.wait("nn")
    d2, idx, m = geo.nn["fp3"]
    f3 = pointwise(S_ * S, S, [(t2[:, 0:64], 64, False)], W.fp["fp3"], new(S_ * S, 128), row_nuniq=nu[1],
                   interp=(l3, 64, m, idx.reshape(-1, 3), d2.reshape(-1, 3), nu[2]))
    d2, idx, m = geo.nn["fp2"]
    f2 = pointwise(S_ * S, S, [(t1[:, 0:32], 32, False)], W.fp["fp2"], new(S_ * S, 128), row_nuniq=nu[0],
                   interp=(f3, 128, m, idx.reshape(-1, 3), d2.reshape(-1, 3), nu[1]))
    d2, idx, m = geo.nn["fp1"]
    if gmax is None:
        gmax = torch.zeros(S_, 128, dtype=torch.float32, device=dev)
    out = pointwise(S_ * n, n, [], W.fp["fp1"], out if out is not None else new(S_ * n, 128),
                    interp=(f2, 128, m, idx.reshape(-1, 3), d2.reshape(-1, 3), nu[0]), colmax=gmax)
    return out, gmax


class FusedBackbone:

    def __init__(self, model, split=True):
        sd = {k: v.detach() for k, v in model.state_dict().items()}
        dev = next(model.parameters()).device
        self.dev = dev
        self.npoint = model.pn_head.sa1.npoint
        g = lambda k: torch.stack([sd["fd_layer.torchGRU.%s_l%d" % (k, l)].float() for l in range(5)])
        self.gru_wih = g("weight_ih").transpose(1, 2).contiguous()
        self.gru_whh = g("weight_hh").transpose(1, 2).contiguous()
        self.gru_bih, self.gru_bhh = g("bias_ih").contiguous(), g("bias_hh").contiguous()
        self.kernel_events = None
        self.kernel_token = None
        self._split_hook = None
        self.side, self.use_side_stream = None, True
        self.cv_shared = False
        self._last_cv = None
        self.enc = _PNHeadWeights(sd, "pn_head.", dev)
        self.dec = _PNHeadWeights(sd, "fd_layer.mse.", dev)
        z = lambda n: torch.zeros(n, dtype=torch.float64, device=sd["bin_score"].device)
        self.enc_q1 = Chain([(self.enc.wq1, z(32), ACT_NONE)], dev)
        self.enc_q1_w = self.enc.wq1.float().to(dev).contiguous()
        w0 = sd["fc_layer.mlp_convs.0.weight"].double().reshape(256, 515)
        b0 = sd["fc_layer.mlp_convs.0.bias"].double()
        self.p1_loc = Chain([(w0[:, 0:128], z(256), ACT_NONE)], dev)
        self.p2_loc = Chain([(w0[:, 256:384], z(256), ACT_NONE)], dev)
        tr = lambda w: w.float().t().contiguous().to(dev)
        self.p1_glob_wt, self.p1_glob_b = tr(w0[:, 128:256]), b0.float().to(dev).contiguous()
        self.p2_glob_wt = tr(w0[:, 384:512])
        self.cv_wd = offset_image(torch.cat([w0[:, 512:515], z(256)[:, None]], 1), dev)
        self.cv_layers = Chain([(sd["fc_layer.mlp_convs.%d.weight" % i].double().reshape(256, 256),
                                 sd["fc_layer.mlp_convs.%d.bias" % i].double(), ACT_LEAKY) for i in (1, 2)], dev)
        self.cv_split = bool(split)
        w23 = [sd["fc_layer.mlp_convs.%d.weight" % i].double().reshape(256, 256).float().to(dev).contiguous() for i in (1, 2)]
        self.cv_bias23 = torch.stack([sd["fc_layer.mlp_convs.%d.bias" % i].double().float() for i in (1, 2)]).to(dev).contiguous()
        self.cv_images = torch.empty(2 * SPLIT_IMAGE_256, dtype=torch.int16, device=dev)
        self.cv_scales = torch.empty(2, dtype=torch.float32, device=dev)
        for l, w in enumerate(w23):
            _lib.call("rtk_pack_split_layer", 256, 256, w.data_ptr(), 0, self.cv_images[l * SPLIT_IMAGE_256:].data_ptr(),
                      self.cv_scales[l:].data_ptr(), _stream())
        torch.cuda.current_stream().synchronize()
        self.wn1 = _WeightNet(sd, "fc_layer.weightnet1", dev)
        self.wn2 = _WeightNet(sd, "fc_layer.weightnet2", dev)
        def predictor(prefix, first_cols):
            layers = []
            for i in range(3):
                w, b = fold_bn(sd["%s.sf_mlp.%d.0.weight" % (prefix, i)], "%s.sf_mlp.%d.1" % (prefix, i), sd)
                layers.append([w, b, ACT_RELU])
            return layers
        cp = predictor("fd_layer.cp", None)
        wl, bl = sd["fd_layer.cp.linear.weight"].double(), sd["fd_layer.cp.linear.bias"].double()
        wc2 = sd["fd_layer.cp.conv2.weight"].double().reshape(3, 32)
        cp.append([wl @ wc2, bl, ACT_SIGMOID])
        self.cls_head = Chain([tuple(x) for x in cp], dev)
        fp = predictor("fd_layer.fp", None)
        w_first = fp[0][0]
        self.flow_glob_wt, self.flow_glob_b = tr(w_first[:, 128:256]), fp[0][1].float().to(dev).contiguous()
        fp[0] = [w_first[:, 0:128], z(128), ACT_RELU]
        fp.append([sd["fd_layer.fp.conv2.weight"].double().reshape(3, 32), z(3), ACT_NONE])
        self.flow_head = Chain([tuple(x) for x in fp], dev)
        wq = self.dec.wq1
        wq_pad = torch.zeros(32, 16, dtype=torch.float64, device=wq.device)
        wq_pad[:, :2] = wq[:, 0:2]
        self.dec_q1 = Chain([(torch.cat([wq_pad, wq[:, 2:130], wq[:, 258:514]], 1), z(32), ACT_NONE)], dev)
        self.dec_q1_glob_wt = tr(wq[:, 130:258])

    def backbone(self, pc1, pc2, feature1, feature2, h, n_valid=None):
        B, _, N = pc1.shape
        dev = pc1.device
        new = lambda rows, c: torch.empty(rows, c, dtype=torch.float32, device=dev)
        xyz = torch.empty(2 * B, N, 3, dtype=torch.float32, device=dev)
        raw = new(2 * B * N, 4)
        q1 = new(2 * B * N, 32)
        ins = [t.contiguous() for t in (pc1, pc2, feature1, feature2)]
        if self.side is None and self.use_side_stream:
            self.side = torch.cuda.Stream(device=dev)
        if n_valid is not None:
            n_valid = n_valid.to(device=dev, dtype=torch.int32).reshape(2 * B).contiguous()
        geo = Geometry(xyz, self.npoint, side=self.side if self.use_side_stream else None, knn_frames=B, n_valid=n_valid,
                       prepare=(ins[0], ins[1], ins[2], ins[3], raw), q1=(self.enc_q1_w, q1))
        geo.wait("front")
        if not geo.q1_done:
            pointwise(2 * B * N, N, [(raw, 2, False)], self.enc_q1, q1)
        elif _TRACE is not None:
            _TRACE.append(("pointwise", 2 * B * N, 64))
        feat12 = new(2 * B * N, 256)
        gmax = torch.zeros(3 * B, 128, dtype=torch.float32, device=dev)
        loc, glob = run_pnhead(self.enc, geo, q1, out=feat12[:, 0:128], gmax=gmax[:2 * B])
        f1, f2 = loc[:B * N], loc[B * N:]
        sb1, sb2, sbq = new(B, 256), new(B, 256), new(B, 32)
        global_terms(glob, [(self.p1_glob_wt, self.p1_glob_b, sb1, 0), (self.p2_glob_wt, None, sb2, B), (self.dec_q1_glob_wt, None, sbq, 0)],
                     bcast=feat12[:, 128:], n=N)
        p1 = pointwise(B * N, N, [(f1, 128, False)], self.p1_loc, new(B * N, 256), sample_bias=sb1)
        p2 = pointwise(B * N, N, [(f2, 128, False)], self.p2_loc, new(B * N, 256), sample_bias=sb2)
        x1, x2 = xyz[:B], xyz[B:]
        geo.wait("knn")
        knn1, knn2 = geo.knn
        cor1 = new(B * N, 256)
        self._last_cv = (B, N, x1, x2, knn1, p1, p2, cor1)
        if self._split_hook is not None:
            geo.events.clear()
            self._split_hook()
        else:
            ev = self.kernel_events
            if ev is not None:
                e0, e1 = torch.cuda.Event(enable_timing=True), torch.cuda.Event(enable_timing=True)
                e0.record()
            self._cost_volume(*self._last_cv)
            if ev is not None:
                e1.record()
                ev.append((e0, e1))
        cor = new(B * N, 256)
        if _TRACE is not None:
            _TRACE.append(("patch_cost", B * N * 16, (3 * 8 + 8 * 8 + 8 * 256) + 256))
        _lib.call("rtk_patch_cost", B, N, x1.data_ptr(), knn2.data_ptr(), cor1.data_ptr(), 256, self.wn2.arr, cor.data_ptr(), 256, 0,
                  _stream())
        cls = torch.empty(B, N, dtype=torch.float32, device=dev)
        pointwise(B * N, N, [(cor, 256, False)], self.cls_head, cls, out_channels=1, channel_major=True)
        q1d = pointwise(B * N, N, [(raw[:B * N], 2, False), (f1, 128, False), (cor, 256, False)], self.dec_q1, new(B * N, 32),
                        sample_bias=sbq)
        prop, gfeat = run_pnhead(self.dec, geo.head(B), q1d, gmax=gmax[2 * B:])
        if h is None:
            h = torch.zeros(5, B, 128, device=dev, dtype=torch.float32)
        gout, h_out, sbf = self._gru_step(gfeat, h)
        flow = torch.empty(B, 3, N, dtype=torch.float32, device=dev)
        pointwise(B * N, N, [(prop, 128, False)], self.flow_head, flow, out_channels=3, sample_bias=sbf, channel_major=True)
        f12 = feat12.view(2 * B, N, 256).permute(0, 2, 1)
        pc1_features, pc2_features = f12[:B], f12[B:]
        cor_cm = cor.view(B, N, 256).permute(0, 2, 1)
        prop_cm = prop.view(B, N, 128).permute(0, 2, 1)
        return flow, h_out, cls, cor_cm, pc1_features, pc2_features, prop_cm

    def _cost_volume(self, B, N, x1, x2, knn1, p1, p2, cor1):
        if _TRACE is not None:
            _TRACE.append(("cost_volume", B * N * 16, 3 * 256 + 2 * 256 * 256 + (3 * 8 + 8 * 8 + 8 * 256) + 256))
        if self.cv_split:
            step = B if B * N <= CV_SPLIT_MAX_ROWS else max(1, CV_SPLIT_MAX_ROWS // N)
            for b0 in range(0, B, step):
                nb = min(step, B - b0)
                wgs = cv_shared_workgroups(nb, N, x1.device) if self.cv_shared else 0
                r0 = b0 * N
                _lib.call("rtk_cost_volume_split_shared", nb, N, N, x1[b0:].data_ptr(), x2[b0:].data_ptr(), knn1[b0:].data_ptr(), p1[r0:].data_ptr(),
                          p2[r0:].data_ptr(), self.cv_wd.data_ptr(), self.cv_images.data_ptr(), self.cv_scales.data_ptr(),
                          self.cv_bias23[0].data_ptr(), self.cv_bias23[1].data_ptr(), self.wn1.arr, cor1[r0:].data_ptr(), 256, wgs, _stream())
            return
        _lib.call("rtk_cost_volume", B, N, N, x1.data_ptr(), x2.data_ptr(), knn1.data_ptr(), p1.data_ptr(), p2.data_ptr(),
                  self.cv_wd.data_ptr(), self.cv_layers.arr, self.wn1.arr, cor1.data_ptr(), 256, _stream())

    def _gru_step(self, x, h):
        L, B, H = h.shape
        if _TRACE is not None:
            _TRACE.append(("gru", B * L, 2 * 3 * H * H))
            _TRACE.append(("global_terms", B, H * self.flow_glob_wt.shape[1]))
        h_out = torch.empty_like(h)
        y = torch.empty(B, H, dtype=torch.float32, device=h.device)
        sbf = torch.empty(B, self.flow_glob_wt.shape[1], dtype=torch.float32, device=h.device)
        h = h.contiguous()
        _lib.call("rtk_gru_step_head", B, L, H, x.data_ptr(), h.data_ptr(), self.gru_wih.data_ptr(), self.gru_whh.data_ptr(),
                  self.gru_bih.data_ptr(), self.gru_bhh.data_ptr(), h_out.data_ptr(), y.data_ptr(), self.flow_glob_wt.data_ptr(),
                  self.flow_glob_b.data_ptr(), sbf.data_ptr(), sbf.shape[1], _stream())
        return y, h_out, sbf

    def time_dominant_kernel(self, iters=20):
        assert self._last_cv is not None, "run backbone() first"
        ev = []
        for _ in range(iters):
            e0, e1 = torch.cuda.Event(enable_timing=True), torch.cuda.Event(enable_timing=True)
            e0.record()
            self._cost_volume(*self._last_cv)
            e1.record()
            ev.append((e0, e1))
        torch.cuda.synchronize()
        return ev

    def capture(self, pc1, pc2, feature1, feature2, h, split_cost_volume=False):
        static = [t.clone() for t in (pc1, pc2, feature1, feature2, h)]
        saved, self.kernel_events = self.kernel_events, None
        side = torch.cuda.Stream()
        side.wait_stream(torch.cuda.current_stream())
        with torch.cuda.stream(side):
            for _ in range(2):
                self.backbone(*static)
        torch.cuda.current_stream().wait_stream(side)
        if not split_cost_volume:
            graph = torch.cuda.CUDAGraph()
            with torch.cuda.graph(graph):
                outs = self.backbone(*static)
            self.kernel_events = saved

            def step(*new_inputs):
                pairs = [(d, s_) for d, s_ in zip(static, new_inputs) if s_ is not None]
                if pairs:
                    _copy_inputs(pairs)
                graph.replay()
                return outs
            step.graph = graph
            return step

        g1, g2 = torch.cuda.CUDAGraph(), torch.cuda.CUDAGraph()
        torch.cuda.synchronize()
        cap = torch.cuda.Stream()
        cap.wait_stream(torch.cuda.current_stream())

        def hook():
            g1.capture_end()
            g2.capture_begin(pool=g1.pool())

        with torch.cuda.stream(cap):
            self._split_hook = hook
            try:
                g1.capture_begin()
                outs = self.backbone(*static)
                g2.capture_end()
            finally:
                self._split_hook = None
        torch.cuda.current_stream().wait_stream(cap)
        cv_args = self._last_cv
        self.kernel_events = saved
        eng = self

        def step(*new_inputs):
            pairs = [(d, s_) for d, s_ in zip(static, new_inputs) if s_ is not None]
            if pairs:
                _copy_inputs(pairs)
            g1.replay()
            ev = eng.kernel_events
            if ev is not None:
                tok = eng.kernel_token
                if tok is not None and tok[0] is not None:
                    torch.cuda.current_stream().wait_event(tok[0])
                e0, e1 = torch.cuda.Event(enable_timing=True), torch.cuda.Event(enable_timing=True)
                e0.record()
            eng._cost_volume(*cv_args)
            if ev is not None:
                e1.record()
                ev.append((e0, e1))
                if tok is not None:
                    tok[0] = e1
            g2.replay()
            return outs
        step.graph = (g1, g2)
        return step


def global_terms(g, jobs, bcast=None, n=0):
    samples, cin = g.shape
    arr = (_GtJob * max(len(jobs), 1))()
    for j, (wt, bias, out, s0) in enumerate(jobs):
        assert wt.shape == (cin, out.shape[1]) and out.is_contiguous() and wt.is_contiguous()
        arr[j].wt, arr[j].bias, arr[j].out = wt.data_ptr(), bias.data_ptr() if bias is not None else None, out.data_ptr()
        arr[j].cout, arr[j].s0, arr[j].count, arr[j].out_pitch = out.shape[1], s0, out.shape[0], out.shape[1]
    if _TRACE is not None:
        _TRACE.append(("global_terms", 1, sum(cin * o.shape[0] * o.shape[1] for _, _, o, _ in jobs)))
    bptr, bpitch = _colptr(bcast) if bcast is not None else (None, 0)
    _lib.call("rtk_global_terms", samples, cin, g.data_ptr(), len(jobs), arr, bptr, bpitch, n, _stream())


def _copy_inputs(pairs):
    if all(d.is_contiguous() and s_.is_contiguous() and d.shape == s_.shape and d.dtype == s_.dtype and d.device == s_.device and
           d.element_size() == 4 for d, s_ in pairs):
        copy_multi(pairs)
    else:
        torch._foreach_copy_([p[0] for p in pairs], [p[1] for p in pairs])


class GraphPipeline:

    def __init__(self, model_or_engine, example_inputs, depth=2, split_cost_volume=False):
        import copy
        eng = model_or_engine if isinstance(model_or_engine, FusedBackbone) else FusedBackbone(model_or_engine)
        if depth > 2:
            eng = copy.copy(eng)
            eng.use_side_stream, eng.side = False, None
            eng.cv_shared = True
        self.engines = [eng]
        for _ in range(depth - 1):
            e = copy.copy(eng)
            e.side, e._last_cv, e.kernel_events = None, None, None
            self.engines.append(e)
        self.depth = depth
        self._token = [None]
        for e in self.engines:
            e.kernel_token = self._token
        with torch.no_grad():
            self.steps = [e.capture(*example_inputs, split_cost_volume=split_cost_volume) for e in self.engines]
        self.streams = [torch.cuda.Stream() for _ in range(depth)]
        self.i = 0
        self._forked = False

    def submit(self, *inputs):
        cur = torch.cuda.current_stream()
        if not self._forked:
            for s in self.streams:
                s.wait_stream(cur)
            self._forked = True
        k = self.i % self.depth
        self.i += 1
        with torch.cuda.stream(self.streams[k]):
            return self.steps[k](*inputs)

    def set_kernel_events(self, events):
        for e in self.engines:
            e.kernel_events = events

    def drain(self):
        cur = torch.cuda.current_stream()
        for s in self.streams:
            cur.wait_stream(s)
        self._forked = False
```

Baseline: 102,700 frame-pairs/s.

## Fuse p1/p2 local projections into fp1 pointwise kernel and fold global terms into cost volume

The fp1 interpolation MLP kernel now also applies the per-frame p1_loc/p2_loc projection to its freshly computed tile, streaming both weight sets through LDS. This removes two separate pointwise launches and the reread of the 128-channel features. The per-sample global bias terms for both frames are summed into one sample_term in global_terms, and a new cost-volume variant adds that term itself. The trade is more work and register pressure in the tap kernel, plus more complex weight streaming.

```diff
diff --git a/include/rtk_fused.h b/include/rtk_fused.h
--- a/include/rtk_fused.h
+++ b/include/rtk_fused.h
@@ -39,6 +39,10 @@
                                  const rtk_layer_t *layers, float *out, int out_pitch, int out_channels,
                                  int out_channel_major, const int *row_nuniq, float *colmax, rtk_stream_t stream);
 
+RTK_EXPORT int rtk_pointwise_mlp_tap(int rows, int rows_per_sample, const rtk_interp_t *interp, const rtk_layer_t *layer, float *out,
+                                     int out_pitch, float *colmax, const rtk_layer_t *proj, int frame_split, float *proj_out,
+                                     int proj_pitch, rtk_stream_t stream);
+
 RTK_EXPORT int rtk_sa_scale(int samples, int n, int npoint, int nsample, const float *xyz,
                             const float *new_xyz, const int *idx, const float *q, int q_pitch, int c1_16,
                             const float *w1xyz_packed, int nlayers, const rtk_layer_t *layers, float *out,
@@ -65,6 +69,11 @@
                                             const void *split_images, const float *image_scales, const float *bias2,
                                             const float *bias3, const rtk_layer_t *wn, float *out, int out_pitch, int workgroups,
                                             rtk_stream_t stream);
+RTK_EXPORT int rtk_cost_volume_split_term(int samples, int n1, int n2, const float *xyz1, const float *xyz2,
+                                          const int64_t *knn_idx, const float *p1, const float *p2, const float *sample_term,
+                                          const float *wd_packed, const void *split_images, const float *image_scales,
+                                          const float *bias2, const float *bias3, const rtk_layer_t *wn, float *out, int out_pitch,
+                                          int workgroups, rtk_stream_t stream);
 RTK_EXPORT int rtk_sa_scale_split(int samples, int n, int npoint, int nsample, const float *xyz, const float *new_xyz,
                                   const int *idx, const float *q, int q_pitch, int c1, const float *w1xyz_packed,
                                   const void *split_image, const float *image_scale, const float *bias2, float *out, int out_pitch,
@@ -98,6 +107,8 @@
     const float *wt, *bias;
     float *out;
     int cout, s0, count, out_pitch;
+    const float *wt2;
+    int s2;
 } rtk_gterm_job_t;
 RTK_EXPORT int rtk_global_terms(int samples, int cin, const float *g, int njobs, const rtk_gterm_job_t *jobs, float *bcast, int bcast_pitch,
                                 int n, rtk_stream_t stream);
diff --git a/ratrack_amd/csrc/fused_common.h b/ratrack_amd/csrc/fused_common.h
--- a/ratrack_amd/csrc/fused_common.h
+++ b/ratrack_amd/csrc/fused_common.h
@@ -287,10 +287,17 @@
         }
     }
     static __device__ __forceinline__ void run(WS &ws, const f4 (&h)[U], float scale, f4 (&acc)[V], f4 (&a)[2][4], u4v (&b)[2]) {
-        constexpr int up = GI / GV, v0 = (GI % GV) * 2;
+        constexpr int up = GI / GV;
         if constexpr (GI + 1 < NG) load<GI + 1>(ws, a[(GI + 1) & 1]);
         if constexpr (GI % GV == 0) split2(h[2 * up], 2 * up + 1 < U ? h[2 * up + 1] : f4_zero(), scale, b);
-        const f4(&c)[4] = a[GI & 1];
+        mm(a[GI & 1], b, acc);
+    }
+    static __device__ __forceinline__ void run_pieces(WS &ws, const u4v (&pc)[(U + 1) / 2][2], f4 (&acc)[V], f4 (&a)[2][4]) {
+        if constexpr (GI + 1 < NG) load<GI + 1>(ws, a[(GI + 1) & 1]);
+        mm(a[GI & 1], pc[GI / GV], acc);
+    }
+    static __device__ __forceinline__ void mm(const f4 (&c)[4], const u4v (&b)[2], f4 (&acc)[V]) {
+        constexpr int v0 = (GI % GV) * 2;
 #define RTK_S16_MM(pa, pb)                                                                            \
         acc[v0] = mfma16_h(__builtin_bit_cast(u4v, c[pa]), b[pb], acc[v0]);                            \
         if constexpr (v0 + 1 < V) acc[v0 + 1] = mfma16_h(__builtin_bit_cast(u4v, c[2 + pa]), b[pb], acc[v0 + 1]);
@@ -306,6 +313,13 @@
     u4v b[2];
     LayerStepS<U, V, FBASE, 0, WS, F>::template load<0>(ws, a[0]);
     (LayerStepS<U, V, FBASE, GI, WS, F>::run(ws, h, scale, acc, a, b), ...);
+}
+
+template <int U, int V, int FBASE, class WS, int F, int... GI>
+__device__ __forceinline__ void mlp_layer_pieces_impl(WS &ws, const u4v (&pc)[(U + 1) / 2][2], f4 (&acc)[V], std::integer_sequence<int, GI...>) {
+    f4 a[2][4];
+    LayerStepS<U, V, FBASE, 0, WS, F>::template load<0>(ws, a[0]);
+    (LayerStepS<U, V, FBASE, GI, WS, F>::run_pieces(ws, pc, acc, a), ...);
 }
 
 template <int U, int V, int FBASE, int NW, int F, int NF>
diff --git a/ratrack_amd/csrc/fused_misc.hip b/ratrack_amd/csrc/fused_misc.hip
--- a/ratrack_amd/csrc/fused_misc.hip
+++ b/ratrack_amd/csrc/fused_misc.hip
@@ -122,28 +122,43 @@
 
 __global__ __launch_bounds__(256) void global_terms_kernel(const GtParams P) {
     __shared__ __attribute__((aligned(16))) float s_g[512];
+    __shared__ float s_g2[RTK_GT_MAX_JOBS][512];
     const int s = blockIdx.x, t = threadIdx.x;
     for (int k = t; k < P.cin; k += 256) s_g[k] = P.g[(long)s * P.cin + k];
+    for (int j = 0; j < P.njobs; ++j)
+        if (P.job[j].wt2 && s >= P.job[j].s0 && s < P.job[j].s0 + P.job[j].count)
+            for (int k = t; k < P.cin; k += 256) s_g2[j][k] = P.g[(long)(s - P.job[j].s0 + P.job[j].s2) * P.cin + k];
     __syncthreads();
     int total = 0;
     for (int j = 0; j < P.njobs; ++j)
-        if (s >= P.job[j].s0 && s < P.job[j].s0 + P.job[j].count) total += P.job[j].cout;
+        if (s >= P.job[j].s0 && s < P.job[j].s0 + P.job[j].count) total = (P.job[j].wt2 ? (total + 1) & ~1 : total) + (P.job[j].wt2 ? 2 : 1) * P.job[j].cout;
     for (int o = blockIdx.y * 256 + t; o < total; o += 256 * gridDim.y) {
-        int c = o, j = 0;
+        int c = -1, j = 0, base = 0;
         for (; j < P.njobs; ++j) {
             if (s < P.job[j].s0 || s >= P.job[j].s0 + P.job[j].count) continue;
-            if (c < P.job[j].cout) break;
-            c -= P.job[j].cout;
-        }
+            if (P.job[j].wt2) base = (base + 1) & ~1;
+            const int span = (P.job[j].wt2 ? 2 : 1) * P.job[j].cout;
+            if (o < base + span) { c = o - base; break; }
+            base += span;
+        }
+        if (c < 0) continue;
         const rtk_gterm_job_t &J = P.job[j];
-        float acc = J.bias ? J.bias[c] : 0.f;
+        const int m = J.wt2 ? (c & 1) : 0;
+        if (J.wt2) c >>= 1;
+        const float *wt = m ? J.wt2 : J.wt, *g = m ? s_g2[j] : s_g;
+        float acc = m == 0 && J.bias ? J.bias[c] : 0.f;
         for (int k0 = 0; k0 < P.cin; k0 += 64) {
             float wv[64];
 #pragma unroll
-            for (int q = 0; q < 64; ++q) wv[q] = J.wt[(long)min(k0 + q, P.cin - 1) * J.cout + c];
+            for (int q = 0; q < 64; ++q) wv[q] = wt[(long)min(k0 + q, P.cin - 1) * J.cout + c];
 #pragma unroll
             for (int q = 0; q < 64; ++q)
-                if (k0 + q < P.cin) acc = fmaf(wv[q], s_g[k0 + q], acc);
+                if (k0 + q < P.cin) acc = fmaf(wv[q], g[k0 + q], acc);
+        }
+        if (J.wt2) {
+            const float other = __shfl_xor(acc, 1);
+            if (m) continue;
+            acc = __fadd_rn(acc, other);
         }
         J.out[(long)(s - J.s0) * J.out_pitch + c] = acc;
     }
@@ -166,7 +181,8 @@
     P.samples = samples; P.cin = cin; P.njobs = njobs; P.n = n; P.bcast_pitch = bcast_pitch; P.g = g; P.bcast = bcast;
     for (int j = 0; j < njobs; ++j) {
         RTK_REQUIRE(jobs[j].wt && jobs[j].out && jobs[j].cout > 0 && jobs[j].s0 >= 0 && jobs[j].count >= 0 && jobs[j].s0 + jobs[j].count <= samples &&
-                    jobs[j].out_pitch >= jobs[j].cout, "global_terms: bad job %d", j);
+                    jobs[j].out_pitch >= jobs[j].cout && (!jobs[j].wt2 || (jobs[j].s2 >= 0 && jobs[j].s2 + jobs[j].count <= samples)),
+                    "global_terms: bad job %d", j);
         P.job[j] = jobs[j];
     }
     global_terms_kernel<<<dim3(samples, bcast ? 8 : 2), 256, 0, (hipStream_t)stream>>>(P);
diff --git a/ratrack_amd/csrc/fused_pointwise.hip b/ratrack_amd/csrc/fused_pointwise.hip
--- a/ratrack_amd/csrc/fused_pointwise.hip
+++ b/ratrack_amd/csrc/fused_pointwise.hip
@@ -95,6 +95,42 @@
             if (c + 1 < P.out_channels) o[(size_t)(c + 1) * n] = acc[v].y;
             if (c + 2 < P.out_channels) o[(size_t)(c + 2) * n] = acc[v].z;
             if (c + 3 < P.out_channels) o[(size_t)(c + 3) * n] = acc[v].w;
+        }
+    }
+}
+
+template <int U>
+__device__ __forceinline__ void load_interp(const PwParams &P, int p, int b, int g, int nslots, f4 (&h)[U]) {
+    const int *idp = P.interp.idx + (size_t)p * 3;
+    int id[3] = {idp[0], idp[1], idp[2]};
+    if (P.interp.nuniq) {
+        const int e = P.interp.nuniq[b];
+        id[0] = id[0] < e ? id[0] : 0; id[1] = id[1] < e ? id[1] : 0; id[2] = id[2] < e ? id[2] : 0;
+    }
+    const float *d2 = P.interp.dist2 + (size_t)p * 3;
+    const float r0 = __fdiv_rn(1.0f, __fadd_rn(__fsqrt_rn(d2[0]), 1e-8f));
+    const float r1 = __fdiv_rn(1.0f, __fadd_rn(__fsqrt_rn(d2[1]), 1e-8f));
+    const float r2 = __fdiv_rn(1.0f, __fadd_rn(__fsqrt_rn(d2[2]), 1e-8f));
+    const float norm = __fadd_rn(__fadd_rn(r0, r1), r2);
+    const float w0 = __fdiv_rn(r0, norm), w1 = __fdiv_rn(r1, norm), w2 = __fdiv_rn(r2, norm);
+    const float *k0 = P.interp.known_feats + ((size_t)b * P.interp.m + id[0]) * P.interp.pitch;
+    const float *k1 = P.interp.known_feats + ((size_t)b * P.interp.m + id[1]) * P.interp.pitch;
+    const float *k2 = P.interp.known_feats + ((size_t)b * P.interp.m + id[2]) * P.interp.pitch;
+#pragma unroll
+    for (int u = 0; u < U; ++u) {
+        if (u < nslots) {
+            const int c = 16 * u + 4 * g;
+            const bool ok = c < P.interp.channels;
+            const int cc = ok ? c : 0;
+            const f4 a0 = *reinterpret_cast<const f4 *>(k0 + cc);
+            const f4 a1 = *reinterpret_cast<const f4 *>(k1 + cc);
+            const f4 a2 = *reinterpret_cast<const f4 *>(k2 + cc);
+            f4 v;
+            v.x = __fmaf_rn(w2, a2.x, __fmaf_rn(w1, a1.x, __fmul_rn(w0, a0.x)));
+            v.y = __fmaf_rn(w2, a2.y, __fmaf_rn(w1, a1.y, __fmul_rn(w0, a0.y)));
+            v.z = __fmaf_rn(w2, a2.z, __fmaf_rn(w1, a1.z, __fmul_rn(w0, a0.z)));
+            v.w = __fmaf_rn(w2, a2.w, __fmaf_rn(w1, a1.w, __fmul_rn(w0, a0.w)));
+            h[u] = ok ? v : f4_zero();
         }
     }
 }
@@ -138,40 +174,7 @@
         const int p = b * rps + (r < rps ? r : rps - 1);
 
         f4 h[U];
-        if (INTERP) {
-            const int *idp = P.interp.idx + (size_t)p * 3;
-            int id[3] = {idp[0], idp[1], idp[2]};
-            if (P.interp.nuniq) {
-                const int e = P.interp.nuniq[b];
-                id[0] = id[0] < e ? id[0] : 0; id[1] = id[1] < e ? id[1] : 0; id[2] = id[2] < e ? id[2] : 0;
-            }
-            const float *d2 = P.interp.dist2 + (size_t)p * 3;
-            const float r0 = __fdiv_rn(1.0f, __fadd_rn(__fsqrt_rn(d2[0]), 1e-8f));
-            const float r1 = __fdiv_rn(1.0f, __fadd_rn(__fsqrt_rn(d2[1]), 1e-8f));
-            const float r2 = __fdiv_rn(1.0f, __fadd_rn(__fsqrt_rn(d2[2]), 1e-8f));
-            const float norm = __fadd_rn(__fadd_rn(r0, r1), r2);
-            const float w0 = __fdiv_rn(r0, norm), w1 = __fdiv_rn(r1, norm), w2 = __fdiv_rn(r2, norm);
-            const float *k0 = P.interp.known_feats + ((size_t)b * P.interp.m + id[0]) * P.interp.pitch;
-            const float *k1 = P.interp.known_feats + ((size_t)b * P.interp.m + id[1]) * P.interp.pitch;
-            const float *k2 = P.interp.known_feats + ((size_t)b * P.interp.m + id[2]) * P.interp.pitch;
-#pragma unroll
-            for (int u = 0; u < U; ++u) {
-                if (u < ustart[0]) {
-                    const int c = 16 * u + 4 * g;
-                    const bool ok = c < P.interp.channels;
-                    const int cc = ok ? c : 0;
-                    const f4 a0 = *reinterpret_cast<const f4 *>(k0 + cc);
-                    const f4 a1 = *reinterpret_cast<const f4 *>(k1 + cc);
-                    const f4 a2 = *reinterpret_cast<const f4 *>(k2 + cc);
-                    f4 v;
-                    v.x = __fmaf_rn(w2, a2.x, __fmaf_rn(w1, a1.x, __fmul_rn(w0, a0.x)));
-                    v.y = __fmaf_rn(w2, a2.y, __fmaf_rn(w1, a1.y, __fmul_rn(w0, a0.y)));
-                    v.z = __fmaf_rn(w2, a2.z, __fmaf_rn(w1, a1.z, __fmul_rn(w0, a0.z)));
-                    v.w = __fmaf_rn(w2, a2.w, __fmaf_rn(w1, a1.w, __fmul_rn(w0, a0.w)));
-                    h[u] = ok ? v : f4_zero();
-                }
-            }
-        }
+        if (INTERP) load_interp<U>(P, p, b, g, ustart[0], h);
         const float *rowp[RTK_MAX_SRC];
         const float *dummy = reinterpret_cast<const float *>(P.layer[0].w_packed);
 #pragma unroll
@@ -312,3 +315,164 @@
     RTK_CHECK_LAUNCH("pointwise_mlp");
     return RTK_OK;
 }
+
+template <int NW, int F, int NF, int C1, int UP, int VH>
+struct WStreamTap {
+    static constexpr int NCHUNKS = NF / F, PR = 2 * VH, PH = UP * PR;
+    static_assert(NF % F == 0 && PR % F == 0 && C1 < NCHUNKS, "whole chunks; a chunk of the projection is one run of the image");
+    const char *blob;
+    const char *proj;
+    f4 *lds;
+    unsigned lane_off;
+    int cur, buf, wave, lane;
+    __device__ __forceinline__ void issue(int chunk, int into) {
+        const char *base;
+        if (chunk < C1) {
+            base = blob + (size_t)chunk * F * 1024;
+        } else {
+            const int l = (chunk - C1) * F, h = l / PH, up = (l % PH) / PR, r = l % PR;
+            base = proj + (size_t)(PR * (2 * up + h) + r) * 1024;
+        }
+#pragma unroll
+        for (int i = 0; i < (F + NW - 1) / NW; ++i) {
+            const int f = wave + i * NW;
+            if (f < F)
+                __builtin_amdgcn_global_load_lds((const __attribute__((address_space(1))) void *)(base + (size_t)i * NW * 1024 + lane_off),
+                                                 (__attribute__((address_space(3))) void *)(lds + (into * F + f) * 64), 16, 0, 0);
+        }
+    }
+    __device__ __forceinline__ void start_deferred(const f4 *blob_, const f4 *proj_, f4 *lds_, int wave_, int lane_) {
+        blob = reinterpret_cast<const char *>(blob_);
+        proj = reinterpret_cast<const char *>(proj_);
+        lds = lds_; wave = wave_; lane = lane_;
+        lane_off = (unsigned)(wave * 64 + lane) * 16u;
+        cur = NCHUNKS - 1; buf = 1;
+        issue(0, 0);
+    }
+    __device__ __forceinline__ void next() {
+        asm volatile("s_waitcnt vmcnt(0)" ::: "memory");
+        __syncthreads();
+        buf ^= 1;
+        cur = cur + 1 == NCHUNKS ? 0 : cur + 1;
+        asm volatile("" : "+s"(cur));
+        issue(cur + 1 == NCHUNKS ? 0 : cur + 1, buf ^ 1);
+    }
+    __device__ __forceinline__ f4 frag(int f_in_chunk) const { return lds[(buf * F + f_in_chunk) * 64 + lane]; }
+    __device__ __forceinline__ void finish() { asm volatile("s_waitcnt vmcnt(0)" ::: "memory"); }
+};
+
+struct TapParams {
+    PwParams pw;
+    const float *proj_w[2];
+    const float *proj_b[2];
+    float proj_inv[2];
+    int frame_split;
+    float *pout;
+    int pout_pitch;
+};
+
+template <int U, int V1, int VP>
+__global__ __launch_bounds__(64 * PW_NW, 2) void pointwise_tap_kernel(const TapParams T) {
+    __shared__ __attribute__((aligned(16))) f4 s_w[2 * PW_F * 64];
+    const PwParams &P = T.pw;
+    const int lane = threadIdx.x & 63, g = lane >> 4, j = lane & 15;
+    const int wave_in_wg = threadIdx.x >> 6;
+    int b, bx, nbx;
+    rtk_decode_block(P.gx, b, bx, nbx);
+    const int rps = P.rows_per_sample;
+    const int groups = (rps + PW_NW * 16 - 1) / (PW_NW * 16);
+    if (bx >= groups) return;
+    constexpr int UP = (V1 + 1) / 2, VH = VP / 2, F1 = split16_nf(U, V1), PH = UP * 2 * VH;
+    static_assert(VP % 2 == 0 && F1 % PW_F == 0, "whole chunks of the layer, two equal halves of the projection");
+    WStreamTap<PW_NW, PW_F, F1 + 2 * PH, F1 / PW_F, UP, VH> ws;
+    const bool f2 = b >= T.frame_split;
+    const float *pbias = f2 ? T.proj_b[1] : T.proj_b[0];
+    const float pinv = f2 ? T.proj_inv[1] : T.proj_inv[0];
+    ws.start_deferred(reinterpret_cast<const f4 *>(P.layer[0].w_packed), reinterpret_cast<const f4 *>(f2 ? T.proj_w[1] : T.proj_w[0]), s_w,
+                      wave_in_wg, lane);
+
+    for (int G = bx; G < groups; G += nbx) {
+        asm volatile("" ::: "memory");
+        const int r = G * (PW_NW * 16) + wave_in_wg * 16 + j;
+        const bool valid = r < rps;
+        const int p = b * rps + (valid ? r : rps - 1);
+        f4 h[U];
+        load_interp<U>(P, p, b, g, U, h);
+        f4 a1[V1];
+        {
+            const LaneScale s1 = lane_scale16(h);
+            init_zero<V1>(a1);
+            ws.next();
+            mlp_layer_split_impl<U, V1, 0, decltype(ws), PW_F>(ws, h, s1.s, a1, std::make_integer_sequence<int, ((U + 1) / 2) * ((V1 + 1) / 2)>{});
+            scale_bias<V1>(a1, s1.inv * P.layer[0].inv_scale, P.layer[0].bias, g);
+            apply_act<V1>(a1, P.layer[0].act);
+        }
+        store_tile<V1>(P, a1, p, b, g, valid);
+        const LaneScale sc = lane_scale16(a1);
+        u4v pc[UP][2];
+#pragma unroll
+        for (int up = 0; up < UP; ++up) split2(a1[2 * up], 2 * up + 1 < V1 ? a1[2 * up + 1] : f4_zero(), sc.s, pc[up]);
+        const float c = sc.inv * pinv;
+        float *o = T.pout + (size_t)p * T.pout_pitch + 4 * g;
+        auto half = [&](auto hc) {
+            constexpr int hv = decltype(hc)::value;
+            f4 acc[VH];
+            init_zero<VH>(acc);
+            mlp_layer_pieces_impl<V1, VH, F1 + hv * PH, decltype(ws), PW_F>(ws, pc, acc, std::make_integer_sequence<int, UP * (VH / 2)>{});
+            scale_bias<VH>(acc, c, pbias + 16 * VH * hv, g);
+            if (valid) {
+#pragma unroll
+                for (int v = 0; v < VH; ++v) *reinterpret_cast<f4 *>(o + 16 * (VH * hv + v)) = acc[v];
+            }
+        };
+        half(std::integral_constant<int, 0>{});
+        half(std::integral_constant<int, 1>{});
+    }
+    ws.finish();
+}
+
+extern "C" int rtk_pointwise_mlp_tap(int rows, int rows_per_sample, const rtk_interp_t *interp, const rtk_layer_t *layer, float *out,
+                                     int out_pitch, float *colmax, const rtk_layer_t *proj, int frame_split, float *proj_out, int proj_pitch,
+                                     rtk_stream_t stream) {
+    RTK_REQUIRE(rows > 0 && rows_per_sample > 0 && rows % rows_per_sample == 0 && rows / rows_per_sample <= 65535,
+                "pointwise_mlp_tap: bad row counts (%d, %d)", rows, rows_per_sample);
+    RTK_REQUIRE(interp && interp->known_feats && interp->idx && interp->dist2 && interp->pitch % 4 == 0 && interp->channels % 4 == 0 &&
+                (interp->channels + 15) / 16 == 8, "pointwise_mlp_tap: bad interp segment (128 channels)");
+    RTK_REQUIRE(layer && layer->w_packed && layer->bias && layer->cin16 == 8 && layer->cout16 == 8 && (layer->act & RTK_LAYER_SPLIT),
+                "pointwise_mlp_tap: the layer must be a split 128 -> 128 image");
+    RTK_REQUIRE(proj && frame_split >= 0 && proj_out && proj_pitch % 4 == 0 && proj_pitch >= 256, "pointwise_mlp_tap: bad projection output");
+    for (int k = 0; k < 2; ++k)
+        RTK_REQUIRE(proj[k].w_packed && proj[k].bias && proj[k].cin16 == 8 && proj[k].cout16 == 16 && (proj[k].act & RTK_LAYER_SPLIT) &&
+                    (proj[k].act & 0xff) == 0, "pointwise_mlp_tap: projection %d must be a split 128 -> 256 image without activation", k);
+    RTK_REQUIRE(out && out_pitch % 4 == 0 && out_pitch >= 128, "pointwise_mlp_tap: bad out_pitch %d", out_pitch);
+    TapParams T;
+    memset(&T, 0, sizeof(T));
+    PwParams &P = T.pw;
+    P.rows = rows;
+    P.rows_per_sample = rows_per_sample;
+    P.interp = *interp;
+    P.layer[0] = *layer;
+    P.layer[0].act = layer->act & 0xff;
+    P.out = out;
+    P.out_pitch = out_pitch;
+    P.out_channels = 128;
+    P.colmax = colmax;
+    for (int k = 0; k < 2; ++k) {
+        T.proj_w[k] = proj[k].w_packed;
+        T.proj_b[k] = proj[k].bias;
+        T.proj_inv[k] = proj[k].inv_scale;
+    }
+    T.frame_split = frame_split;
+    T.pout = proj_out;
+    T.pout_pitch = proj_pitch;
+    const int samples = rows / rows_per_sample;
+    const int groups = (rows_per_sample + PW_NW * 16 - 1) / (PW_NW * 16);
+    int gx = PW_WGS_TARGET / samples;
+    if (gx < 1) gx = 1;
+    if (gx > groups) gx = groups;
+    P.gx = samples % 8 == 0 ? gx : 0;
+    const dim3 blocks = P.gx ? dim3(gx * samples) : dim3(gx, samples);
+    pointwise_tap_kernel<8, 8, 16><<<blocks, 64 * PW_NW, 0, (hipStream_t)stream>>>(T);
+    RTK_CHECK_LAUNCH("pointwise_mlp_tap");
+    return RTK_OK;
+}
diff --git a/ratrack_amd/csrc/fused_split.hip b/ratrack_amd/csrc/fused_split.hip
--- a/ratrack_amd/csrc/fused_split.hip
+++ b/ratrack_amd/csrc/fused_split.hip
@@ -105,6 +105,7 @@
     const float *xyz1, *xyz2;
     const int64_t *knn;
     const float *p1, *p2;
+    const float *st;
     const float *wd;
     const f4 *blob;
     const float *wsc;
@@ -252,6 +253,9 @@
         : "=&v"(o.x), "=&v"(o.y), "=&v"(o.z), "=&v"(o.w)
         : "v"(q.x), "v"(q.y), "v"(q.z), "v"(q.w), "v"(r.x), "v"(r.y), "v"(r.z), "v"(r.w), "n"(K));
     return o;
+}
+__device__ __forceinline__ f4 add4_rn(const f4 a, const f4 b) {
+    return (f4){__fadd_rn(a.x, b.x), __fadd_rn(a.y, b.y), __fadd_rn(a.z, b.z), __fadd_rn(a.w, b.w)};
 }
 template <int V0, int V1>
 __device__ __forceinline__ void cv_layer1_blocks(const CvSplitParams &P, const f4 q0, const f4 q1, float b0, float b1, int hh, int col, float kinf, f4 (&h)[32]) {
@@ -313,6 +317,7 @@
         nb = (long)b * P.n2 + (long)P.knn[i * 16 + j];
         cv_rows_request<0>(P.p2, (int)nb, rows, lane);
         q0 = ldc4(P.p1 + i * 256 + 4 * hh + 8 * j); q1 = ldc4(P.p1 + i * 256 + 4 * hh + 8 * (16 + j));
+        if (P.st) { q0 = add4_rn(q0, ldc4(P.st + b * 256 + 4 * hh + 8 * j)); q1 = add4_rn(q1, ldc4(P.st + b * 256 + 4 * hh + 8 * (16 + j))); }
         dx = __fsub_rn(P.xyz2[nb * 3], P.xyz1[i * 3]); dy = __fsub_rn(P.xyz2[nb * 3 + 1], P.xyz1[i * 3 + 1]);
         dz = __fsub_rn(P.xyz2[nb * 3 + 2], P.xyz1[i * 3 + 2]);
     }
@@ -391,15 +396,17 @@
         out_block(0);
         out_block(1);
         float cn[6] = {0.f, 0.f, 0.f, 0.f, 0.f, 0.f};
-        f4 q0n = q0, q1n = q1;
+        f4 q0n = q0, q1n = q1, s0n = q0, s1n = q1;
         if (more) {
 #pragma unroll
             for (int c = 0; c < 3; ++c) { cn[c] = ldc(P.xyz2 + nbn * 3 + c); cn[3 + c] = ldc(P.xyz1 + in_ * 3 + c); }
             q0n = ldc4(P.p1 + in_ * 256 + 4 * hh + 8 * j); q1n = ldc4(P.p1 + in_ * 256 + 4 * hh + 8 * (16 + j));
         }
+        if (more && P.st) { s0n = ldc4(P.st + bn * 256 + 4 * hh + 8 * j); s1n = ldc4(P.st + bn * 256 + 4 * hh + 8 * (16 + j)); }
 #pragma unroll
         for (int v = 2; v < SPLIT_VB; ++v) out_block(v);
         pt = ptn; valid = validn; i = in_; nb = nbn; q0 = q0n; q1 = q1n;
+        if (P.st) { q0 = add4_rn(q0n, s0n); q1 = add4_rn(q1n, s1n); }
         dx = __fsub_rn(cn[0], cn[3]); dy = __fsub_rn(cn[1], cn[4]); dz = __fsub_rn(cn[2], cn[5]);
     }
     ws.finish();
@@ -699,7 +706,7 @@
     P.blob = reinterpret_cast<const f4 *>(split_images);
     P.wsc = image_scales;
     P.wn.wa = wn[0].w_packed; P.wn.wb = wn[1].w_packed; P.wn.wc = wn[2].w_packed; P.wn.bb = wn[1].bias; P.wn.bc = wn[2].bias;
-    P.p1 = P.p2 = P.wd = P.bias2 = P.bias3 = nullptr;
+    P.p1 = P.p2 = P.st = P.wd = P.bias2 = P.bias3 = nullptr;
     P.out = nullptr; P.out_pitch = 0; P.sv1 = P.sv2 = P.sv3 = nullptr; P.mk1 = P.mk2 = nullptr; P.amax = nullptr;
     const int groups = (n1 + 2 * SP_NW - 1) / (2 * SP_NW);
     int gx = 256 / samples;
@@ -719,7 +726,8 @@
 static int cv_split_forward(const char *who, int samples, int n1, int n2, const float *xyz1, const float *xyz2, const int64_t *knn_idx,
                             const float *p1, const float *p2, const float *wd_packed, const void *split_images, const float *image_scales,
                             const float *bias2, const float *bias3, const rtk_layer_t *wn, float *out, int out_pitch, float *a1, float *a2,
-                            float *a3, void *mask1, void *mask2, float *amax, int workgroups, rtk_stream_t stream) {
+                            float *a3, void *mask1, void *mask2, float *amax, int workgroups, rtk_stream_t stream,
+                            const float *sample_term = nullptr) {
     CvSplitParams P;
     dim3 grid;
     if (cv_split_fill(who, P, samples, n1, n2, xyz1, xyz2, knn_idx, split_images, image_scales, wn, grid) != RTK_OK) return RTK_ERR_INVALID;
@@ -729,7 +737,7 @@
     const bool save = a1 != nullptr;
     RTK_REQUIRE(!save || ((double)samples * n1 * 16.0 * 1024.0 < 4294967296.0), "%s: more than 4 GiB per saved activation (32-bit row "
                 "offsets): split the batch", who);
-    P.p1 = p1; P.p2 = p2; P.wd = wd_packed; P.bias2 = bias2; P.bias3 = bias3; P.out = out; P.out_pitch = out_pitch;
+    P.p1 = p1; P.p2 = p2; P.st = sample_term; P.wd = wd_packed; P.bias2 = bias2; P.bias3 = bias3; P.out = out; P.out_pitch = out_pitch;
     P.sv1 = a1; P.sv2 = a2; P.sv3 = a3; P.mk1 = (uint2 *)mask1; P.mk2 = (uint2 *)mask2; P.amax = amax;
     if (samples % 8 == 0) {
         const int tiles_x = (samples / 8) * ((n1 + 2 * SP_NW - 1) / (2 * SP_NW));
@@ -760,6 +768,15 @@
     RTK_REQUIRE(workgroups >= 0, "cost_volume_split_shared: workgroups = %d", workgroups);
     return cv_split_forward("cost_volume_split_shared", samples, n1, n2, xyz1, xyz2, knn_idx, p1, p2, wd_packed, split_images, image_scales,
                             bias2, bias3, wn, out, out_pitch, nullptr, nullptr, nullptr, nullptr, nullptr, nullptr, workgroups, stream);
+}
+
+extern "C" int rtk_cost_volume_split_term(int samples, int n1, int n2, const float *xyz1, const float *xyz2, const int64_t *knn_idx,
+                                          const float *p1, const float *p2, const float *sample_term, const float *wd_packed,
+                                          const void *split_images, const float *image_scales, const float *bias2, const float *bias3,
+                                          const rtk_layer_t *wn, float *out, int out_pitch, int workgroups, rtk_stream_t stream) {
+    RTK_REQUIRE(workgroups >= 0 && sample_term, "cost_volume_split_term: workgroups = %d, sample_term = %p", workgroups, (const void *)sample_term);
+    return cv_split_forward("cost_volume_split_term", samples, n1, n2, xyz1, xyz2, knn_idx, p1, p2, wd_packed, split_images, image_scales,
+                            bias2, bias3, wn, out, out_pitch, nullptr, nullptr, nullptr, nullptr, nullptr, nullptr, workgroups, stream, sample_term);
 }
 
 extern "C" int rtk_cost_volume_split_train(int samples, int n1, int n2, const float *xyz1, const float *xyz2, const int64_t *knn_idx,
diff --git a/ratrack_amd/fused.py b/ratrack_amd/fused.py
--- a/ratrack_amd/fused.py
+++ b/ratrack_amd/fused.py
@@ -27,12 +27,15 @@
 _lib.SIGNATURES.update({
     "rtk_pointwise_mlp": [_ci, _ci, ctypes.POINTER(_Interp), _ci, ctypes.POINTER(_Src), _vp, _ci, ctypes.POINTER(_Layer), _vp,
                           _ci, _ci, _ci, _vp, _vp, _vp],
+    "rtk_pointwise_mlp_tap": [_ci, _ci, ctypes.POINTER(_Interp), ctypes.POINTER(_Layer), _vp, _ci, _vp, ctypes.POINTER(_Layer), _ci, _vp, _ci,
+                              _vp],
     "rtk_sa_scale": [_ci] * 4 + [_vp] * 4 + [_ci, _ci, _vp, _ci, ctypes.POINTER(_Layer), _vp, _ci, _ci, _vp, _vp, _vp],
     "rtk_cost_volume": [_ci] * 3 + [_vp] * 6 + [ctypes.POINTER(_Layer), ctypes.POINTER(_Layer), _vp, _ci, _vp],
     "rtk_patch_cost": [_ci] * 2 + [_vp] * 3 + [_ci, ctypes.POINTER(_Layer), _vp, _ci, _ci, _vp],
     "rtk_pack_split_layer": [_ci, _ci, _vp, _ci, _vp, _vp, _vp],
     "rtk_cost_volume_split": [_ci] * 3 + [_vp] * 10 + [ctypes.POINTER(_Layer), _vp, _ci, _vp],
     "rtk_cost_volume_split_shared": [_ci] * 3 + [_vp] * 10 + [ctypes.POINTER(_Layer), _vp, _ci, _ci, _vp],
+    "rtk_cost_volume_split_term": [_ci] * 3 + [_vp] * 11 + [ctypes.POINTER(_Layer), _vp, _ci, _ci, _vp],
     "rtk_split_mlp2": [_ci, _vp, _vp, _vp, _vp, _vp, _vp, _vp],
     "rtk_sa_scale_split": [_ci] * 4 + [_vp] * 4 + [_ci, _ci, _vp, _vp, _vp, _vp, _vp, _ci, _ci, _vp, _vp, _vp],
     "rtk_prepare_inputs": [_ci] * 2 + [_vp] * 6 + [_vp],
@@ -59,7 +62,7 @@
 
 class _GtJob(ctypes.Structure):
     _fields_ = [("wt", ctypes.c_void_p), ("bias", ctypes.c_void_p), ("out", ctypes.c_void_p), ("cout", ctypes.c_int), ("s0", ctypes.c_int),
-                ("count", ctypes.c_int), ("out_pitch", ctypes.c_int)]
+                ("count", ctypes.c_int), ("out_pitch", ctypes.c_int), ("wt2", ctypes.c_void_p), ("s2", ctypes.c_int)]
 
 
 class _CopyJob(ctypes.Structure):
@@ -284,6 +287,23 @@
 
 
 pointwise_mlp = pointwise
+
+
+def pointwise_tap(rows, rows_per_sample, chain, out, colmax, interp, proj, frame_split, proj_out):
+    assert PW_SPLIT and chain.n == 1 and all(c.n == 1 for c in proj)
+    kf, ch, m, idx, d2 = interp[:5]
+    nu = interp[5] if len(interp) > 5 else None
+    ptr, pitch = _colptr(kf)
+    ip = ctypes.pointer(_Interp(ptr, pitch, ch, m, idx.data_ptr(), d2.data_ptr(), nu.data_ptr() if nu is not None else None))
+    if _TRACE is not None:
+        _TRACE.append(("pointwise", rows, sum(co * ci for co, ci in chain.dims) + 3 * ch))
+        _TRACE.append(("pointwise", rows, sum(co * ci for co, ci in proj[0].dims)))
+    pa = (_Layer * 2)(proj[0].split_arr()[0], proj[1].split_arr()[0])
+    optr, opitch = _colptr(out)
+    pptr, ppitch = _colptr(proj_out)
+    _lib.call("rtk_pointwise_mlp_tap", rows, rows_per_sample, ip, chain.split_arr(), optr, opitch, colmax.data_ptr(), pa, frame_split,
+              pptr, ppitch, _stream())
+    return out, proj_out
 
 
 def offset_image(w4, device):
@@ -610,7 +630,7 @@
               sc.chain.n, sc.chain.arr, optr, opitch, out_offset, src_nu, geo.nuniq[lvl].data_ptr(), _stream())
 
 
-def run_pnhead(W, geo, q1, out=None, gmax=None):
+def run_pnhead(W, geo, q1, out=None, gmax=None, tap=None):
     S_, n, S = geo.samples, geo.n, geo.npoint
     dev = q1.device
     new = lambda rows, c: torch.empty(rows, c, dtype=torch.float32, device=dev)
@@ -640,8 +660,12 @@
     d2, idx, m = geo.nn["fp1"]
     if gmax is None:
         gmax = torch.zeros(S_, 128, dtype=torch.float32, device=dev)
-    out = pointwise(S_ * n, n, [], W.fp["fp1"], out if out is not None else new(S_ * n, 128),
-                    interp=(f2, 128, m, idx.reshape(-1, 3), d2.reshape(-1, 3), nu[0]), colmax=gmax)
+    out = out if out is not None else new(S_ * n, 128)
+    interp = (f2, 128, m, idx.reshape(-1, 3), d2.reshape(-1, 3), nu[0])
+    if tap is not None:
+        pointwise_tap(S_ * n, n, W.fp["fp1"], out, gmax, interp, *tap)
+    else:
+        pointwise(S_ * n, n, [], W.fp["fp1"], out, interp=interp, colmax=gmax)
     return out, gmax
 
 
@@ -661,6 +685,7 @@
         self._split_hook = None
         self.side, self.use_side_stream = None, True
         self.cv_shared = False
+        self.proj_tap = True
         self._last_cv = None
         self.enc = _PNHeadWeights(sd, "pn_head.", dev)
         self.dec = _PNHeadWeights(sd, "fd_layer.mse.", dev)
@@ -732,18 +757,29 @@
             _TRACE.append(("pointwise", 2 * B * N, 64))
         feat12 = new(2 * B * N, 256)
         gmax = torch.zeros(3 * B, 128, dtype=torch.float32, device=dev)
-        loc, glob = run_pnhead(self.enc, geo, q1, out=feat12[:, 0:128], gmax=gmax[:2 * B])
+        tap = self.proj_tap and self.cv_split and PW_SPLIT
+        p12 = new(2 * B * N, 256) if tap else None
+        loc, glob = run_pnhead(self.enc, geo, q1, out=feat12[:, 0:128], gmax=gmax[:2 * B],
+                               tap=((self.p1_loc, self.p2_loc), B, p12) if tap else None)
         f1, f2 = loc[:B * N], loc[B * N:]
-        sb1, sb2, sbq = new(B, 256), new(B, 256), new(B, 32)
-        global_terms(glob, [(self.p1_glob_wt, self.p1_glob_b, sb1, 0), (self.p2_glob_wt, None, sb2, B), (self.dec_q1_glob_wt, None, sbq, 0)],
-                     bcast=feat12[:, 128:], n=N)
-        p1 = pointwise(B * N, N, [(f1, 128, False)], self.p1_loc, new(B * N, 256), sample_bias=sb1)
-        p2 = pointwise(B * N, N, [(f2, 128, False)], self.p2_loc, new(B * N, 256), sample_bias=sb2)
+        sbq = new(B, 32)
+        if tap:
+            st = new(B, 256)
+            global_terms(glob, [(self.p1_glob_wt, self.p1_glob_b, st, 0, self.p2_glob_wt, B), (self.dec_q1_glob_wt, None, sbq, 0)],
+                         bcast=feat12[:, 128:], n=N)
+            p1, p2 = p12[:B * N], p12[B * N:]
+        else:
+            st = None
+            sb1, sb2 = new(B, 256), new(B, 256)
+            global_terms(glob, [(self.p1_glob_wt, self.p1_glob_b, sb1, 0), (self.p2_glob_wt, None, sb2, B), (self.dec_q1_glob_wt, None, sbq, 0)],
+                         bcast=feat12[:, 128:], n=N)
+            p1 = pointwise(B * N, N, [(f1, 128, False)], self.p1_loc, new(B * N, 256), sample_bias=sb1)
+            p2 = pointwise(B * N, N, [(f2, 128, False)], self.p2_loc, new(B * N, 256), sample_bias=sb2)
         x1, x2 = xyz[:B], xyz[B:]
         geo.wait("knn")
         knn1, knn2 = geo.knn
         cor1 = new(B * N, 256)
-        self._last_cv = (B, N, x1, x2, knn1, p1, p2, cor1)
+        self._last_cv = (B, N, x1, x2, knn1, p1, p2, cor1, st)
         if self._split_hook is not None:
             geo.events.clear()
             self._split_hook()
@@ -777,7 +813,8 @@
         prop_cm = prop.view(B, N, 128).permute(0, 2, 1)
         return flow, h_out, cls, cor_cm, pc1_features, pc2_features, prop_cm
 
-    def _cost_volume(self, B, N, x1, x2, knn1, p1, p2, cor1):
+    def _cost_volume(self, B, N, x1, x2, knn1, p1, p2, cor1, sample_term=None):
+        assert sample_term is None or self.cv_split
         if _TRACE is not None:
             _TRACE.append(("cost_volume", B * N * 16, 3 * 256 + 2 * 256 * 256 + (3 * 8 + 8 * 8 + 8 * 256) + 256))
         if self.cv_split:
@@ -786,6 +823,12 @@
                 nb = min(step, B - b0)
                 wgs = cv_shared_workgroups(nb, N, x1.device) if self.cv_shared else 0
                 r0 = b0 * N
+                if sample_term is not None:
+                    _lib.call("rtk_cost_volume_split_term", nb, N, N, x1[b0:].data_ptr(), x2[b0:].data_ptr(), knn1[b0:].data_ptr(),
+                              p1[r0:].data_ptr(), p2[r0:].data_ptr(), sample_term[b0:].data_ptr(), self.cv_wd.data_ptr(),
+                              self.cv_images.data_ptr(), self.cv_scales.data_ptr(), self.cv_bias23[0].data_ptr(), self.cv_bias23[1].data_ptr(),
+                              self.wn1.arr, cor1[r0:].data_ptr(), 256, wgs, _stream())
+                    continue
                 _lib.call("rtk_cost_volume_split_shared", nb, N, N, x1[b0:].data_ptr(), x2[b0:].data_ptr(), knn1[b0:].data_ptr(), p1[r0:].data_ptr(),
                           p2[r0:].data_ptr(), self.cv_wd.data_ptr(), self.cv_images.data_ptr(), self.cv_scales.data_ptr(),
                           self.cv_bias23[0].data_ptr(), self.cv_bias23[1].data_ptr(), self.wn1.arr, cor1[r0:].data_ptr(), 256, wgs, _stream())
@@ -892,12 +935,16 @@
 def global_terms(g, jobs, bcast=None, n=0):
     samples, cin = g.shape
     arr = (_GtJob * max(len(jobs), 1))()
-    for j, (wt, bias, out, s0) in enumerate(jobs):
+    for j, job in enumerate(jobs):
+        wt, bias, out, s0 = job[:4]
+        wt2, s2 = job[4:] if len(job) > 4 else (None, 0)
         assert wt.shape == (cin, out.shape[1]) and out.is_contiguous() and wt.is_contiguous()
+        assert wt2 is None or (wt2.shape == wt.shape and wt2.is_contiguous())
         arr[j].wt, arr[j].bias, arr[j].out = wt.data_ptr(), bias.data_ptr() if bias is not None else None, out.data_ptr()
         arr[j].cout, arr[j].s0, arr[j].count, arr[j].out_pitch = out.shape[1], s0, out.shape[0], out.shape[1]
+        arr[j].wt2, arr[j].s2 = wt2.data_ptr() if wt2 is not None else None, s2
     if _TRACE is not None:
-        _TRACE.append(("global_terms", 1, sum(cin * o.shape[0] * o.shape[1] for _, _, o, _ in jobs)))
+        _TRACE.append(("global_terms", 1, sum(cin * j[2].shape[0] * j[2].shape[1] * (2 if len(j) > 4 else 1) for j in jobs)))
     bptr, bpitch = _colptr(bcast) if bcast is not None else (None, 0)
     _lib.call("rtk_global_terms", samples, cin, g.data_ptr(), len(jobs), arr, bptr, bpitch, n, _stream())
 
```

Result: faster. 104,100 frame-pairs/s (median of 6 runs) (+1.3%).
